# ActiveVisionLab/DFNet

Measured on AMD Instinct MI355X. Metric: rendered rays/sec (64+128 samples, 640x480), higher is better.
Workload: dtype f16x3; 1 GPU; BASELINE configs[1]: synthetic random-weight NeRF-H (D=8, W=128), 640x480, 64+128 samples, test-time render_image, 1 frame per step per GPU; parallelism=frames sharded over 1 GPU(s), gather at end, collectives=none (one rank)

## Files before the change

### dfnet_amd/csrc/nerfh_api.hip

```cpp
#include <hip/hip_runtime.h>

#include <cmath>
#include <cstdarg>
#include <cstdio>
#include <cstdlib>
#include <cstring>
#include <map>
#include <string>
#include <type_traits>
#include <vector>

#include "../../include/dfnet_hip.h"
#include "dfn_common.h"
#include "nerfh_fused_train.h"
#include "nerfh_handle.h"
#include "nerfh_kernels.h"
#include "nerfh_layout.h"

using namespace dfn;

namespace dfn {
static thread_local char g_err[512] = "";
int set_error(int code, const char* fmt, ...) {
  va_list ap;
  va_start(ap, fmt);
  vsnprintf(g_err, sizeof g_err, fmt, ap);
  va_end(ap);
  return code;
}
int device_cu_count() {
  static int n = 0;
  if (!n) {
    int dev = 0;
    hipDeviceProp_t p;
    if (hipGetDevice(&dev) == hipSuccess && hipGetDeviceProperties(&p, dev) == hipSuccess) n = p.multiProcessorCount;
    if (n <= 0) n = 256;
  }
  return n;
}
}

extern "C" const char* dfn_last_error(void) { return g_err; }
extern "C" int dfn_abi_version(void) { return 1; }

static std::map<std::string, std::vector<size_t>> expected_shapes(const dfn_nerfh_desc& d) {
  std::map<std::string, std::vector<size_t>> m;
  const size_t W = d.width, na = size_t(d.hist_bin) * d.dim_a, nt = size_t(d.hist_bin) * d.dim_t;
  for (int f = 0; f < 2; ++f) {
    const std::string pre = f ? "fine." : "coarse.";
    for (int i = 0; i < d.depth; ++i) {
      const size_t k = i == 0 ? kChXyz : (i == 4 ? W + kChXyz : W);
      m[pre + "xyz_encoding_" + std::to_string(i + 1) + ".0.weight"] = {W, k};
      m[pre + "xyz_encoding_" + std::to_string(i + 1) + ".0.bias"] = {W};
    }
    m[pre + "xyz_encoding_final.weight"] = {W, W};
    m[pre + "xyz_encoding_final.bias"] = {W};
    m[pre + "dir_encoding.0.weight"] = {W / 2, W + kChDir + (f ? na : 0)};
    m[pre + "dir_encoding.0.bias"] = {W / 2};
    m[pre + "static_sigma.0.weight"] = {1, W};
    m[pre + "static_sigma.0.bias"] = {1};
    m[pre + "static_rgb.0.weight"] = {3, W / 2};
    m[pre + "static_rgb.0.bias"] = {3};
    if (f) {
      const size_t ks[4] = {W + nt, W / 2, W / 2, W / 2};
      for (int j = 0; j < 4; ++j) {
        m[pre + "transient_encoding." + std::to_string(2 * j) + ".weight"] = {W / 2, ks[j]};
        m[pre + "transient_encoding." + std::to_string(2 * j) + ".bias"] = {W / 2};
      }
      m[pre + "transient_sigma.0.weight"] = {1, W / 2};
      m[pre + "transient_sigma.0.bias"] = {1};
      m[pre + "transient_rgb.0.weight"] = {3, W / 2};
      m[pre + "transient_rgb.0.bias"] = {3};
      m[pre + "transient_beta.0.weight"] = {1, W / 2};
      m[pre + "transient_beta.0.bias"] = {1};
    }
  }
  m["embedding_a.weight"] = {size_t(d.n_vocab), size_t(d.dim_a)};
  m["embedding_t.weight"] = {size_t(d.n_vocab), size_t(d.dim_t)};
  return m;
}

extern "C" int dfn_nerfh_create(const dfn_nerfh_desc* desc, dfn_nerfh_t* out) {
  if (!desc || !out) return set_error(DFN_ERR_ARG, "dfn_nerfh_create: null argument");
  if (desc->depth != 8 || desc->multires != kLxyz || desc->multires_views != kLdir)
    return set_error(DFN_ERR_UNSUPPORTED,
                     "dfn_nerfh_create: kernels are specialised for netdepth=8 multires=%d multires_views=%d (got %d/%d/%d)",
                     kLxyz, kLdir, desc->depth, desc->multires, desc->multires_views);
  if (desc->width < 2 || desc->width > 1024 || (desc->width & 1))
    return set_error(DFN_ERR_UNSUPPORTED, "dfn_nerfh_create: netwidth must be even and in [2, 1024] (got %d)", desc->width);
  if (desc->hist_bin <= 0 || desc->dim_a <= 0 || desc->dim_t <= 0 || desc->n_vocab <= 0 ||
      desc->hist_bin * (desc->dim_a + desc->dim_t) > 1024)
    return set_error(DFN_ERR_ARG, "dfn_nerfh_create: bad embedding geometry");
  auto* h = new dfn_nerfh_s();
  h->desc = *desc;
  *out = h;
  return DFN_OK;
}

static void free_packed(dfn_nerfh_s* h) {
  for (auto& a : h->net)
    for (auto& b : a)
      for (auto& n : b) {
        if (n.blob) (void)hipFree(n.blob);
        if (n.tab) (void)hipFree(n.tab);
        if (n.res_blob) (void)hipFree(n.res_blob);
        n = PackedNet();
      }
  for (PackedNet* n : {&h->bwd[0], &h->bwd[1], &h->bwd[2], &h->half_maps}) {
    if (n->blob) (void)hipFree(n->blob);
    if (n->tab) (void)hipFree(n->tab);
    *n = PackedNet();
  }
  if (h->extra) (void)hipFree(h->extra);
  h->extra = nullptr;
  if (h->gen_blob) (void)hipFree(h->gen_blob);
  h->gen_blob = nullptr;
  h->gen_params.clear();
  h->fast = false;
}

extern "C" int dfn_nerfh_destroy(dfn_nerfh_t h) {
  if (!h) return DFN_OK;
  free_packed(h);
  dfn::fused::destroy_state(h);
  for (hipEvent_t e : h->side_ev) if (e) (void)hipEventDestroy(e);
  if (h->side_stream) (void)hipStreamDestroy(h->side_stream);
  if (h->range_flag) (void)hipFree(h->range_flag);
  delete h;
  return DFN_OK;
}

extern "C" int dfn_nerfh_set_param(dfn_nerfh_t h, const char* name, const float* host, size_t numel) {
  if (!h || !name || !host) return set_error(DFN_ERR_ARG, "dfn_nerfh_set_param: null argument");
  const auto shapes = expected_shapes(h->desc);
  const auto it = shapes.find(name);
  if (it == shapes.end()) return set_error(DFN_ERR_ARG, "dfn_nerfh_set_param: unknown parameter '%s'", name);
  size_t want = 1;
  for (size_t s : it->second) want *= s;
  if (want != numel)
    return set_error(DFN_ERR_ARG, "dfn_nerfh_set_param: '%s' has %zu elements, expected %zu", name, numel, want);
  h->params[name].assign(host, host + numel);
  h->committed = false;
  return DFN_OK;
}

namespace {

struct Mat {
  const float* w = nullptr;
  const float* b = nullptr;
  int rows = 0, cols = 0;
};

struct Packer {
  const dfn_nerfh_s* h;
  std::string pre;
  int width() const { return h->desc.width; }
  mutable int fwd_units = 0;
  std::vector<float> fold_dir, fold_tr;
  bool half_heads = false, half_thead = false;
  bool half_block(int layer) const { return half_heads && (layer == LY_SIG || layer == LY_RGB || (layer == LY_THEAD && half_thead)); }
  Mat mat(const std::string& key) const {
    Mat m;
    const auto& w = h->params.at(pre + key + ".weight");
    const auto& b = h->params.at(pre + key + ".bias");
    m.w = w.data();
    m.b = b.data();
    m.rows = int(b.size());
    m.cols = int(w.size() / b.size());
    return m;
  }
  void row_source(int layer, int mb, int i, Mat& m, int& row) const {
    row = 32 * mb + i;
    switch (layer) {
      case LY_L1: case LY_L2: case LY_L3: case LY_L4: case LY_L5: case LY_L6: case LY_L7: case LY_L8:
        m = mat("xyz_encoding_" + std::to_string(layer - LY_L1 + 1) + ".0");
        break;
      case LY_FIN:
        if (mb < width() / 32) m = mat("xyz_encoding_final");
        else { m = mat("static_sigma.0"); row = i == 0 ? 0 : -1; }
        break;
      case LY_DIR: m = mat("dir_encoding.0"); break;
      case LY_RGB: m = mat("static_rgb.0"); row = i < 3 ? i : -1; break;
      case LY_TE0: m = mat("transient_encoding.0"); break;
      case LY_TE1: m = mat("transient_encoding.2"); break;
      case LY_TE2: m = mat("transient_encoding.4"); break;
      case LY_TE3: m = mat("transient_encoding.6"); break;
      case LY_THEAD:
        if (i < 3) { m = mat("transient_rgb.0"); row = i; }
        else if (i == 3) { m = mat("transient_sigma.0"); row = 0; }
        else if (i == 8) { m = mat("transient_beta.0"); row = 0; }
        else { m = mat("transient_beta.0"); row = -1; }
        break;
      case LY_SIG: m = mat("static_sigma.0"); row = i == 0 ? 0 : -1; break;
      case LY_DIRF: case LY_TE0F:
        m = Mat();
        m.w = (layer == LY_DIRF ? fold_dir : fold_tr).data();
        m.rows = width() / 2;
        m.cols = width();
        break;
    }
  }
  static int col_source(int layer, int hh, int s) {
    if (layer == LY_L1) return pe_xyz_feature(hh, s);
    if (layer == LY_L5) return s < 32 ? pe_xyz_feature(hh, s) : kChXyz + hidden_feature(hh, s - 32);
    return hidden_feature(hh, s);
  }
  static int col_source_m16(int layer, int g, int s) {
    if (layer == LY_L1) return pe_xyz_feature_m16(g, s);
    if (layer == LY_L5) return s < 16 ? pe_xyz_feature_m16(g, s) : kChXyz + hidden_feature_m16(g, s - 16);
    return hidden_feature_m16(g, s);
  }
  bool head_block(int layer, int mb) const {
    return layer == LY_RGB || layer == LY_THEAD || layer == LY_SIG || (layer == LY_FIN && mb == width() / 32);
  }
  int row_m16(int layer, int mb, int i) const { return head_block(layer, mb) ? head_row_m16(i) : i; }
  static bool unit_has_bias(int layer) { return layer != LY_DIR && layer != LY_TE0 && layer != LY_DIRF && layer != LY_TE0F; }

  float wscale = 1.f;
  template <class P>
  void pack_blocks(int layer, int mb0, int group, uint8_t* base) const {
    using Elem = typename std::conditional<P::kSlotsPerChunk == 8, _Float16, float>::type;
    const LayerShape sh = layer_shape(layer, width());
    const int KC = sh.slots / P::kSlotsPerChunk;
    Elem* frag = reinterpret_cast<Elem*>(base);
    const bool half = P::kM16 && half_block(layer);
    const int KCP = half ? KC / 2 : KC;
    float* bias = reinterpret_cast<float*>(base + size_t(group) * KCP * 64 * P::kLaneBytes);
    for (int g = 0; g < group; ++g) {
      const int mb = mb0 + g;
      if constexpr (P::kM16) {
        auto source = [&](int i, Mat& m, int& row) {
          const int ri = row_m16(layer, mb, i);
          if (ri < 0) { m = Mat(); row = -1; return; }
          row_source(layer, mb, ri, m, row);
          if (row >= m.rows) row = -1;
        };
        for (int lane = 0; lane < 64; ++lane)
          for (int kc = 0; kc < KC; ++kc) {
            if (half && (kc & 1)) continue;
            Mat m;
            int row;
            source(16 * (kc & 1) + (lane & 15), m, row);
            for (int j = 0; j < 8; ++j) {
              const int col = col_source_m16(layer, lane >> 4, 8 * (kc >> 1) + j);
              const float v = (row >= 0 && col >= 0 && col < m.cols) ? m.w[size_t(row) * m.cols + col] : 0.f;
              Elem* fr = frag + (size_t(g) * KCP + (half ? kc >> 1 : kc)) * 64 * 16;
              const Elem hi = Elem(v * wscale);
              fr[lane * 8 + j] = hi;
              fr[512 + lane * 8 + j] = Elem(v * wscale - float(hi));
            }
          }
        for (int lg = 0; lg < 4; ++lg)
          for (int ms = 0; ms < 2; ++ms)
            for (int r = 0; r < 4; ++r) {
              Mat m;
              int row;
              source(16 * ms + 4 * lg + r, m, row);
              const float b = (row >= 0 && unit_has_bias(layer)) ? m.b[row] : 0.f;
              bias[g * 32 + lg * 8 + ms * 4 + r] = b * wscale * kX3ActScale;
            }
        continue;
      }
      for (int lane = 0; lane < 64; ++lane) {
        const int i = lane & 31, hh = lane >> 5;
        Mat m;
        int row;
        row_source(layer, mb, i, m, row);
        if (row >= m.rows) row = -1;
        for (int kc = 0; kc < KC; ++kc)
          for (int j = 0; j < P::kSlotsPerChunk; ++j) {
            const int col = col_source(layer, hh, kc * P::kSlotsPerChunk + j);
            const float v = (row >= 0 && col >= 0 && col < m.cols) ? m.w[size_t(row) * m.cols + col] : 0.f;
            if constexpr (P::kSplit) {
              Elem* fr = frag + (size_t(g) * KC + kc) * 64 * 16;
              const Elem hi = Elem(v * wscale);
              fr[lane * 8 + j] = hi;
              fr[512 + lane * 8 + j] = Elem(v * wscale - float(hi));
            } else {
              frag[((size_t(g) * KC + kc) * 64 + lane) * P::kSlotsPerChunk + j] = Elem(v);
            }
          }
      }
      for (int hh = 0; hh < 2; ++hh)
        for (int r = 0; r < 16; ++r) {
          Mat m;
          int row;
          row_source(layer, mb, mblock_row(hh, r), m, row);
          if (row >= m.rows) row = -1;
          const float b = (row >= 0 && unit_has_bias(layer)) ? m.b[row] : 0.f;
          bias[(g * 2 + hh) * 16 + r] = P::kSplit ? b * wscale * kX3ActScale : b;
        }
    }
  }
  float bwd_elem(int layer, int mb, int i, int hh, int s) const {
    const int k = 32 * mb + i;
    auto W = [](const Mat& m, int row, int col) {
      return (row >= 0 && row < m.rows && col >= 0 && col < m.cols) ? m.w[size_t(row) * m.cols + col] : 0.f;
    };
    auto pe_col = [&](int blk) { return pe_xyz_feature(mblock_half_of_row(i), 16 * blk + mblock_reg_of_row(i)); };
    const int j = hidden_feature(hh, s);
    switch (layer) {
      case BW_THEAD:
        if (j < 3) return W(mat("transient_rgb.0"), j, k);
        if (j == 3) return W(mat("transient_sigma.0"), 0, k);
        if (j == 8) return W(mat("transient_beta.0"), 0, k);
        return 0.f;
      case BW_TE3: return W(mat("transient_encoding.6"), j, k);
      case BW_TE2: return W(mat("transient_encoding.4"), j, k);
      case BW_TE1: return W(mat("transient_encoding.2"), j, k);
      case BW_RGB: return j < 3 ? W(mat("static_rgb.0"), j, k) : 0.f;
      case BW_FINCAT: {
        const bool dirpart = s >= 32;
        const int jj = hidden_feature(hh, s & 31);
        if (mb < 4) return W(mat(dirpart ? "dir_encoding.0" : "transient_encoding.0"), jj, k);
        if (!dirpart) return 0.f;
        const int c = pe_dir_feature(mblock_half_of_row(i), mblock_reg_of_row(i));
        return c >= 0 ? W(mat("dir_encoding.0"), jj, kWidth + c) : 0.f;
      }
      case BW_FIN:
        if (s < 64) return W(mat("xyz_encoding_final"), j, k);
        return (s == 64 && hh == 0) ? W(mat("static_sigma.0"), 0, k) : 0.f;
      case BW_L5:
        if (mb < 4) return W(mat("xyz_encoding_5.0"), j, kChXyz + k);
        return W(mat("xyz_encoding_5.0"), j, pe_col(mb - 4));
      case BW_L1: return W(mat("xyz_encoding_1.0"), j, pe_col(mb));
      default: {
        const int n = 8 - (layer - BW_L8);
        return W(mat("xyz_encoding_" + std::to_string(n) + ".0"), j, k);
      }
    }
  }
  template <class P>
  void pack_bwd_blocks(int layer, int mb0, int group, uint8_t* base) const {
    using Elem = typename std::conditional<P::kSlotsPerChunk == 8, _Float16, float>::type;
    const LayerShape sh = bwd_layer_shape(layer);
    const int KC = sh.slots / P::kSlotsPerChunk;
    Elem* frag = reinterpret_cast<Elem*>(base);
    for (int g = 0; g < group; ++g)
      for (int lane = 0; lane < 64; ++lane)
        for (int kc = 0; kc < KC; ++kc)
          for (int j = 0; j < P::kSlotsPerChunk; ++j) {
            const float v = bwd_elem(layer, mb0 + g, lane & 31, lane >> 5, kc * P::kSlotsPerChunk + j);
            if constexpr (P::kSplit) {
              Elem* fr = frag + (size_t(g) * KC + kc) * 64 * 16;
              const Elem hi = Elem(v * wscale);
              fr[lane * 8 + j] = hi;
              fr[512 + lane * 8 + j] = Elem(v * wscale - float(hi));
            } else {
              frag[((size_t(g) * KC + kc) * 64 + lane) * P::kSlotsPerChunk + j] = Elem(v);
            }
          }
  }
  template <class PF, class P>
  void pack_bwd(std::vector<uint8_t>& blob, std::vector<uint32_t>& tab) const {
    pack<PF>(true, bwd_fwd_unit_mb<PF>(), false, blob, tab);
    fwd_units = int(tab.size() / 2);
    const int umb = bwd_unit_mb<P>();
    for (int layer = 0; layer < BW_COUNT; ++layer) {
      const LayerShape sh = bwd_layer_shape(layer);
      for (int u0 = 0; u0 < sh.mb; u0 += umb) {
        const int mb0 = (umb <= 2 && layer == BW_L5) ? (u0 < 2 ? 4 + u0 : u0 - 2) : u0;
        const int group = sh.mb - mb0 < umb ? sh.mb - mb0 : umb;
        const uint32_t bytes = unit_bytes<P>(sh.slots, group);
        const uint32_t off = uint32_t(blob.size());
        blob.resize(off + bytes, 0);
        tab.push_back(off);
        tab.push_back(bytes);
        pack_bwd_blocks<P>(layer, mb0, group, blob.data() + off);
      }
    }
  }

  template <class P>
  uint32_t blocks_bytes(int layer, int group) const {
    const LayerShape sh = layer_shape(layer, width());
    const bool half = P::kM16 && half_block(layer);
    return uint32_t(group) * (sh.slots / P::kSlotsPerChunk / (half ? 2 : 1)) * 64 * P::kLaneBytes + uint32_t(group) * 128;
  }

  template <class P>
  void pack(bool fine, int umb, bool merge, std::vector<uint8_t>& blob, std::vector<uint32_t>& tab, int l5_umb = -1, bool fold = false,
            std::vector<uint8_t>* res = nullptr) const {
    const int* seq = fine ? (fold ? kFineFoldSeq : kFineSeq) : kCoarseSeq;
    const int* grp = fine ? kFineGroup : kCoarseGroup;
    const int nl = fine ? kFineLayers : kCoarseLayers;
    if (merge) {
      for (int li = 0; li < nl;) {
        int lj = li;
        uint32_t bytes = 0;
        while (lj < nl && grp[lj] == grp[li]) bytes += blocks_bytes<P>(seq[lj], layer_shape(seq[lj], width()).mb), ++lj;
        if (seq[li] == LY_L5) {
          const LayerShape sh = layer_shape(LY_L5, width());
          const int g = l5_unit_mb(umb);
          for (int mb0 = 0; mb0 < sh.mb; mb0 += g) {
            const uint32_t ub = unit_bytes<P>(sh.slots, g), uo = uint32_t(blob.size());
            blob.resize(uo + ub, 0);
            tab.push_back(uo);
            tab.push_back(ub);
            pack_blocks<P>(LY_L5, mb0, g, blob.data() + uo);
          }
          li = lj;
          continue;
        }
        const uint32_t off = uint32_t(blob.size());
        blob.resize(off + align_piece(bytes), 0);
        tab.push_back(off);
        tab.push_back(align_piece(bytes));
        uint32_t at = off;
        for (int l = li; l < lj; ++l) {
          pack_blocks<P>(seq[l], 0, layer_shape(seq[l], width()).mb, blob.data() + at);
          at += blocks_bytes<P>(seq[l], layer_shape(seq[l], width()).mb);
        }
        li = lj;
      }
      return;
    }
    for (int li = 0; li < nl; ++li) {
      const LayerShape sh = layer_shape(seq[li], width());
      const int lu = (seq[li] == LY_L5 && l5_umb > 0) ? l5_umb : umb;
      for (int mb0 = 0; mb0 < sh.mb; mb0 += lu) {
        const int group = sh.mb - mb0 < lu ? sh.mb - mb0 : lu;
        if (res && layer_resident(fine, seq[li])) {
          const size_t at = res->size();
          res->resize(at + blocks_bytes<P>(seq[li], group), 0);
          pack_blocks<P>(seq[li], mb0, group, res->data() + at);
          continue;
        }
        const uint32_t bytes = unit_bytes<P>(sh.slots, group, P::kM16 && half_block(seq[li]));
        const uint32_t off = uint32_t(blob.size());
        blob.resize(off + bytes, 0);
        tab.push_back(off);
        tab.push_back(bytes);
        pack_blocks<P>(seq[li], mb0, group, blob.data() + off);
      }
    }
    if (res) res->resize(align_piece(uint32_t(res->size())), 0);
  }
};

void fold_final(const std::vector<float>& a, int rows, int lda, const std::vector<float>& F, const std::vector<float>& bF, int W,
                std::vector<float>& af, std::vector<float>& ab) {
  af.assign(size_t(rows) * W, 0.f);
  ab.assign(rows, 0.f);
  std::vector<double> acc(W);
  for (int r = 0; r < rows; ++r) {
    std::fill(acc.begin(), acc.end(), 0.0);
    double b = 0.0;
    for (int k = 0; k < W; ++k) {
      const double ark = a[size_t(r) * lda + k];
      const float* frow = &F[size_t(k) * W];
      for (int c = 0; c < W; ++c) acc[c] += ark * double(frow[c]);
      b += ark * double(bF[k]);
    }
    for (int c = 0; c < W; ++c) af[size_t(r) * W + c] = float(acc[c]);
    ab[r] = float(b);
  }
}

int upload(const void* src, size_t bytes, void** dst) {
  if (hipMalloc(dst, bytes ? bytes : 16) != hipSuccess) return set_error(DFN_ERR_HIP, "hipMalloc(%zu) failed", bytes);
  if (bytes && hipMemcpy(*dst, src, bytes, hipMemcpyHostToDevice) != hipSuccess)
    return set_error(DFN_ERR_HIP, "hipMemcpy H2D (%zu bytes) failed", bytes);
  return DFN_OK;
}

}

__global__ void range_fetch_kernel(int* flag) { flag[1] = atomicExch(flag, 0); }

extern "C" int dfn_nerfh_set_render_options(dfn_nerfh_t h, int flags) {
  if (!h) return set_error(DFN_ERR_ARG, "dfn_nerfh_set_render_options: null handle");
  if (flags & ~(DFN_RENDER_LINDISP | DFN_RENDER_COARSE_F16)) return set_error(DFN_ERR_UNSUPPORTED, "dfn_nerfh_set_render_options: unknown option bits 0x%x", flags);
  h->render_flags = flags;
  return DFN_OK;
}

extern "C" int dfn_nerfh_range_status(dfn_nerfh_t h, int* flags, void* stream) {
  if (!h) return set_error(DFN_ERR_ARG, "dfn_nerfh_range_status: null handle");
  int v = 0;
  if (h->range_flag) {
    hipStream_t s = static_cast<hipStream_t>(stream);
    hipLaunchKernelGGL(range_fetch_kernel, dim3(1), dim3(1), 0, s, h->range_flag);
    if (hipGetLastError() != hipSuccess || hipMemcpyAsync(&v, h->range_flag + 1, sizeof(int), hipMemcpyDeviceToHost, s) != hipSuccess ||
        hipStreamSynchronize(s) != hipSuccess)
      return set_error(DFN_ERR_HIP, "dfn_nerfh_range_status: reading the flag failed");
  }
  if (flags) { *flags = v; return DFN_OK; }
  if (v)
    return set_error(DFN_ERR_RANGE, "NeRF-H render: activations left the range of the %s arithmetic since the last check (%s); the frames rendered "
                     "since then are not the network's output: render them with DFN_PREC_F32",
                     (v & DFN_RANGE_F16_OVERFLOW) ? "f16" : "split-f16",
                     (v & DFN_RANGE_F16_OVERFLOW) ? "an f16 layer output overflowed to inf: |activation| > 65504"
                                                  : "a split-f16 hi half saturated: |activation| >= 4094 (hidden layers of the render kernels: "
                                                    ">= 4094 x the network's largest |weight|, the accumulators are narrowed before they are scaled)");
  return DFN_OK;
}

extern "C" int dfn_nerfh_range_status_async(dfn_nerfh_t h, int* host_flags, void* stream) {
  if (!h || !host_flags) return set_error(DFN_ERR_ARG, "dfn_nerfh_range_status_async: null handle / destination");
  if (!h->range_flag) { *host_flags = 0; return DFN_OK; }
  hipStream_t s = static_cast<hipStream_t>(stream);
  hipLaunchKernelGGL(range_fetch_kernel, dim3(1), dim3(1), 0, s, h->range_flag);
  if (hipGetLastError() != hipSuccess || hipMemcpyAsync(host_flags, h->range_flag + 1, sizeof(int), hipMemcpyDeviceToHost, s) != hipSuccess)
    return set_error(DFN_ERR_HIP, "dfn_nerfh_range_status_async: enqueueing the read failed");
  return DFN_OK;
}

extern "C" int dfn_nerfh_commit(dfn_nerfh_t h) {
  if (!h) return set_error(DFN_ERR_ARG, "dfn_nerfh_commit: null handle");
  for (const auto& kv : expected_shapes(h->desc))
    if (!h->params.count(kv.first)) return set_error(DFN_ERR_STATE, "dfn_nerfh_commit: parameter '%s' not set", kv.first.c_str());
  free_packed(h);
  dfn::fused::destroy_state(h);
  if (!h->range_flag) {
    if (hipMalloc(reinterpret_cast<void**>(&h->range_flag), 3 * sizeof(int)) != hipSuccess) {
      h->range_flag = nullptr;
      return set_error(DFN_ERR_HIP, "dfn_nerfh_commit: allocating the range-guard flag failed");
    }
    if (hipMemset(h->range_flag, 0, 3 * sizeof(int)) != hipSuccess) return set_error(DFN_ERR_HIP, "dfn_nerfh_commit: clearing the range-guard flag failed");
  }
  {
    std::vector<float> all;
    std::vector<size_t> offs;
    const int np = dfn_nerfh_train_param_count();
    for (int i = 0; i < np; ++i) {
      const auto& v = h->params.at(dfn_nerfh_train_param_name(i));
      offs.push_back(all.size());
      all.insert(all.end(), v.begin(), v.end());
      all.resize((all.size() + 3) & ~size_t(3));
    }
    int rc = upload(all.data(), all.size() * 4, reinterpret_cast<void**>(&h->gen_blob));
    if (rc) return rc;
    for (size_t o : offs) h->gen_params.push_back(h->gen_blob + o);
  }
  const int Wd = h->desc.width;
  std::vector<float> fold_bd, fold_bt;
  if (Wd != kWidth && Wd != kMaxWidth) {
    h->committed = true;
    return DFN_OK;
  }
  if (Wd == kMaxWidth) {
    for (int f = 0; f < 2; ++f)
      for (int prec = 0; prec < 3; ++prec) {
        Packer pk{h, f ? "fine." : "coarse."};
        std::vector<uint8_t> blob;
        std::vector<uint32_t> tab;
        PackedNet& n = h->net[f][prec][0];
        if (prec == DFN_PREC_F16) pk.pack<PrecF16>(f, unit_mb_w256<PrecF16>(), false, blob, tab);
        else if (prec == DFN_PREC_F32) pk.pack<PrecF32>(f, unit_mb_w256<PrecF32>(), false, blob, tab);
        else {
          float wmax = 0.f;
          for (const auto& kv : h->params)
            if (kv.first.compare(0, pk.pre.size(), pk.pre) == 0 && kv.first.find(".weight") != std::string::npos)
              for (float v : kv.second) wmax = std::fmax(wmax, std::fabs(v));
          int sexp = wmax > 0.f ? -int(std::ceil(std::log2(wmax))) : 0;
          sexp = sexp < -8 ? -8 : (sexp > 24 ? 24 : sexp);
          pk.wscale = std::ldexp(1.f, sexp);
          n.in_scale = pk.wscale * kX3ActScale;
          pk.pack<PrecX3>(f, unit_mb_w256<PrecX3>(), false, blob, tab);
        }
        int rc = upload(blob.data(), blob.size(), reinterpret_cast<void**>(&n.blob));
        if (rc) return rc;
        rc = upload(tab.data(), tab.size() * 4, reinterpret_cast<void**>(&n.tab));
        if (rc) return rc;
        n.n_units = int(tab.size() / 2);
      }
  } else {
  for (int f = 0; f < 2; ++f)
    for (int prec = 0; prec < 3; ++prec)
      for (int var = 0; var < kVariants; ++var) {
        const bool resident = var == kResidentVariant;
        const bool half = var == kHalfVariant || resident;
        const bool fold = var == kFoldVariant || (half && f == 1);
        if (var == kFoldVariant && !(f == 1 && prec == DFN_PREC_F16X3)) continue;
        if (half && prec != DFN_PREC_F16X3) continue;
        Packer pk{h, f ? "fine." : "coarse."};
        pk.half_heads = half;
        pk.half_thead = half;
        std::vector<uint8_t> blob, rblob;
        std::vector<uint8_t>* res = resident ? &rblob : nullptr;
        std::vector<uint32_t> tab;
        PackedNet& n = h->net[f][prec][var];
        if (prec == DFN_PREC_F16) pk.pack<PrecF16>(f, unit_mb<PrecF16>(var), unit_mb<PrecF16>(var) >= 8, blob, tab);
        else if (prec == DFN_PREC_F32) pk.pack<PrecF32>(f, unit_mb<PrecF32>(var), false, blob, tab);
        else {
          float wmax = 0.f;
          for (const auto& kv : h->params)
            if (kv.first.compare(0, pk.pre.size(), pk.pre) == 0 && kv.first.find(".weight") != std::string::npos)
              for (float v : kv.second) wmax = std::fmax(wmax, std::fabs(v));
          int sexp = wmax > 0.f ? -int(std::ceil(std::log2(wmax))) : 0;
          sexp = sexp < -8 ? -8 : (sexp > 24 ? 24 : sexp);
          pk.wscale = std::ldexp(1.f, sexp);
          n.in_scale = pk.wscale * kX3ActScale;
          if (fold) {
            const int ldd = Wd + kChDir + h->desc.hist_bin * h->desc.dim_a, ldt = Wd + h->desc.hist_bin * h->desc.dim_t;
            const auto& F = h->params.at("fine.xyz_encoding_final.weight");
            const auto& bF = h->params.at("fine.xyz_encoding_final.bias");
            fold_final(h->params.at("fine.dir_encoding.0.weight"), Wd / 2, ldd, F, bF, Wd, pk.fold_dir, fold_bd);
            fold_final(h->params.at("fine.transient_encoding.0.weight"), Wd / 2, ldt, F, bF, Wd, pk.fold_tr, fold_bt);
            pk.pack<PrecX3M16>(f, unit_mb<PrecX3M16>(var), false, blob, tab, l5_unit_mb_p<PrecX3M16>(unit_mb<PrecX3M16>(var)), true, res);
            if (half && !resident) {
              std::vector<uint8_t> mblob;
              std::vector<uint32_t> mtab;
              pk.half_thead = false;
              pk.pack<PrecX3M16>(f, unit_mb<PrecX3M16>(var), false, mblob, mtab, l5_unit_mb_p<PrecX3M16>(unit_mb<PrecX3M16>(var)), true);
              PackedNet& m = h->half_maps;
              m.in_scale = n.in_scale;
              int rc = upload(mblob.data(), mblob.size(), reinterpret_cast<void**>(&m.blob));
              if (rc) return rc;
              rc = upload(mtab.data(), mtab.size() * 4, reinterpret_cast<void**>(&m.tab));
              if (rc) return rc;
              m.n_units = int(mtab.size() / 2);
            }
          } else if (var == 4 || half) pk.pack<PrecX3M16>(f, unit_mb<PrecX3M16>(var), false, blob, tab, l5_unit_mb_p<PrecX3M16>(unit_mb<PrecX3M16>(var)), false, res);
          else pk.pack<PrecX3>(f, unit_mb<PrecX3>(var), false, blob, tab, l5_unit_mb_p<PrecX3>(unit_mb<PrecX3>(var)));
        }
        int rc = upload(blob.data(), blob.size(), reinterpret_cast<void**>(&n.blob));
        if (rc) return rc;
        rc = upload(tab.data(), tab.size() * 4, reinterpret_cast<void**>(&n.tab));
        if (rc) return rc;
        n.n_units = int(tab.size() / 2);
        if (resident) {
          if (rblob.size() != resident_bytes<PrecX3M16>(f != 0))
            return set_error(DFN_ERR_STATE, "dfn_nerfh_commit: the resident layers pack to %zu bytes, the kernels expect %u", rblob.size(),
                             resident_bytes<PrecX3M16>(f != 0));
          rc = upload(rblob.data(), rblob.size(), reinterpret_cast<void**>(&n.res_blob));
          if (rc) return rc;
          n.res_bytes = uint32_t(rblob.size());
        }
      }
  for (int prec = 0; prec < 3; ++prec) {
    Packer pk{h, "fine."};
    std::vector<uint8_t> blob;
    std::vector<uint32_t> tab;
    PackedNet& n = h->bwd[prec];
    if (prec == DFN_PREC_F16) pk.pack_bwd<PrecF16, PrecF16>(blob, tab);
    else if (prec == DFN_PREC_F32) pk.pack_bwd<PrecF32, PrecF32>(blob, tab);
    else {
      n.in_scale = h->net[1][2][0].in_scale * 1024.f;
      pk.wscale = n.in_scale / kX3ActScale;
      pk.pack_bwd<PrecX3, PrecX3>(blob, tab);
    }
    int rc = upload(blob.data(), blob.size(), reinterpret_cast<void**>(&n.blob));
    if (rc) return rc;
    rc = upload(tab.data(), tab.size() * 4, reinterpret_cast<void**>(&n.tab));
    if (rc) return rc;
    n.n_units = int(tab.size() / 2);
    n.n_fwd_units = pk.fwd_units;
  }
  }
  const dfn_nerfh_desc& d = h->desc;
  const int na = d.hist_bin * d.dim_a, nt = d.hist_bin * d.dim_t, kd = kChDir + na, NO = Wd / 2;
  const auto& wd = h->params.at("fine.dir_encoding.0.weight");
  const auto& bd = h->params.at("fine.dir_encoding.0.bias");
  const auto& wt = h->params.at("fine.transient_encoding.0.weight");
  const auto& bt = h->params.at("fine.transient_encoding.0.bias");
  const auto& ea = h->params.at("embedding_a.weight");
  const auto& et = h->params.at("embedding_t.weight");
  std::vector<float> ex;
  const size_t o_wd = 0, o_bd = o_wd + size_t(kd) * NO, o_wt = o_bd + NO, o_bt = o_wt + size_t(nt) * NO,
               o_ea = o_bt + NO, o_et = o_ea + ea.size(), o_bdf = o_et + et.size(), o_btf = o_bdf + NO;
  ex.resize(o_btf + NO);
  const int ld_d = Wd + kd, ld_t = Wd + nt;
  for (int j = 0; j < kd; ++j)
    for (int f = 0; f < NO; ++f) ex[o_wd + size_t(j) * NO + f] = wd[size_t(f) * ld_d + Wd + j];
  for (int j = 0; j < nt; ++j)
    for (int f = 0; f < NO; ++f) ex[o_wt + size_t(j) * NO + f] = wt[size_t(f) * ld_t + Wd + j];
  std::memcpy(&ex[o_bd], bd.data(), NO * 4);
  std::memcpy(&ex[o_bt], bt.data(), NO * 4);
  std::memcpy(&ex[o_ea], ea.data(), ea.size() * 4);
  std::memcpy(&ex[o_et], et.data(), et.size() * 4);
  for (int f = 0; f < NO; ++f) {
    ex[o_bdf + f] = fold_bd.empty() ? bd[f] : bd[f] + fold_bd[f];
    ex[o_btf + f] = fold_bt.empty() ? bt[f] : bt[f] + fold_bt[f];
  }
  int rc = upload(ex.data(), ex.size() * 4, reinterpret_cast<void**>(&h->extra));
  if (rc) return rc;
  h->rb.w_dir = h->extra + o_wd;
  h->rb.b_dir = h->extra + o_bd;
  h->rb.w_tr = h->extra + o_wt;
  h->rb.b_tr = h->extra + o_bt;
  h->rb.emb_a = h->extra + o_ea;
  h->rb.emb_t = h->extra + o_et;
  h->rb.hist_bin = d.hist_bin;
  h->rb.dim_a = d.dim_a;
  h->rb.dim_t = d.dim_t;
  h->rb.n_vocab = d.n_vocab;
  h->rb.nout = NO;
  h->rb_fold = h->rb;
  h->rb_fold.b_dir = h->extra + o_bdf;
  h->rb_fold.b_tr = h->extra + o_btf;
  h->committed = true;
  h->fast = true;
  return DFN_OK;
}

namespace {
struct KernelTimer {
  bool on = false;
  std::vector<std::pair<hipEvent_t, hipEvent_t>> ev[DFN_PROF_SLOTS];
} g_prof;
struct ScopedTimer {
  int which;
  hipStream_t s;
  hipEvent_t a = nullptr, b = nullptr;
  ScopedTimer(int w, hipStream_t st) : which(w), s(st) {
    if (!g_prof.on) return;
    (void)hipEventCreate(&a);
    (void)hipEventCreate(&b);
    (void)hipEventRecord(a, s);
  }
  ~ScopedTimer() {
    if (!a) return;
    (void)hipEventRecord(b, s);
    g_prof.ev[which].emplace_back(a, b);
  }
};
}

extern "C" int dfn_profile_enable(int on) {
  for (auto& v : g_prof.ev) {
    for (auto& p : v) { (void)hipEventDestroy(p.first); (void)hipEventDestroy(p.second); }
    v.clear();
  }
  g_prof.on = on != 0;
  return DFN_OK;
}
extern "C" int dfn_profile_read(int which, double* avg_ms, int* launches) {
  if (which < 0 || which >= DFN_PROF_SLOTS || !avg_ms || !launches) return set_error(DFN_ERR_ARG, "dfn_profile_read: bad argument");
  double tot = 0;
  for (auto& p : g_prof.ev[which]) {
    float ms = 0;
    if (hipEventSynchronize(p.second) != hipSuccess || hipEventElapsedTime(&ms, p.first, p.second) != hipSuccess)
      return set_error(DFN_ERR_HIP, "dfn_profile_read: event query failed");
    tot += ms;
  }
  *launches = int(g_prof.ev[which].size());
  *avg_ms = *launches ? tot / *launches : 0.0;
  return DFN_OK;
}

#define HS(s) reinterpret_cast<hipStream_t>(s)
#define CHECK_HIP(expr, what)                                                                   \
  do {                                                                                          \
    hipError_t e_ = (expr);                                                                     \
    if (e_ != hipSuccess) return set_error(DFN_ERR_HIP, "%s: %s", what, hipGetErrorString(e_)); \
  } while (0)

static int check_net(dfn_nerfh_t h, int prec, const char* fn, bool allow_x3 = false) {
  if (!h) return set_error(DFN_ERR_ARG, "%s: null handle", fn);
  if (!h->committed) return set_error(DFN_ERR_STATE, "%s: dfn_nerfh_commit() has not been called", fn);
  if (!h->fast)
    return set_error(DFN_ERR_UNSUPPORTED, "%s: the register-resident kernels exist for netwidth %d and %d (this handle: %d); "
                     "use the generic-width entry points (dfn_nerfh_generic_*)", fn, kWidth, kMaxWidth, h->desc.width);
  if (prec != DFN_PREC_F16 && prec != DFN_PREC_F32 && !(allow_x3 && prec == DFN_PREC_F16X3))
    return set_error(DFN_ERR_ARG, "%s: unknown / unsupported precision %d", fn, prec);
  return DFN_OK;
}

static int check_grad_width(dfn_nerfh_t h, const char* fn) {
  if (h->desc.width != kWidth)
    return set_error(DFN_ERR_UNSUPPORTED, "%s: the input-gradient kernels are built for netwidth %d only (this handle: %d)", fn, kWidth,
                     h->desc.width);
  return DFN_OK;
}
static int check_grad_prec(int prec, const char* fn) {
  if (prec == DFN_PREC_F16)
    return set_error(DFN_ERR_UNSUPPORTED, "%s: gradients run in DFN_PREC_F16X3 or DFN_PREC_F32 only (plain-f16 ReLU gates are 3e-2 off "
                     "autograd)", fn);
  return DFN_OK;
}

constexpr int kDefaultVariant = kResidentVariant;
static int mlp_variant_128();
static int mlp_variant_of(dfn_nerfh_t h) { return h->desc.width == kWidth ? mlp_variant_128() : 0; }
static int mlp_variant_128() {
  static int v = -1;
  if (v < 0) {
    const char* e = getenv("DFN_MLP_VARIANT");
    v = (e && e[0] >= '0' && e[0] < '0' + kVariants) ? e[0] - '0' : kDefaultVariant;
  }
  return v;
}
static int base_variant(int var) { return var == kFoldVariant || var == kHalfVariant || var == kResidentVariant ? 4 : var; }
static bool fold_fine(int var, int prec) { return (var == kFoldVariant || var == kHalfVariant || var == kResidentVariant) && prec == DFN_PREC_F16X3; }
static bool half_heads(int var, int prec) { return (var == kHalfVariant || var == kResidentVariant) && prec == DFN_PREC_F16X3; }
static bool resident_layers(int var, int prec) { return var == kResidentVariant && prec == DFN_PREC_F16X3; }
static MlpResArgs res_args(const MlpArgs& a, const PackedNet& n) {
  MlpResArgs r{};
  static_cast<MlpArgs&>(r) = a;
  r.res_blob = n.res_blob;
  r.res_bytes = n.res_bytes;
  return r;
}

static int* range_flag_of(dfn_nerfh_t h) { return h->range_flag; }

static unsigned long long* g_timing_buf = nullptr;
extern "C" void dfn_debug_set_timing_buffer(void* p) { g_timing_buf = static_cast<unsigned long long*>(p); }


extern "C" int dfn_raygen(int H, int W, float focal, const float* c2w, float* rays_o, float* rays_d,
                          float* viewdirs, void* stream) {
  if (H < 0 || W < 0 || !c2w || !rays_o || !rays_d || !(focal > 0)) return set_error(DFN_ERR_ARG, "dfn_raygen: bad argument");
  CHECK_HIP(launch_raygen(H, W, focal, c2w, rays_o, rays_d, viewdirs, HS(stream)), "dfn_raygen");
  return DFN_OK;
}

extern "C" int dfn_posenc(const float* x, size_t n, int L, int mode, float* out, void* stream) {
  if (!x || !out || L < 0 || L > 16 || (mode != 0 && mode != 1)) return set_error(DFN_ERR_ARG, "dfn_posenc: bad argument");
  CHECK_HIP(launch_posenc(x, n, L, mode, out, HS(stream)), "dfn_posenc");
  return DFN_OK;
}

extern "C" int dfn_mlp_coarse(dfn_nerfh_t h, int prec, const float* rays_o, const float* rays_d, size_t n_rays,
                              int Nc, float near, float far, float* sigma, void* stream) {
  if (int rc = check_net(h, prec, "dfn_mlp_coarse", true)) return rc;
  if (!n_rays) return DFN_OK;
  if (!rays_o || !rays_d || !sigma || Nc < 1) return set_error(DFN_ERR_ARG, "dfn_mlp_coarse: bad argument");
  const bool half = half_heads(mlp_variant_of(h), prec), res = resident_layers(mlp_variant_of(h), prec);
  const int var = base_variant(mlp_variant_of(h));
  const PackedNet& n = h->net[0][prec][res ? kResidentVariant : (half ? kHalfVariant : var)];
  MlpArgs a{n.blob, n.tab, n.n_units, rays_o, rays_d, nullptr, nullptr, sigma, nullptr, (long long)n_rays, Nc, near, far, nullptr, n.in_scale,
            h->render_flags & DFN_RENDER_LINDISP};
  a.status = range_flag_of(h);
  ScopedTimer t(0, HS(stream));
  if (res) CHECK_HIP(launch_mlp_res(false, res_args(a, n), device_cu_count(), HS(stream)), "dfn_mlp_coarse");
  else if (half) CHECK_HIP(launch_mlp_half(false, false, a, device_cu_count(), HS(stream)), "dfn_mlp_coarse");
  else CHECK_HIP(launch_mlp(false, prec, var, a, device_cu_count(), HS(stream), h->desc.width), "dfn_mlp_coarse");
  return DFN_OK;
}

extern "C" int dfn_coarse_weights(const float* sigma, const float* z, size_t n, int N, float* weights, void* stream) {
  if (!sigma || !z || !weights || N < 1 || N > 2048) return set_error(DFN_ERR_ARG, "dfn_coarse_weights: bad argument");
  CHECK_HIP(launch_coarse_weights(sigma, z, n, N, weights, HS(stream)), "dfn_coarse_weights");
  return DFN_OK;
}

extern "C" int dfn_sample_pdf(const float* bins, const float* weights, size_t n, int nb, int Ni, const float* u,
                              float* out, void* stream) {
  if (!bins || !weights || !out || nb < 2 || Ni < 1 || 3 * nb + 2 * Ni > 8192)
    return set_error(DFN_ERR_ARG, "dfn_sample_pdf: bad argument");
  CHECK_HIP(launch_sample_pdf(bins, weights, n, nb, Ni, u, out, HS(stream)), "dfn_sample_pdf");
  return DFN_OK;
}

extern "C" int dfn_sample_fine_opt(const float* sigma, size_t n_rays, int Nc, int Ni, float near, float far, int render_flags,
                                   float* z_fine, float* weights_coarse, float* z_samples, void* stream) {
  if (!sigma || !z_fine || Nc < 3 || Ni < 1 || 6 * Nc + 2 * Ni > 8192)
    return set_error(DFN_ERR_ARG, "dfn_sample_fine: bad argument (need N_samples >= 3, N_importance >= 1)");
  if ((render_flags & DFN_RENDER_LINDISP) && !(near > 0.f))
    return set_error(DFN_ERR_ARG, "dfn_sample_fine: lindisp needs near > 0");
  CHECK_HIP(launch_sample_fine(sigma, n_rays, Nc, Ni, near, far, z_fine, weights_coarse, z_samples, HS(stream),
                               render_flags & DFN_RENDER_LINDISP),
            "dfn_sample_fine");
  return DFN_OK;
}
extern "C" int dfn_sample_fine(const float* sigma, size_t n_rays, int Nc, int Ni, float near, float far,
                               float* z_fine, float* weights_coarse, float* z_samples, void* stream) {
  return dfn_sample_fine_opt(sigma, n_rays, Nc, Ni, near, far, 0, z_fine, weights_coarse, z_samples, stream);
}

extern "C" int dfn_ndc_rays(int H, int W, float focal, float near, const float* rays_o, const float* rays_d, size_t n, float* out_o,
                            float* out_d, void* stream) {
  if (!n) return DFN_OK;
  if (!rays_o || !rays_d || !out_o || !out_d || H < 1 || W < 1 || !(focal > 0.f)) return set_error(DFN_ERR_ARG, "dfn_ndc_rays: bad argument");
  CHECK_HIP(launch_ndc_rays(H, W, focal, near, rays_o, rays_d, n, out_o, out_d, HS(stream)), "dfn_ndc_rays");
  return DFN_OK;
}

extern "C" int dfn_upsample_bicubic(const float* in, int H, int W, int C, int outH, int outW, float* out, void* stream) {
  if (!in || !out || H < 1 || W < 1 || C < 1 || outH < 1 || outW < 1) return set_error(DFN_ERR_ARG, "dfn_upsample_bicubic: bad argument");
  CHECK_HIP(launch_bicubic(in, H, W, C, outH, outW, out, HS(stream)), "dfn_upsample_bicubic");
  return DFN_OK;
}

extern "C" int dfn_upsample_bicubic_frames(const float* in, int B, int H, int W, int C, int outH, int outW, int out_nchw, float* out,
                                           void* stream) {
  if (!in || !out || B < 1 || H < 1 || W < 1 || C < 1 || outH < 1 || outW < 1) return set_error(DFN_ERR_ARG, "dfn_upsample_bicubic_frames: bad argument");
  CHECK_HIP(launch_bicubic(in, H, W, C, outH, outW, out, HS(stream), B, out_nchw != 0), "dfn_upsample_bicubic_frames");
  return DFN_OK;
}
extern "C" int dfn_upsample_bicubic_frames_backward(const float* grad_out, int B, int H, int W, int C, int outH, int outW, int out_nchw,
                                                    float* grad_in, void* stream) {
  if (!grad_out || !grad_in || B < 1 || H < 1 || W < 1 || C < 1 || outH < 1 || outW < 1)
    return set_error(DFN_ERR_ARG, "dfn_upsample_bicubic_frames_backward: bad argument");
  CHECK_HIP(launch_bicubic_backward(grad_out, H, W, C, outH, outW, grad_in, HS(stream), B, out_nchw != 0), "dfn_upsample_bicubic_frames_backward");
  return DFN_OK;
}

extern "C" int dfn_upsample_bicubic_backward(const float* grad_out, int H, int W, int C, int outH, int outW, float* grad_in,
                                             void* stream) {
  if (!grad_out || !grad_in || H < 1 || W < 1 || C < 1 || outH < 1 || outW < 1)
    return set_error(DFN_ERR_ARG, "dfn_upsample_bicubic_backward: bad argument");
  CHECK_HIP(launch_bicubic_backward(grad_out, H, W, C, outH, outW, grad_in, HS(stream)), "dfn_upsample_bicubic_backward");
  return DFN_OK;
}

extern "C" size_t dfn_fine_bias_bytes(size_t n_rays) { return (n_rays ? n_rays : 1) * ray_bias_floats(kMaxWidth) * sizeof(float); }

extern "C" int dfn_mlp_fine(dfn_nerfh_t h, int prec, const float* rays_o, const float* rays_d, const float* viewdirs,
                            const float* hist, size_t hist_rows, size_t n_rays, const float* z_fine, int Nf,
                            float* raw, void* bias_ws, void* stream) {
  if (int rc = check_net(h, prec, "dfn_mlp_fine", true)) return rc;
  if (!n_rays) return DFN_OK;
  if (!rays_o || !rays_d || !viewdirs || !hist || !z_fine || !raw || !bias_ws || Nf < 1 ||
      (hist_rows != 1 && hist_rows != n_rays))
    return set_error(DFN_ERR_ARG, "dfn_mlp_fine: bad argument (hist_rows must be 1 or n_rays)");
  float* table = static_cast<float*>(bias_ws);
  const bool fold = fold_fine(mlp_variant_of(h), prec);
  const int var = fold ? kFoldVariant : base_variant(mlp_variant_of(h));
  CHECK_HIP(launch_ray_bias(fold ? h->rb_fold : h->rb, viewdirs, hist, hist_rows, n_rays, table, HS(stream)), "dfn_mlp_fine(ray_bias)");
  const PackedNet& n = h->net[1][prec][var];
  MlpArgs a{n.blob, n.tab, n.n_units, rays_o, rays_d, z_fine, table, raw, nullptr, (long long)n_rays, Nf, 0.f, 0.f, g_timing_buf, n.in_scale};
  a.status = range_flag_of(h);
  ScopedTimer t(1, HS(stream));
  if (fold) CHECK_HIP(launch_mlp_fold(false, a, device_cu_count(), HS(stream)), "dfn_mlp_fine");
  else CHECK_HIP(launch_mlp(true, prec, var, a, device_cu_count(), HS(stream), h->desc.width), "dfn_mlp_fine");
  return DFN_OK;
}

extern "C" int dfn_composite_fine(const float* raw, const float* z, size_t n_rays, int Nf, float beta_min, int flags,
                                  float* rgb, float* disp, float* acc, float* depth, float* weights, float* beta,
                                  void* stream) {
  if (!raw || !z || !rgb || !disp || !acc || Nf < 1 || Nf > 512)
    return set_error(DFN_ERR_ARG, "dfn_composite_fine: bad argument (1 <= Nf <= 512)");
  CHECK_HIP(launch_composite_fine(raw, z, n_rays, Nf, beta_min, flags, rgb, disp, acc, depth, weights, beta, HS(stream)),
            "dfn_composite_fine");
  return DFN_OK;
}

static MapPtrs map_ptrs(const dfn_render_maps* m) {
  return m ? MapPtrs{m->depth, m->depth_static, m->beta, m->rgb_static, m->rgb_transient} : MapPtrs{};
}

extern "C" int dfn_composite_fine_maps(const float* raw, const float* z, size_t n_rays, int Nf, float beta_min,
                                       const dfn_render_maps* maps, void* stream) {
  if (!raw || !z || Nf < 1 || Nf > 512) return set_error(DFN_ERR_ARG, "dfn_composite_fine_maps: bad argument (1 <= Nf <= 512)");
  CHECK_HIP(launch_composite_fine_maps(raw, z, n_rays, Nf, beta_min, map_ptrs(maps), HS(stream)), "dfn_composite_fine_maps");
  return DFN_OK;
}

namespace {
constexpr size_t kMaxChunkRays = 65536;
inline size_t al(size_t b) { return (b + 255) & ~size_t(255); }
inline size_t chunk_rays(size_t n_rays) {
  const size_t passes = (n_rays + kMaxChunkRays - 1) / kMaxChunkRays;
  const size_t c = passes ? (n_rays + passes - 1) / passes : 1;
  return (c + 63) & ~size_t(63);
}
struct Workspace {
  float *o, *d, *v, *sigma, *z, *raw, *bias, *partial;
  size_t total;
};
Workspace carve(char* base, size_t n_rays, int Nc, int Ni, bool own_rays, int rec_floats = 12) {
  const size_t chunk = chunk_rays(n_rays);
  const size_t Nf = size_t(Nc) + Ni;
  Workspace w{};
  size_t off = 0;
  auto take = [&](size_t bytes) { char* p = base ? base + off : nullptr; off += al(bytes); return reinterpret_cast<float*>(p); };
  w.o = take(own_rays ? n_rays * 12 : 0);
  w.d = take(own_rays ? n_rays * 12 : 0);
  w.v = take(n_rays * 12);
  w.sigma = take(chunk * Nc * 4);
  w.z = take(chunk * Nf * 4);
  w.raw = take(chunk * Nf * 9 * 4);
  w.bias = take(chunk * ray_bias_floats(kMaxWidth) * 4);
  w.partial = take(chunk * ((Nf + 31) / 32) * rec_floats * 4);
  w.total = off;
  return w;
}

int render_core(dfn_nerfh_t h, int prec, const float* o, const float* d, const float* v, const float* hist,
                size_t hist_rows, size_t n_rays, int Nc, int Ni, float near, float far, float* rgb, float* disp,
                float* acc, float* raw_out, const Workspace& w, hipStream_t s, const MapPtrs& maps = MapPtrs{}) {
  const int Nf = Nc + Ni;
  const bool want_maps = maps.any();
  const bool fold = fold_fine(mlp_variant_of(h), prec);
  const int var = base_variant(mlp_variant_of(h));
  const int seg = prec == DFN_PREC_F16 ? 64 : 32;
  const bool fused = !raw_out && Nf % seg == 0 && !(prec == DFN_PREC_F16 && var == 2) && h->desc.width == kWidth;
  const int cprec = (h->render_flags & DFN_RENDER_COARSE_F16) ? DFN_PREC_F16 : prec;
  const bool half_c = half_heads(mlp_variant_of(h), cprec), half_f = half_heads(mlp_variant_of(h), prec) && fused;
  const bool res_c = resident_layers(mlp_variant_of(h), cprec), res_f = resident_layers(mlp_variant_of(h), prec) && fused && !want_maps;
  const PackedNet& nc = h->net[0][cprec][res_c ? kResidentVariant : (half_c ? kHalfVariant : var)];
  const PackedNet& nf = res_f ? h->net[1][prec][kResidentVariant]
                      : half_f ? (want_maps ? h->half_maps : h->net[1][prec][kHalfVariant]) : h->net[1][prec][fold ? kFoldVariant : var];
  const int cus = device_cu_count();
  const size_t chunk = chunk_rays(n_rays);
  for (size_t r0 = 0; r0 < n_rays; r0 += chunk) {
    const size_t n = n_rays - r0 < chunk ? n_rays - r0 : chunk;
    const float* co = o + r0 * 3;
    const float* cd = d + r0 * 3;
    const float* cv = v + r0 * 3;
    const float* ch = hist_rows == 1 ? hist : hist + r0 * h->desc.hist_bin;
    float* raw = raw_out ? raw_out + r0 * size_t(Nf) * 9 : w.raw;
    {
      MlpArgs a{nc.blob, nc.tab, nc.n_units, co, cd, nullptr, nullptr, w.sigma, nullptr, (long long)n, Nc, near, far, nullptr, nc.in_scale,
                 h->render_flags & DFN_RENDER_LINDISP};
      a.status = range_flag_of(h);
      ScopedTimer t(0, s);
      if (res_c) CHECK_HIP(launch_mlp_res(false, res_args(a, nc), cus, s), "render: coarse MLP (resident layers)");
      else if (half_c) CHECK_HIP(launch_mlp_half(false, false, a, cus, s), "render: coarse MLP (half-height heads)");
      else CHECK_HIP(launch_mlp(false, cprec, var, a, cus, s, h->desc.width), "render: coarse MLP");
    }
    {
      ScopedTimer t(DFN_PROF_SAMPLE_FINE, s);
      CHECK_HIP(launch_sample_fine(w.sigma, n, Nc, Ni, near, far, w.z, nullptr, nullptr, s, h->render_flags & DFN_RENDER_LINDISP),
                "render: sample_fine");
    }
    {
      ScopedTimer t(DFN_PROF_RAY_BIAS, s);
      CHECK_HIP(launch_ray_bias(fold ? h->rb_fold : h->rb, cv, ch, hist_rows, n, w.bias, s), "render: ray_bias");
    }
    {
      MlpArgs a{nf.blob, nf.tab, nf.n_units, co, cd, w.z, w.bias, raw, fused ? w.partial : nullptr, (long long)n, Nf, 0.f, 0.f, g_timing_buf, nf.in_scale};
      a.status = range_flag_of(h);
      ScopedTimer t(1, s);
      if (res_f) CHECK_HIP(launch_mlp_res(true, res_args(a, nf), cus, s), "render: fine MLP (resident layers)");
      else if (half_f) CHECK_HIP(launch_mlp_half(true, want_maps, a, cus, s), "render: fine MLP (half-height heads)");
      else if (fold) CHECK_HIP(launch_mlp_fold(fused && want_maps, a, cus, s), "render: fine MLP (folded)");
      else if (fused && want_maps) CHECK_HIP(launch_mlp_maps(true, prec, var, a, cus, s, h->desc.width), "render: fine MLP (maps)");
      else CHECK_HIP(launch_mlp(true, prec, var, a, cus, s, h->desc.width), "render: fine MLP");
    }
    if (fused && want_maps) {
      ScopedTimer t(DFN_PROF_COMBINE, s);
      CHECK_HIP(launch_composite_combine_maps(w.partial, n, Nf / seg, 0.1f, DFN_COMP_TEST_TIME | DFN_COMP_STATIC_ONLY, rgb + r0 * 3,
                                              disp + r0, acc + r0, maps.at(r0), s),
                "render: composite combine (maps)");
    } else if (fused) {
      ScopedTimer t(DFN_PROF_COMBINE, s);
      CHECK_HIP(launch_composite_combine(w.partial, n, Nf / seg, 0.1f, DFN_COMP_TEST_TIME | DFN_COMP_STATIC_ONLY, rgb + r0 * 3,
                                         disp + r0, acc + r0, s),
                "render: composite combine");
    } else {
      ScopedTimer t(DFN_PROF_COMPOSITE, s);
      CHECK_HIP(launch_composite_fine(raw, w.z, n, Nf, 0.1f, DFN_COMP_TEST_TIME | DFN_COMP_STATIC_ONLY, rgb + r0 * 3,
                                      disp + r0, acc + r0, nullptr, nullptr, nullptr, s),
                "render: composite");
      if (want_maps) CHECK_HIP(launch_composite_fine_maps(raw, w.z, n, Nf, 0.1f, maps.at(r0), s), "render: composite (maps)");
    }
  }
  return DFN_OK;
}

int check_render_args(int Nc, int Ni, const char* fn) {
  if (Nc < 3 || Ni < 1 || Nc + Ni > 512 || 6 * Nc + 2 * Ni > 8192)
    return set_error(DFN_ERR_UNSUPPORTED, "%s: need 3 <= N_samples, 1 <= N_importance, N_samples+N_importance <= 512", fn);
  return DFN_OK;
}
}

extern "C" size_t dfn_render_workspace_bytes(size_t n_rays, int Nc, int Ni) {
  return carve(nullptr, n_rays ? n_rays : 1, Nc, Ni, true).total;
}

static int render_rays_entry(const char* fn, dfn_nerfh_t h, int prec, const float* rays_o, const float* rays_d, const float* viewdirs,
                             const float* hist, size_t hist_rows, size_t n_rays, int Nc, int Ni, float near, float far,
                             float* rgb, float* disp, float* acc, float* raw, void* workspace, size_t workspace_bytes,
                             const MapPtrs& maps, void* stream) {
  if (int rc = check_net(h, prec, fn, true)) return rc;
  if (int rc = check_render_args(Nc, Ni, fn)) return rc;
  if (!n_rays) return DFN_OK;
  if (!rays_o || !rays_d || !hist || !rgb || !disp || !acc || !workspace || (hist_rows != 1 && hist_rows != n_rays))
    return set_error(DFN_ERR_ARG, "%s: bad argument (hist_rows must be 1 or n_rays)", fn);
  const Workspace w = carve(static_cast<char*>(workspace), n_rays, Nc, Ni, true, maps.any() ? kMapsRecFloats : 12);
  if (w.total > workspace_bytes)
    return set_error(DFN_ERR_ARG, "%s: workspace too small (%zu < %zu)", fn, workspace_bytes, w.total);
  const float* v = viewdirs;
  if (!v) {
    if (hipError_t e = launch_viewdirs(rays_d, n_rays, w.v, HS(stream)); e != hipSuccess)
      return set_error(DFN_ERR_HIP, "%s: viewdirs: %s", fn, hipGetErrorString(e));
    v = w.v;
  }
  return render_core(h, prec, rays_o, rays_d, v, hist, hist_rows, n_rays, Nc, Ni, near, far, rgb, disp, acc, raw, w,
                     HS(stream), maps);
}

static int render_image_entry(const char* fn, dfn_nerfh_t h, int prec, const float* c2w, int H, int W, float focal, float near,
                              float far, int Nc, int Ni, const float* hist, float* rgb, float* disp, float* acc,
                              void* workspace, size_t workspace_bytes, const MapPtrs& maps, void* stream) {
  if (int rc = check_net(h, prec, fn, true)) return rc;
  if (int rc = check_render_args(Nc, Ni, fn)) return rc;
  if (!c2w || !hist || !rgb || !disp || !acc || !workspace || H < 1 || W < 1 || !(focal > 0))
    return set_error(DFN_ERR_ARG, "%s: bad argument", fn);
  const size_t n_rays = size_t(H) * W;
  const Workspace w = carve(static_cast<char*>(workspace), n_rays, Nc, Ni, true, maps.any() ? kMapsRecFloats : 12);
  if (w.total > workspace_bytes)
    return set_error(DFN_ERR_ARG, "%s: workspace too small (%zu < %zu)", fn, workspace_bytes, w.total);
  if (hipError_t e = launch_raygen(H, W, focal, c2w, w.o, w.d, w.v, HS(stream)); e != hipSuccess)
    return set_error(DFN_ERR_HIP, "%s: raygen: %s", fn, hipGetErrorString(e));
  return render_core(h, prec, w.o, w.d, w.v, hist, 1, n_rays, Nc, Ni, near, far, rgb, disp, acc, nullptr, w, HS(stream), maps);
}

extern "C" int dfn_render_rays(dfn_nerfh_t h, int prec, const float* rays_o, const float* rays_d, const float* viewdirs,
                               const float* hist, size_t hist_rows, size_t n_rays, int Nc, int Ni, float near, float far,
                               float* rgb, float* disp, float* acc, float* raw, void* workspace, size_t workspace_bytes,
                               void* stream) {
  return render_rays_entry("dfn_render_rays", h, prec, rays_o, rays_d, viewdirs, hist, hist_rows, n_rays, Nc, Ni, near, far, rgb, disp,
                           acc, raw, workspace, workspace_bytes, MapPtrs{}, stream);
}

extern "C" int dfn_render_image(dfn_nerfh_t h, int prec, const float* c2w, int H, int W, float focal, float near,
                                float far, int Nc, int Ni, const float* hist, float* rgb, float* disp, float* acc,
                                void* workspace, size_t workspace_bytes, void* stream) {
  return render_image_entry("dfn_render_image", h, prec, c2w, H, W, focal, near, far, Nc, Ni, hist, rgb, disp, acc, workspace,
                            workspace_bytes, MapPtrs{}, stream);
}

extern "C" size_t dfn_render_maps_workspace_bytes(size_t n_rays, int Nc, int Ni) {
  return carve(nullptr, n_rays ? n_rays : 1, Nc, Ni, true, kMapsRecFloats).total;
}

extern "C" int dfn_render_rays_maps(dfn_nerfh_t h, int prec, const float* rays_o, const float* rays_d, const float* viewdirs,
                                    const float* hist, size_t hist_rows, size_t n_rays, int Nc, int Ni, float near, float far,
                                    float* rgb, float* disp, float* acc, float* raw, void* workspace, size_t workspace_bytes,
                                    const dfn_render_maps* maps, void* stream) {
  return render_rays_entry("dfn_render_rays_maps", h, prec, rays_o, rays_d, viewdirs, hist, hist_rows, n_rays, Nc, Ni, near, far, rgb,
                           disp, acc, raw, workspace, workspace_bytes, map_ptrs(maps), stream);
}

extern "C" int dfn_render_image_maps(dfn_nerfh_t h, int prec, const float* c2w, int H, int W, float focal, float near,
                                     float far, int Nc, int Ni, const float* hist, float* rgb, float* disp, float* acc,
                                     void* workspace, size_t workspace_bytes, const dfn_render_maps* maps, void* stream) {
  return render_image_entry("dfn_render_image_maps", h, prec, c2w, H, W, focal, near, far, Nc, Ni, hist, rgb, disp, acc, workspace,
                            workspace_bytes, map_ptrs(maps), stream);
}

extern "C" int dfn_composite_fine_backward(const float* raw, const float* z, const float* grad_rgb, size_t n_rays, int Nf,
                                           float* grad_raw, void* stream) {
  if (!raw || !z || !grad_rgb || !grad_raw || Nf < 1 || Nf > 512)
    return set_error(DFN_ERR_ARG, "dfn_composite_fine_backward: bad argument (1 <= Nf <= 512)");
  CHECK_HIP(launch_composite_fine_backward(raw, z, grad_rgb, n_rays, Nf, grad_raw, HS(stream)), "dfn_composite_fine_backward");
  return DFN_OK;
}

extern "C" int dfn_composite_fine_backward_maps(const float* raw, const float* z, size_t n_rays, int Nf, float beta_min,
                                                const dfn_map_grads* grads, const float* grad_raw_ext, float* grad_raw, void* stream) {
  if (!raw || !z || !grad_raw || Nf < 1 || Nf > 512)
    return set_error(DFN_ERR_ARG, "dfn_composite_fine_backward_maps: bad argument (1 <= Nf <= 512)");
  const MapGrads g = grads ? MapGrads{grads->rgb, grads->acc, grads->depth, grads->depth_static, grads->disp, grads->beta,
                                      grads->rgb_static, grads->rgb_transient}
                           : MapGrads{};
  if (!g.any() && !grad_raw_ext)
    return set_error(DFN_ERR_ARG, "dfn_composite_fine_backward_maps: bad argument (no upstream gradient and no grad_raw_ext)");
  CHECK_HIP(launch_composite_fine_backward_all(raw, z, n_rays, Nf, beta_min, g, grad_raw, HS(stream), grad_raw_ext),
            "dfn_composite_fine_backward_maps");
  return DFN_OK;
}

extern "C" int dfn_mlp_fine_backward(dfn_nerfh_t h, int prec, const float* rays_o, const float* rays_d, const float* viewdirs,
                                     const float* hist, size_t hist_rows, size_t n_rays, const float* z_fine, int Nf,
                                     const float* grad_raw, float* grad_pts, void* bias_ws, void* stream) {
  if (int rc = check_net(h, prec, "dfn_mlp_fine_backward", true)) return rc;
  if (int rc = check_grad_prec(prec, "dfn_mlp_fine_backward")) return rc;
  if (int rc = check_grad_width(h, "dfn_mlp_fine_backward")) return rc;
  if (!n_rays) return DFN_OK;
  if (!rays_o || !rays_d || !viewdirs || !hist || !z_fine || !grad_raw || !grad_pts || !bias_ws || Nf < 1 ||
      (hist_rows != 1 && hist_rows != n_rays))
    return set_error(DFN_ERR_ARG, "dfn_mlp_fine_backward: bad argument (hist_rows must be 1 or n_rays)");
  float* table = static_cast<float*>(bias_ws);
  CHECK_HIP(launch_ray_bias(h->rb, viewdirs, hist, hist_rows, n_rays, table, HS(stream)), "dfn_mlp_fine_backward(ray_bias)");
  const PackedNet& n = h->bwd[prec];
  BwdArgs a{n.blob, n.tab, n.n_units, rays_o, rays_d, viewdirs, z_fine, table, grad_raw, grad_pts, (long long)n_rays, Nf, n.in_scale};
  CHECK_HIP(launch_mlp_fine_backward(prec, a, device_cu_count(), HS(stream)), "dfn_mlp_fine_backward");
  return DFN_OK;
}

static int check_points(size_t n_rows, int N, const char* fn) {
  if (N < 1) return set_error(DFN_ERR_ARG, "%s: bad argument (N >= 1)", fn);
  if (n_rows > ((size_t(1) << 31) - 1) / size_t(N)) return set_error(DFN_ERR_ARG, "%s: n_rows * N must stay below 2^31 (chunk by rows)", fn);
  return DFN_OK;
}

extern "C" int dfn_mlp_coarse_points(dfn_nerfh_t h, int prec, const float* pts, size_t n_rows, int N, float* sigma, void* stream) {
  if (int rc = check_net(h, prec, "dfn_mlp_coarse_points", true)) return rc;
  if (!n_rows) return DFN_OK;
  if (!pts || !sigma) return set_error(DFN_ERR_ARG, "dfn_mlp_coarse_points: bad argument");
  if (int rc = check_points(n_rows, N, "dfn_mlp_coarse_points")) return rc;
  const bool w128 = h->desc.width == kWidth;
  const bool half = w128 && half_heads(kDefaultVariant, prec);
  const PackedNet& n = h->net[0][prec][half ? kHalfVariant : (w128 ? base_variant(kDefaultVariant) : 0)];
  MlpArgs a{n.blob, n.tab, n.n_units, pts, nullptr, nullptr, nullptr, sigma, nullptr, (long long)n_rows, N, 0.f, 0.f, nullptr, n.in_scale};
  a.status = range_flag_of(h);
  if (half) CHECK_HIP(launch_mlp_pts_half(a, device_cu_count(), HS(stream)), "dfn_mlp_coarse_points");
  else CHECK_HIP(launch_mlp_pts(false, prec, a, device_cu_count(), HS(stream), h->desc.width), "dfn_mlp_coarse_points");
  return DFN_OK;
}

extern "C" int dfn_mlp_fine_points(dfn_nerfh_t h, int prec, const float* pts, const float* viewdirs, const float* hist, size_t hist_rows,
                                   size_t n_rows, int N, float* raw, void* bias_ws, void* stream) {
  if (int rc = check_net(h, prec, "dfn_mlp_fine_points", true)) return rc;
  if (!n_rows) return DFN_OK;
  if (!pts || !viewdirs || !hist || !raw || !bias_ws || (hist_rows != 1 && hist_rows != n_rows))
    return set_error(DFN_ERR_ARG, "dfn_mlp_fine_points: bad argument (hist_rows must be 1 or n_rows)");
  if (int rc = check_points(n_rows, N, "dfn_mlp_fine_points")) return rc;
  float* table = static_cast<float*>(bias_ws);
  const bool w128 = h->desc.width == kWidth;
  const bool fold = w128 && fold_fine(kDefaultVariant, prec);
  CHECK_HIP(launch_ray_bias(fold ? h->rb_fold : h->rb, viewdirs, hist, hist_rows, n_rows, table, HS(stream)), "dfn_mlp_fine_points(ray_bias)");
  const PackedNet& n = h->net[1][prec][fold ? kFoldVariant : (w128 ? base_variant(kDefaultVariant) : 0)];
  MlpArgs a{n.blob, n.tab, n.n_units, pts, nullptr, nullptr, table, raw, nullptr, (long long)n_rows, N, 0.f, 0.f, nullptr, n.in_scale};
  a.status = range_flag_of(h);
  if (fold) CHECK_HIP(launch_mlp_pts_fold(a, device_cu_count(), HS(stream)), "dfn_mlp_fine_points");
  else CHECK_HIP(launch_mlp_pts(true, prec, a, device_cu_count(), HS(stream), h->desc.width), "dfn_mlp_fine_points");
  return DFN_OK;
}

extern "C" int dfn_mlp_fine_points_backward(dfn_nerfh_t h, int prec, const float* pts, const float* viewdirs, const float* hist,
                                            size_t hist_rows, size_t n_rows, int N, const float* grad_raw, float* grad_pts, void* bias_ws,
                                            void* stream) {
  if (int rc = check_net(h, prec, "dfn_mlp_fine_points_backward", true)) return rc;
  if (int rc = check_grad_prec(prec, "dfn_mlp_fine_points_backward")) return rc;
  if (int rc = check_grad_width(h, "dfn_mlp_fine_points_backward")) return rc;
  if (!n_rows) return DFN_OK;
  if (!pts || !viewdirs || !hist || !grad_raw || !grad_pts || !bias_ws || (hist_rows != 1 && hist_rows != n_rows))
    return set_error(DFN_ERR_ARG, "dfn_mlp_fine_points_backward: bad argument (hist_rows must be 1 or n_rows)");
  if (int rc = check_points(n_rows, N, "dfn_mlp_fine_points_backward")) return rc;
  float* table = static_cast<float*>(bias_ws);
  CHECK_HIP(launch_ray_bias(h->rb, viewdirs, hist, hist_rows, n_rows, table, HS(stream)), "dfn_mlp_fine_points_backward(ray_bias)");
  const PackedNet& n = h->bwd[prec];
  BwdArgs a{n.blob, n.tab, n.n_units, pts, nullptr, viewdirs, nullptr, table, grad_raw, grad_pts, (long long)n_rows, N, n.in_scale};
  CHECK_HIP(launch_mlp_fine_backward_pts(prec, a, device_cu_count(), HS(stream)), "dfn_mlp_fine_points_backward");
  return DFN_OK;
}

extern "C" size_t dfn_mlp_fine_mask_bytes(size_t n_points) {
  return (n_points + kBwdTilePoints - 1) / kBwdTilePoints * (kBwdTilePoints / 32) * kBwdMaskWords * 64 * sizeof(uint32_t);
}

extern "C" int dfn_mlp_fine_saving(dfn_nerfh_t h, int prec, const float* rays_o, const float* rays_d, const float* viewdirs,
                                   const float* hist, size_t hist_rows, size_t n_rays, const float* z_fine, int Nf, float* raw,
                                   void* masks, void* bias_ws, void* stream) {
  if (int rc = check_net(h, prec, "dfn_mlp_fine_saving", true)) return rc;
  if (int rc = check_grad_width(h, "dfn_mlp_fine_saving")) return rc;
  if (prec != DFN_PREC_F16X3) return set_error(DFN_ERR_UNSUPPORTED, "dfn_mlp_fine_saving: split-f16 (DFN_PREC_F16X3) only");
  if (!n_rays) return DFN_OK;
  if (!rays_o || !rays_d || !viewdirs || !hist || !z_fine || !raw || !masks || !bias_ws || Nf < 1 ||
      (hist_rows != 1 && hist_rows != n_rays))
    return set_error(DFN_ERR_ARG, "dfn_mlp_fine_saving: bad argument (hist_rows must be 1 or n_rays)");
  float* table = static_cast<float*>(bias_ws);
  CHECK_HIP(launch_ray_bias(h->rb, viewdirs, hist, hist_rows, n_rays, table, HS(stream)), "dfn_mlp_fine_saving(ray_bias)");
  const PackedNet& n = h->net[1][prec][0];
  MlpArgs a{n.blob, n.tab, n.n_units, rays_o, rays_d, z_fine, table, raw, nullptr, (long long)n_rays, Nf, 0.f, 0.f, nullptr, n.in_scale};
  a.status = range_flag_of(h);
  a.masks = static_cast<uint32_t*>(masks);
  CHECK_HIP(launch_mlp(true, prec, 0, a, device_cu_count(), HS(stream), h->desc.width), "dfn_mlp_fine_saving");
  return DFN_OK;
}

extern "C" int dfn_mlp_fine_backward_saved(dfn_nerfh_t h, int prec, const float* rays_o, const float* rays_d, const float* viewdirs,
                                           size_t n_rays, const float* z_fine, int Nf, const float* raw, const void* masks,
                                           const float* grad_raw, float* grad_pts, void* stream) {
  if (int rc = check_net(h, prec, "dfn_mlp_fine_backward_saved", true)) return rc;
  if (int rc = check_grad_width(h, "dfn_mlp_fine_backward_saved")) return rc;
  if (prec != DFN_PREC_F16X3) return set_error(DFN_ERR_UNSUPPORTED, "dfn_mlp_fine_backward_saved: split-f16 (DFN_PREC_F16X3) only");
  if (!n_rays) return DFN_OK;
  if (!rays_o || !rays_d || !viewdirs || !z_fine || !raw || !masks || !grad_raw || !grad_pts || Nf < 1)
    return set_error(DFN_ERR_ARG, "dfn_mlp_fine_backward_saved: bad argument");
  const PackedNet& n = h->bwd[prec];
  BwdArgs a{n.blob, n.tab + 2 * n.n_fwd_units, n.n_units - n.n_fwd_units, rays_o, rays_d, viewdirs, z_fine, nullptr, grad_raw, grad_pts,
            (long long)n_rays, Nf, n.in_scale, nullptr, raw, static_cast<uint32_t*>(const_cast<void*>(masks))};
  CHECK_HIP(launch_mlp_fine_backward(prec, a, device_cu_count(), HS(stream), 2), "dfn_mlp_fine_backward_saved");
  return DFN_OK;
}

extern "C" int dfn_ray_grad_reduce(const float* grad_pts, const float* z_fine, const float* rays_d, size_t n_rays, int Nf,
                                   int derive_viewdirs, float* grad_rays_o, float* grad_rays_d, float* grad_viewdirs,
                                   void* stream) {
  if (!grad_pts || !z_fine || !rays_d || !grad_rays_o || !grad_rays_d || Nf < 1)
    return set_error(DFN_ERR_ARG, "dfn_ray_grad_reduce: bad argument");
  CHECK_HIP(launch_ray_grad_reduce(grad_pts, z_fine, rays_d, n_rays, Nf, derive_viewdirs, grad_rays_o, grad_rays_d, grad_viewdirs,
                                   HS(stream)),
            "dfn_ray_grad_reduce");
  return DFN_OK;
}

extern "C" int dfn_raygen_frames(int B, int H, int W, float focal, const float* c2w, float* rays_o, float* rays_d, float* viewdirs,
                                 void* stream) {
  if (B < 1 || H < 0 || W < 0 || !c2w || !rays_o || !rays_d || !(focal > 0)) return set_error(DFN_ERR_ARG, "dfn_raygen_frames: bad argument");
  CHECK_HIP(launch_raygen(H, W, focal, c2w, rays_o, rays_d, viewdirs, HS(stream), B), "dfn_raygen_frames");
  return DFN_OK;
}
extern "C" int dfn_raygen_frames_backward(int B, int H, int W, float focal, const float* grad_rays_o, const float* grad_rays_d,
                                          float* grad_c2w, void* stream) {
  if (B < 1 || H < 1 || W < 1 || !grad_rays_o || !grad_rays_d || !grad_c2w || !(focal > 0))
    return set_error(DFN_ERR_ARG, "dfn_raygen_frames_backward: bad argument");
  CHECK_HIP(launch_raygen_backward(H, W, focal, grad_rays_o, grad_rays_d, grad_c2w, HS(stream), B), "dfn_raygen_frames_backward");
  return DFN_OK;
}

extern "C" int dfn_raygen_backward(int H, int W, float focal, const float* grad_rays_o, const float* grad_rays_d, float* grad_c2w,
                                   void* stream) {
  if (H < 1 || W < 1 || !(focal > 0) || !grad_rays_o || !grad_rays_d || !grad_c2w)
    return set_error(DFN_ERR_ARG, "dfn_raygen_backward: bad argument");
  CHECK_HIP(launch_raygen_backward(H, W, focal, grad_rays_o, grad_rays_d, grad_c2w, HS(stream)), "dfn_raygen_backward");
  return DFN_OK;
}

namespace {
struct BwdWorkspace {
  Workspace f;
  float *graw, *gpts, *go, *gd;
  size_t total;
};
BwdWorkspace carve_bwd(char* base, size_t n_rays, int Nc, int Ni) {
  BwdWorkspace b{};
  b.f = carve(base, n_rays, Nc, Ni, true);
  const size_t chunk = chunk_rays(n_rays), Nf = size_t(Nc) + Ni;
  size_t off = b.f.total;
  auto take = [&](size_t bytes) { char* p = base ? base + off : nullptr; off += al(bytes); return reinterpret_cast<float*>(p); };
  b.graw = take(chunk * Nf * 9 * 4);
  b.gpts = take(chunk * Nf * 6 * 4);
  b.go = take(n_rays * 12);
  b.gd = take(n_rays * 12);
  b.total = off;
  return b;
}

int render_backward_core(dfn_nerfh_t h, int prec, const float* o, const float* d, const float* v, bool derive_v,
                         const float* hist, size_t hist_rows, size_t n_rays, int Nc, int Ni, float near, float far,
                         const float* grad_rgb, float* go, float* gd, float* gv, const BwdWorkspace& w, hipStream_t s) {
  const int Nf = Nc + Ni, var = base_variant(mlp_variant_of(h)), cus = device_cu_count();
  const PackedNet& nc = h->net[0][prec][var];
  const PackedNet& nf = h->net[1][prec][var];
  const PackedNet& nb = h->bwd[prec];
  const size_t chunk = chunk_rays(n_rays);
  for (size_t r0 = 0; r0 < n_rays; r0 += chunk) {
    const size_t n = n_rays - r0 < chunk ? n_rays - r0 : chunk;
    const float* co = o + r0 * 3;
    const float* cd = d + r0 * 3;
    const float* cv = v + r0 * 3;
    const float* ch = hist_rows == 1 ? hist : hist + r0 * h->desc.hist_bin;
    MlpArgs ac{nc.blob, nc.tab, nc.n_units, co, cd, nullptr, nullptr, w.f.sigma, nullptr, (long long)n, Nc, near, far, nullptr, nc.in_scale,
                 h->render_flags & DFN_RENDER_LINDISP};
    ac.status = range_flag_of(h);
    CHECK_HIP(launch_mlp(false, prec, var, ac, cus, s, h->desc.width), "render backward: coarse MLP");
    CHECK_HIP(launch_sample_fine(w.f.sigma, n, Nc, Ni, near, far, w.f.z, nullptr, nullptr, s, h->render_flags & DFN_RENDER_LINDISP),
              "render backward: sample_fine");
    CHECK_HIP(launch_ray_bias(h->rb, cv, ch, hist_rows, n, w.f.bias, s), "render backward: ray_bias");
    MlpArgs af{nf.blob, nf.tab, nf.n_units, co, cd, w.f.z, w.f.bias, w.f.raw, nullptr, (long long)n, Nf, 0.f, 0.f, nullptr, nf.in_scale};
    af.status = range_flag_of(h);
    CHECK_HIP(launch_mlp(true, prec, var, af, cus, s, h->desc.width), "render backward: fine MLP");
    CHECK_HIP(launch_composite_fine_backward(w.f.raw, w.f.z, grad_rgb + r0 * 3, n, Nf, w.graw, s), "render backward: composite");
    BwdArgs ab{nb.blob, nb.tab, nb.n_units, co, cd, cv, w.f.z, w.f.bias, w.graw, w.gpts, (long long)n, Nf, nb.in_scale};
    CHECK_HIP(launch_mlp_fine_backward(prec, ab, cus, s), "render backward: fine MLP gradient");
    CHECK_HIP(launch_ray_grad_reduce(w.gpts, w.f.z, cd, n, Nf, derive_v ? 1 : 0, go + r0 * 3, gd + r0 * 3,
                                     gv ? gv + r0 * 3 : nullptr, s),
              "render backward: ray reduction");
  }
  return DFN_OK;
}
}

extern "C" size_t dfn_render_backward_workspace_bytes(size_t n_rays, int Nc, int Ni) {
  return carve_bwd(nullptr, n_rays ? n_rays : 1, Nc, Ni).total;
}

extern "C" int dfn_render_rays_backward(dfn_nerfh_t h, int prec, const float* rays_o, const float* rays_d, const float* viewdirs,
                                        const float* hist, size_t hist_rows, size_t n_rays, int Nc, int Ni, float near,
                                        float far, const float* grad_rgb, float* grad_rays_o, float* grad_rays_d,
                                        float* grad_viewdirs, void* workspace, size_t workspace_bytes, void* stream) {
  if (int rc = check_net(h, prec, "dfn_render_rays_backward", true)) return rc;
  if (int rc = check_grad_prec(prec, "dfn_render_rays_backward")) return rc;
  if (int rc = check_grad_width(h, "dfn_render_rays_backward")) return rc;
  if (int rc = check_render_args(Nc, Ni, "dfn_render_rays_backward")) return rc;
  if (!n_rays) return DFN_OK;
  if (!rays_o || !rays_d || !hist || !grad_rgb || !grad_rays_o || !grad_rays_d || !workspace ||
      (hist_rows != 1 && hist_rows != n_rays))
    return set_error(DFN_ERR_ARG, "dfn_render_rays_backward: bad argument (hist_rows must be 1 or n_rays)");
  if (!n_rays) return DFN_OK;
  const BwdWorkspace w = carve_bwd(static_cast<char*>(workspace), n_rays, Nc, Ni);
  if (w.total > workspace_bytes)
    return set_error(DFN_ERR_ARG, "dfn_render_rays_backward: workspace too small (%zu < %zu)", workspace_bytes, w.total);
  const float* v = viewdirs;
  if (!v) {
    CHECK_HIP(launch_viewdirs(rays_d, n_rays, w.f.v, HS(stream)), "dfn_render_rays_backward: viewdirs");
    v = w.f.v;
  }
  return render_backward_core(h, prec, rays_o, rays_d, v, viewdirs == nullptr, hist, hist_rows, n_rays, Nc, Ni, near, far,
                              grad_rgb, grad_rays_o, grad_rays_d, viewdirs ? grad_viewdirs : nullptr, w, HS(stream));
}

extern "C" int dfn_render_image_backward(dfn_nerfh_t h, int prec, const float* c2w, int H, int W, float focal, float near,
                                         float far, int Nc, int Ni, const float* hist, const float* grad_rgb,
                                         float* grad_c2w, void* workspace, size_t workspace_bytes, void* stream) {
  if (int rc = check_net(h, prec, "dfn_render_image_backward", true)) return rc;
  if (int rc = check_grad_prec(prec, "dfn_render_image_backward")) return rc;
  if (int rc = check_grad_width(h, "dfn_render_image_backward")) return rc;
  if (int rc = check_render_args(Nc, Ni, "dfn_render_image_backward")) return rc;
  if (!c2w || !hist || !grad_rgb || !grad_c2w || !workspace || H < 1 || W < 1 || !(focal > 0))
    return set_error(DFN_ERR_ARG, "dfn_render_image_backward: bad argument");
  const size_t n_rays = size_t(H) * W;
  const BwdWorkspace w = carve_bwd(static_cast<char*>(workspace), n_rays, Nc, Ni);
  if (w.total > workspace_bytes)
    return set_error(DFN_ERR_ARG, "dfn_render_image_backward: workspace too small (%zu < %zu)", workspace_bytes, w.total);
  CHECK_HIP(launch_raygen(H, W, focal, c2w, w.f.o, w.f.d, w.f.v, HS(stream)), "dfn_render_image_backward: raygen");
  if (int rc = render_backward_core(h, prec, w.f.o, w.f.d, w.f.v, true, hist, 1, n_rays, Nc, Ni, near, far, grad_rgb, w.go,
                                    w.gd, nullptr, w, HS(stream)))
    return rc;
  CHECK_HIP(launch_raygen_backward(H, W, focal, w.go, w.gd, grad_c2w, HS(stream)), "dfn_render_image_backward: raygen");
  return DFN_OK;
}
```

### dfnet_amd/csrc/nerfh_handle.h

```cpp
#pragma once
#include <map>
#include <string>
#include <vector>

#include "../../include/dfnet_hip.h"
#include "nerfh_kernels.h"
#include "nerfh_layout.h"

struct PackedNet {
  char* blob = nullptr;
  uint32_t* tab = nullptr;
  int n_units = 0;
  int n_fwd_units = 0;
  float in_scale = 1.f;
  char* res_blob = nullptr;
  uint32_t res_bytes = 0;
};

struct dfn_nerfh_s {
  dfn_nerfh_desc desc;
  std::map<std::string, std::vector<float>> params;
  bool committed = false;
  PackedNet net[2][3][dfn::kVariants];
  PackedNet half_maps;
  PackedNet bwd[3];
  float* extra = nullptr;
  dfn::RayBiasWeights rb{};
  dfn::RayBiasWeights rb_fold{};
  bool fast = false;
  float* gen_blob = nullptr;
  std::vector<const float*> gen_params;
  int render_flags = 0;
  int* range_flag = nullptr;
  void* fused = nullptr;
  bool train_forward_exact = false;
  bool train_split_fine = false;
  bool train_forward_split = false;
  bool train_exact = false;
  hipStream_t side_stream = nullptr;
  hipEvent_t side_ev[2] = {nullptr, nullptr};
};
```

### dfnet_amd/csrc/nerfh_kernels.h

```cpp
#pragma once
#include <hip/hip_runtime.h>
#include <stddef.h>
#include <stdint.h>

namespace dfn {

struct MlpArgs {
  const char* blob;
  const uint32_t* tab;
  int n_units;
  const float* rays_o;
  const float* rays_d;
  const float* z;
  const float* ray_bias;
  float* out;
  float* partial;
  long long n_rays;
  int n_samples;
  float near, far;
  unsigned long long* timing;
  float in_scale;
  int lindisp;
  int dma_waves;
  int* status;
  uint32_t* masks;
};

constexpr int kMapsRecFloats = 16;
hipError_t launch_mlp(bool fine, int prec, int variant, const MlpArgs& a, int n_cu, hipStream_t stream, int width = 128);
hipError_t launch_mlp_maps(bool fine, int prec, int variant, const MlpArgs& a, int n_cu, hipStream_t stream, int width = 128);
hipError_t launch_mlp_fold(bool maps, const MlpArgs& a, int n_cu, hipStream_t stream);
hipError_t launch_mlp_half(bool fine, bool maps, const MlpArgs& a, int n_cu, hipStream_t stream);
struct MlpResArgs : MlpArgs {
  const char* res_blob;
  uint32_t res_bytes;
};
hipError_t launch_mlp_res(bool fine, const MlpResArgs& a, int n_cu, hipStream_t stream);

hipError_t launch_mlp_pts(bool fine, int prec, const MlpArgs& a, int n_cu, hipStream_t stream, int width = 128);
hipError_t launch_mlp_pts_fold(const MlpArgs& a, int n_cu, hipStream_t stream);
hipError_t launch_mlp_pts_half(const MlpArgs& a, int n_cu, hipStream_t stream);

hipError_t launch_raygen(int H, int W, float focal, const float* c2w, float* rays_o, float* rays_d,
                         float* viewdirs, hipStream_t stream, int frames = 1);
hipError_t launch_viewdirs(const float* rays_d, size_t n, float* viewdirs, hipStream_t stream);
hipError_t launch_ndc_rays(int H, int W, float focal, float near, const float* rays_o, const float* rays_d, size_t n, float* out_o,
                           float* out_d, hipStream_t stream);
hipError_t launch_posenc(const float* x, size_t n, int L, int mode, float* out, hipStream_t stream);

struct RayBiasWeights {
  const float* w_dir;
  const float* b_dir;
  const float* w_tr;
  const float* b_tr;
  const float* emb_a;
  const float* emb_t;
  int hist_bin, dim_a, dim_t, n_vocab;
  int nout;
};
hipError_t launch_ray_bias(const RayBiasWeights& w, const float* viewdirs, const float* hist,
                           size_t hist_rows, size_t n_rays, float* table, hipStream_t stream);

hipError_t launch_coarse_weights(const float* sigma, const float* z, size_t n, int N, float* weights,
                                 hipStream_t stream);
hipError_t launch_sample_pdf(const float* bins, const float* weights, size_t n, int nb, int Ni,
                             const float* u, float* out, hipStream_t stream);
hipError_t launch_sample_fine(const float* sigma, size_t n_rays, int Nc, int Ni, float near, float far,
                              float* z_fine, float* weights_coarse, float* z_samples, hipStream_t stream, int lindisp = 0);
hipError_t launch_composite_fine(const float* raw, const float* z, size_t n_rays, int Nf, float beta_min,
                                 int flags, float* rgb, float* disp, float* acc, float* depth,
                                 float* weights, float* beta, hipStream_t stream);

hipError_t launch_composite_combine(const float* partial, size_t n_rays, int segs, float beta_min, int flags, float* rgb,
                                    float* disp, float* acc, hipStream_t stream);

struct MapPtrs {
  float *depth, *depth_static, *beta, *rgb_static, *rgb_transient;
  bool any() const { return depth || depth_static || beta || rgb_static || rgb_transient; }
  MapPtrs at(size_t ray) const {
    return MapPtrs{depth ? depth + ray : nullptr, depth_static ? depth_static + ray : nullptr, beta ? beta + ray : nullptr,
                   rgb_static ? rgb_static + ray * 3 : nullptr, rgb_transient ? rgb_transient + ray * 3 : nullptr};
  }
};
hipError_t launch_composite_fine_maps(const float* raw, const float* z, size_t n_rays, int Nf, float beta_min, const MapPtrs& maps,
                                      hipStream_t stream);
hipError_t launch_composite_combine_maps(const float* partial, size_t n_rays, int segs, float beta_min, int flags, float* rgb,
                                         float* disp, float* acc, const MapPtrs& maps, hipStream_t stream);

struct BwdArgs {
  const char* blob;
  const uint32_t* tab;
  int n_units;
  const float* rays_o;
  const float* rays_d;
  const float* viewdirs;
  const float* z;
  const float* ray_bias;
  const float* graw;
  float* gpts;
  long long n_rays;
  int n_samples;
  float in_scale;
  float* raw_out;
  const float* raw_in;
  uint32_t* masks;
};
constexpr int kBwdMaskWords = 21;
constexpr int kBwdTilePoints = 256;
hipError_t launch_mlp_fine_backward(int prec, const BwdArgs& a, int n_cu, hipStream_t stream, int mode = 0);
hipError_t launch_mlp_fine_backward_pts(int prec, const BwdArgs& a, int n_cu, hipStream_t stream, int mode = 0);
hipError_t launch_composite_fine_backward(const float* raw, const float* z, const float* grad_rgb, size_t n_rays, int Nf,
                                          float* graw, hipStream_t stream, const float* grad_raw_ext = nullptr);
struct MapGrads {
  const float *rgb, *acc, *depth, *depth_static, *disp, *beta, *rgb_static, *rgb_transient;
  bool any() const { return rgb || acc || depth || depth_static || disp || beta || rgb_static || rgb_transient; }
};
hipError_t launch_composite_fine_backward_all(const float* raw, const float* z, size_t n_rays, int Nf, float beta_min, const MapGrads& g,
                                              float* graw, hipStream_t stream, const float* grad_raw_ext = nullptr);
hipError_t launch_ray_grad_reduce(const float* gpts, const float* z, const float* rays_d, size_t n_rays, int Nf,
                                  int derive_viewdirs, float* grad_o, float* grad_d, float* grad_viewdirs,
                                  hipStream_t stream, int accumulate = 0);
hipError_t launch_raygen_backward(int H, int W, float focal, const float* grad_o, const float* grad_d, float* grad_c2w,
                                  hipStream_t stream, int frames = 1);
hipError_t launch_bicubic_backward(const float* gout, int H, int W, int C, int UH, int UW, float* gin, hipStream_t stream, int frames = 1,
                                   bool nchw = false);
hipError_t launch_bicubic(const float* in, int H, int W, int C, int UH, int UW, float* out, hipStream_t stream, int frames = 1,
                          bool nchw = false);

}
```

### dfnet_amd/csrc/nerfh_layout.h

```cpp
#pragma once
#include <stdint.h>

#if defined(__HIPCC__) || defined(__HIP__)
#define DFN_HD __host__ __device__
#else
#define DFN_HD
#endif

namespace dfn {

constexpr int kWidth = 128;
constexpr int kLxyz = 10;
constexpr int kLdir = 4;
constexpr int kChXyz = 63, kChDir = 27;

enum LayerId {
  LY_L1 = 0, LY_L2, LY_L3, LY_L4, LY_L5, LY_L6, LY_L7, LY_L8,
  LY_FIN,
  LY_DIR,
  LY_RGB,
  LY_TE0,
  LY_TE1, LY_TE2, LY_TE3,
  LY_THEAD,
  LY_SIG,
  LY_DIRF,
  LY_TE0F,
  LY_COUNT
};

struct LayerShape { int slots; int mb; };

DFN_HD constexpr LayerShape layer_shape(int id, int W = kWidth) {
  return id == LY_L1 ? LayerShape{32, W / 32}
       : id == LY_L5 ? LayerShape{32 + W / 2, W / 32}
       : id <= LY_L8 ? LayerShape{W / 2, W / 32}
       : id == LY_FIN ? LayerShape{W / 2, W / 32 + 1}
       : id == LY_DIR ? LayerShape{W / 2, W / 64}
       : id == LY_RGB ? LayerShape{W / 4, 1}
       : id == LY_TE0 ? LayerShape{W / 2, W / 64}
       : id <= LY_TE3 ? LayerShape{W / 4, W / 64}
       : id == LY_THEAD ? LayerShape{W / 4, 1}
       : id == LY_DIRF || id == LY_TE0F ? LayerShape{W / 2, W / 64}
       : LayerShape{W / 2, 1};
}

constexpr int kCoarseSeq[] = {LY_L1, LY_L2, LY_L3, LY_L4, LY_L5, LY_L6, LY_L7, LY_L8, LY_SIG};
constexpr int kFineSeq[] = {LY_L1, LY_L2, LY_L3, LY_L4, LY_L5, LY_L6, LY_L7, LY_L8, LY_FIN,
                            LY_DIR, LY_RGB, LY_TE0, LY_TE1, LY_TE2, LY_TE3, LY_THEAD};
constexpr int kFineFoldSeq[] = {LY_L1, LY_L2, LY_L3, LY_L4, LY_L5, LY_L6, LY_L7, LY_L8, LY_SIG,
                                LY_DIRF, LY_RGB, LY_TE0F, LY_TE1, LY_TE2, LY_TE3, LY_THEAD};
static_assert(sizeof(kFineFoldSeq) == sizeof(kFineSeq), "the folded sequence has the layer count of the plain one");
constexpr int kCoarseGroup[] = {0, 1, 2, 3, 4, 5, 6, 7, 7};
constexpr int kFineGroup[] = {0, 1, 2, 3, 4, 5, 6, 7, 8, 9, 9, 10, 10, 10, 10, 10};
constexpr int kCoarseLayers = sizeof(kCoarseSeq) / sizeof(int);
constexpr int kFineLayers = sizeof(kFineSeq) / sizeof(int);

DFN_HD constexpr int hidden_feature(int h, int s) {
  return 32 * (s >> 4) + 4 * h + (s & 3) + 8 * ((s & 15) >> 2);
}
DFN_HD constexpr int mblock_row(int h, int r) { return (r & 3) + 8 * (r >> 2) + 4 * h; }

DFN_HD constexpr int pe_xyz_feature(int h, int s) {
  return s < 30 ? 3 + 6 * (5 * h + s / 6) + (s % 6) : (s == 30 ? (h ? 2 : 0) : (h ? -1 : 1));
}

DFN_HD constexpr int hidden_feature_m16(int g, int s) { return 32 * (s >> 3) + 16 * ((s & 7) >> 2) + 4 * g + (s & 3); }
DFN_HD constexpr int pe_xyz_feature_m16(int g, int s) {
  return s < 12 ? 3 + 6 * (2 * g + s / 6) + (s % 6)
       : (g == 3 ? (s < 15 ? s - 12 : -1)
                 : 3 + 6 * (8 + (2 * g + ((s - 12) >> 1)) / 3) + 3 * ((s - 12) & 1) + (2 * g + ((s - 12) >> 1)) % 3);
}
DFN_HD constexpr int head_row_m16(int i) {
  return ((i >> 2) & 3) < 2 ? (i & 3) + 8 * (i >> 4) : -1;
}

struct PrecF16 { static constexpr int kSlotsPerChunk = 8, kLaneBytes = 16; static constexpr bool kSplit = false, kM16 = false; };
struct PrecF32 { static constexpr int kSlotsPerChunk = 1, kLaneBytes = 4; static constexpr bool kSplit = false, kM16 = false; };
struct PrecX3 { static constexpr int kSlotsPerChunk = 8, kLaneBytes = 32; static constexpr bool kSplit = true, kM16 = false; };
constexpr float kX3ActScale = 16.f;
struct PrecX3M16 { static constexpr int kSlotsPerChunk = 8, kLaneBytes = 32; static constexpr bool kSplit = true, kM16 = true; };

constexpr int kVariants = 8;
constexpr int kFoldVariant = 5;
constexpr int kHalfVariant = 6;
constexpr int kResidentVariant = 7;
template <class P> DFN_HD constexpr int unit_mb(int variant) {
  return P::kSlotsPerChunk == 1 ? 1 : (P::kSplit ? 2 : (variant == 1 ? 2 : 8));
}
DFN_HD constexpr int variant_waves(int variant) { return variant == 0 ? 8 : 4; }
template <class P> DFN_HD constexpr int unit_mb_w256() { return (P::kSlotsPerChunk == 1 || P::kSplit) ? 1 : 2; }

constexpr uint32_t kPiece = 1024;

DFN_HD constexpr uint32_t align_piece(uint32_t b) { return (b + kPiece - 1) / kPiece * kPiece; }

template <class P>
DFN_HD constexpr uint32_t unit_bytes(int slots, int nmb, bool half = false) {
  return align_piece(uint32_t(nmb) * (slots / P::kSlotsPerChunk / (half ? 2 : 1)) * 64 * P::kLaneBytes + uint32_t(nmb) * 2 * 16 * 4);
}
DFN_HD constexpr int l5_unit_mb(int umb) { return umb >= 8 ? 2 : umb; }
template <class P> DFN_HD constexpr int l5_unit_mb_p(int umb) { return (P::kSplit && umb == 2) ? 1 : l5_unit_mb(umb); }
template <class P>
DFN_HD constexpr uint32_t max_unit_bytes(int umb, int W = kWidth) {
  const int m5 = l5_unit_mb_p<P>(umb), mbw = W / 32;
  const uint32_t a = unit_bytes<P>(32 + W / 2, m5 < mbw ? m5 : mbw), b = unit_bytes<P>(W / 2, umb < mbw + 1 ? umb : mbw + 1);
  const uint32_t g = umb >= 8 ? align_piece(44u * 64 * P::kLaneBytes + 9u * 128) : 0;
  return a > b ? (a > g ? a : g) : (b > g ? b : g);
}

constexpr int kCoarseResident[] = {LY_L1, LY_SIG};
constexpr int kFineResident[] = {LY_SIG, LY_RGB, LY_TE3, LY_THEAD};
DFN_HD constexpr int resident_count(bool fine) { return int(fine ? sizeof(kFineResident) : sizeof(kCoarseResident)) / int(sizeof(int)); }
DFN_HD constexpr int resident_at(bool fine, int i) { return fine ? kFineResident[i] : kCoarseResident[i]; }
DFN_HD constexpr bool layer_resident(bool fine, int id) {
  for (int i = 0; i < resident_count(fine); ++i)
    if (resident_at(fine, i) == id) return true;
  return false;
}
DFN_HD constexpr bool resident_half(int id) { return id == LY_SIG || id == LY_RGB || id == LY_THEAD; }
template <class P>
DFN_HD constexpr uint32_t resident_layer_bytes(int id) {
  const LayerShape sh = layer_shape(id);
  return uint32_t(sh.mb) * (uint32_t(sh.slots / P::kSlotsPerChunk / (resident_half(id) ? 2 : 1)) * 64 * P::kLaneBytes + 128u);
}
template <class P>
DFN_HD constexpr uint32_t resident_offset(bool fine, int id) {
  uint32_t off = 0;
  for (int i = 0; i < resident_count(fine) && resident_at(fine, i) != id; ++i) off += resident_layer_bytes<P>(resident_at(fine, i));
  return off;
}
template <class P> DFN_HD constexpr uint32_t resident_bytes(bool fine) { return align_piece(resident_offset<P>(fine, LY_COUNT)); }
constexpr uint32_t kLdsBytes = 163840;

enum BwdLayerId {
  BW_THEAD = 0,
  BW_TE3, BW_TE2, BW_TE1,
  BW_RGB,
  BW_FINCAT,
  BW_FIN,
  BW_L8, BW_L7, BW_L6,
  BW_L5,
  BW_L4, BW_L3, BW_L2,
  BW_L1,
  BW_COUNT
};
DFN_HD constexpr LayerShape bwd_layer_shape(int id) {
  return id == BW_THEAD || id == BW_RGB ? LayerShape{16, 2}
       : id <= BW_TE1 ? LayerShape{32, 2}
       : id == BW_FINCAT ? LayerShape{64, 5}
       : id == BW_FIN ? LayerShape{80, 4}
       : id == BW_L5 ? LayerShape{64, 6}
       : id == BW_L1 ? LayerShape{64, 2}
       : LayerShape{64, 4};
}
DFN_HD constexpr int mblock_half_of_row(int i) { return (i >> 2) & 1; }
DFN_HD constexpr int mblock_reg_of_row(int i) { return (i & 3) + 4 * (i >> 3); }
DFN_HD constexpr int pe_dir_feature(int h, int r) {
  return r < 12 ? 3 + 6 * (2 * h + r / 6) + (r % 6) : (h == 0 && r < 15 ? r - 12 : -1);
}
template <class P> DFN_HD constexpr int bwd_fwd_unit_mb() { return (P::kSlotsPerChunk == 8 && !P::kSplit) ? 8 : (P::kSplit ? 2 : 1); }
template <class P> DFN_HD constexpr int bwd_unit_mb() { return (P::kSlotsPerChunk == 8 && !P::kSplit) ? 8 : (P::kSplit ? 2 : 1); }
template <class P>
DFN_HD constexpr uint32_t bwd_max_unit_bytes() {
  constexpr bool whole = P::kSlotsPerChunk == 8 && !P::kSplit;
  constexpr int uf = bwd_fwd_unit_mb<P>(), ub = bwd_unit_mb<P>();
  const uint32_t a = unit_bytes<P>(96, whole ? 4 : uf);
  const uint32_t f5 = unit_bytes<P>(64, whole ? 5 : uf);
  const uint32_t b = unit_bytes<P>(64, whole ? 6 : ub), c = unit_bytes<P>(80, whole ? 4 : ub);
  const uint32_t m1 = a > f5 ? a : f5, m2 = b > c ? b : c;
  return m1 > m2 ? m1 : m2;
}

constexpr int kRayBiasFloats = 2 * 2 * 2 * 16;
DFN_HD constexpr int ray_bias_floats(int W) { return W; }
constexpr int kMaxWidth = 256;

}
```

### dfnet_amd/csrc/nerfh_mlp.hip

```cpp
#include <hip/hip_runtime.h>
#include <stdint.h>
#include <stdlib.h>

#include "nerfh_device.h"
#include "nerfh_kernels.h"
#include "nerfh_layout.h"
#include "mfma_frag.h"

#include "nerfh_mlp_core.h"
#include "nerfh_mask.h"

namespace dfn {

#ifdef DFN_MLP_MAPS_TU
constexpr bool kMapsTU = true;
#define DFN_LAUNCH_MLP launch_mlp_maps
#else
constexpr bool kMapsTU = false;
#define DFN_LAUNCH_MLP launch_mlp
#endif
#if defined(DFN_MLP_PTS_TU)
#if defined(DFN_MLP_HALF_TU)
#define DFN_FINE_KERNEL nerfh_fine_half_pts_kernel
#define DFN_COARSE_KERNEL nerfh_coarse_half_pts_kernel
constexpr bool kHalfHeads = true;
#elif defined(DFN_MLP_FOLD_TU)
#define DFN_FINE_KERNEL nerfh_fine_fold_pts_kernel
#define DFN_COARSE_KERNEL nerfh_coarse_fold_pts_kernel
constexpr bool kHalfHeads = false;
#else
#define DFN_FINE_KERNEL nerfh_fine_pts_kernel
#define DFN_COARSE_KERNEL nerfh_coarse_pts_kernel
constexpr bool kHalfHeads = false;
#endif
#elif defined(DFN_MLP_RES_TU)
#define DFN_FINE_KERNEL nerfh_fine_res_kernel
#define DFN_COARSE_KERNEL nerfh_coarse_res_kernel
constexpr bool kHalfHeads = true;
#elif defined(DFN_MLP_HALF_TU)
#define DFN_FINE_KERNEL nerfh_fine_half_kernel
#define DFN_COARSE_KERNEL nerfh_coarse_half_kernel
constexpr bool kHalfHeads = true;
#else
#ifdef DFN_MLP_FOLD_TU
#define DFN_FINE_KERNEL nerfh_fine_fold_kernel
#else
#define DFN_FINE_KERNEL nerfh_fine_kernel
#endif
#define DFN_COARSE_KERNEL nerfh_coarse_kernel
constexpr bool kHalfHeads = false;
#endif

#if defined(DFN_MLP_RES_TU)
#if !defined(DFN_MLP_HALF_TU) || defined(DFN_MLP_PTS_TU)
#error "the resident layers exist in the half-height render kernels"
#endif
constexpr bool kResident = true;
#define DFN_MLP_KARGS MlpResArgs
#else
constexpr bool kResident = false;
#define DFN_MLP_KARGS MlpArgs
#endif

template <class P, bool FAST> DFN_DEV float head_softplus(float v) { return FAST ? softplus_fast(v) : (P::kSplit ? softplus_hw(v) : softplus(v)); }
template <class P, bool FAST> DFN_DEV float head_sigmoid(float v) { return FAST ? sigmoid_fast(v) : (P::kSplit ? sigmoid_hw(v) : sigmoid(v)); }
template <class P, bool FAST> DFN_DEV float head_exp(float v) { return FAST ? __expf(v) : (P::kSplit ? exp_hw(v) : expf(v)); }

template <class P, int W> constexpr uint32_t ring_slots() { return 3; }
template <class P, int UMB, int WAVES, int NB, int W = kWidth> constexpr uint32_t lds_bytes() {
  return ring_slots<P, W>() * max_unit_bytes<P>(UMB, W) + WAVES * ((NB * 32 + 63) / 64) * 8 * 256;
}

template <class P, int UMB, int WAVES, int NB, int W, bool FINE> constexpr int res_base(int id) {
  return kResident && layer_resident(FINE, id) ? int(lds_bytes<P, UMB, WAVES, NB, W>() + resident_offset<P>(FINE, id)) : -1;
}
constexpr bool resident_set_supported(bool fine) {
  for (int i = 0; i < resident_count(fine); ++i) {
    const int id = resident_at(fine, i);
    const bool ok = id == LY_L1 || id == LY_SIG || (fine && (id == LY_RGB || (id >= LY_TE1 && id <= LY_THEAD)));
    if (!ok) return false;
  }
  return true;
}
static_assert(resident_set_supported(false) && resident_set_supported(true), "a resident layer the kernels stream");
static_assert(lds_bytes<PrecX3M16, unit_mb<PrecX3M16>(0), 8, 1>() + resident_bytes<PrecX3M16>(true) <= kLdsBytes &&
              lds_bytes<PrecX3M16, unit_mb<PrecX3M16>(0), 8, 1>() + resident_bytes<PrecX3M16>(false) <= kLdsBytes,
              "ring + input slots + resident layers must fit the LDS of a CU");

template <class P, int WAVES, int NB, int W> constexpr int mlp_min_blocks() {
  if (W > kWidth && (P::kSplit || P::kSlotsPerChunk == 1 || NB >= 2)) return 1;
  return WAVES * NB >= 12 ? (WAVES == 8 ? 2 : 1) : 2;
}

template <class P, bool FAST, int WAVES, int UMB, int NB, bool PIPE, int W = kWidth>
__global__ __launch_bounds__(WAVES * 64, (mlp_min_blocks<P, WAVES, NB, W>())) void DFN_COARSE_KERNEL(DFN_MLP_KARGS a) {
  extern __shared__ __attribute__((aligned(16))) char smem[];
  constexpr int PPT = WAVES * NB * 32;
  using F = typename FragOf<P>::type;
  Stager st;
  st.blob = a.blob; st.tab = a.tab; st.n_units = a.n_units; st.u = 0;
  st.waves = WAVES;
  st.dma_waves = a.dma_waves > 0 && a.dma_waves < WAVES ? a.dma_waves : WAVES;
  st.in_scale = a.in_scale;
  st.out_scale = 1.f / a.in_scale;
  st.lane_mul = 1.f;
  st.rmax = 0;
  st.t_sync = st.t_wait = 0;
  st.trace = nullptr;
  st.n_trace = 0;
  st.lane = threadIdx.x & 63;
  st.wave = __builtin_amdgcn_readfirstlane(threadIdx.x >> 6);
#ifdef DFN_TIMING
  const unsigned long long t_begin = __builtin_amdgcn_s_memtime();
  unsigned long long t_pro = 0;
  if (a.timing && blockIdx.x == 7) st.trace = a.timing + 8192 * 4 + st.wave * 192;
#endif
  const int p = st.lane & 31, h = st.lane >> 5;
  const long long n_pts = (long long)a.n_rays * a.n_samples;
  const long long n_tiles = (n_pts + PPT - 1) / PPT;
  long long tile = blockIdx.x;
  if (tile >= n_tiles) return;
#ifdef DFN_MLP_RES_TU
  stage_resident(st, smem, a.res_blob, resident_bytes<P>(false), lds_bytes<P, UMB, WAVES, NB, W>());
#endif
  stage_prime(st, smem, max_unit_bytes<P>(UMB, W), ring_slots<P, W>());
  for (; tile < n_tiles; tile += gridDim.x) {
    st.more = tile + gridDim.x < n_tiles;
    constexpr int LP = lane_pts<P>(NB);
    float x[LP][3];
    uint32_t pt[NB];
    const uint32_t npts = uint32_t(n_pts);
#pragma unroll
    for (int nb = 0; nb < NB; ++nb) pt[nb] = uint32_t(tile) * uint32_t(PPT) + st.wave * (NB * 32) + nb * 32 + p;
#pragma unroll
    for (int n = 0; n < LP; ++n) {
      const uint32_t pn = P::kM16 ? uint32_t(tile) * uint32_t(PPT) + st.wave * 32 + 16 * n + (st.lane & 15) : pt[n];
      const uint32_t q = pn < npts ? pn : npts - 1;
#ifdef DFN_MLP_PTS_TU
#pragma unroll
      for (int c = 0; c < 3; ++c) x[n][c] = a.rays_o[size_t(q) * 3 + c];
#else
      const uint32_t ray = q / uint32_t(a.n_samples);
      const int i = int(q - ray * uint32_t(a.n_samples));
      const float z = coarse_z_at(i, a.n_samples, a.near, a.far, a.lindisp != 0);
#pragma unroll
      for (int c = 0; c < 3; ++c)
        x[n][c] = add_rn(a.rays_o[ray * 3 + c], mul_rn(a.rays_d[ray * 3 + c], z));
#endif
    }
    constexpr bool CY = PIPE && P::kSlotsPerChunk == 8, MERGE = UMB >= 8;
    F hid[NB][chunks_of<P>(W / 2)];
    f32x16 carry[NB];
    constexpr int R_L1 = res_base<P, UMB, WAVES, NB, W, false>(LY_L1), R_SIG = res_base<P, UMB, WAVES, NB, W, false>(LY_SIG);
    trunk<P, UMB, PIPE, FAST, NB, W, NoTrunkHook, R_L1>(st, smem, x, hid, carry);
    f32x16 head[NB];
    F dummy[NB][chunks_of<P>(16)];
    const float* const norb[LP] = {};
    layer<P, UMB, PIPE, NB, chunks_of<P>(W / 2), 0, false, true, false, !MERGE && R_SIG < 0, (CY ? 6 : -1), true, false, false, false, true, kHalfHeads, R_SIG>(st, smem, hid, dummy, head, norb, carry);
#pragma unroll
    for (int nb = 0; nb < NB; ++nb)
      if (h == 0 && pt[nb] < npts) a.out[pt[nb]] = head_softplus<P, FAST>(head[nb][0]);
  }
  range_report<P>(st.rmax, a.status);
}

template <class P, bool FAST, int WAVES, int UMB, int NB, bool PIPE, int W = kWidth, bool MASKS = false, bool MAPS = false>
__global__ __launch_bounds__(WAVES * 64, (mlp_min_blocks<P, WAVES, NB, W>())) void DFN_FINE_KERNEL(DFN_MLP_KARGS a) {
  static_assert(!MASKS || (P::kSplit && !P::kM16 && NB == 1 && WAVES == 8 && W == kWidth), "the sign masks follow the gradient kernel's tile geometry");
  static_assert(!MAPS || (!MASKS && W == kWidth && NB <= 2), "the maps flavour exists where the fused compositing does");
  extern __shared__ __attribute__((aligned(16))) char smem[];
  constexpr int PPT = WAVES * NB * 32;
  constexpr int HC = chunks_of<P>(W / 2), QC = chunks_of<P>(W / 4);
  constexpr int MBW = W / 32, MBQ = W / 64;
  constexpr uint32_t USTRIDE = max_unit_bytes<P>(UMB, W);
  constexpr int PF_ROUNDS = (NB * 32 + 63) / 64;
  constexpr int LP = lane_pts<P>(NB);
  constexpr bool NOBETA = kHalfHeads && !MAPS;
  constexpr int R_L1 = res_base<P, UMB, WAVES, NB, W, true>(LY_L1);
  constexpr int R_SIG = res_base<P, UMB, WAVES, NB, W, true>(LY_SIG), R_RGB = res_base<P, UMB, WAVES, NB, W, true>(LY_RGB),
                R_TE1 = res_base<P, UMB, WAVES, NB, W, true>(LY_TE1), R_TE2 = res_base<P, UMB, WAVES, NB, W, true>(LY_TE2),
                R_TE3 = res_base<P, UMB, WAVES, NB, W, true>(LY_TE3), R_THEAD = res_base<P, UMB, WAVES, NB, W, true>(LY_THEAD);
  using F = typename FragOf<P>::type;
  Stager st;
  st.blob = a.blob; st.tab = a.tab; st.n_units = a.n_units; st.u = 0;
  st.waves = WAVES;
  st.dma_waves = a.dma_waves > 0 && a.dma_waves < WAVES ? a.dma_waves : WAVES;
  st.in_scale = a.in_scale;
  st.out_scale = 1.f / a.in_scale;
  st.lane_mul = 1.f;
  st.rmax = 0;
  st.t_sync = st.t_wait = 0;
  st.trace = nullptr;
  st.n_trace = 0;
  st.lane = threadIdx.x & 63;
  st.wave = __builtin_amdgcn_readfirstlane(threadIdx.x >> 6);
#ifdef DFN_TIMING
  const unsigned long long t_begin = __builtin_amdgcn_s_memtime();
  unsigned long long t_pro = 0;
  if (a.timing && blockIdx.x == 7) st.trace = a.timing + 8192 * 4 + st.wave * 192;
#endif
  const int p = st.lane & 31, h = st.lane >> 5;
  const long long n_pts = (long long)a.n_rays * a.n_samples;
  const long long n_tiles = (n_pts + PPT - 1) / PPT;
  long long tile = blockIdx.x;
  if (tile >= n_tiles) return;
#ifdef DFN_MLP_RES_TU
  static_assert(!MAPS && !MASKS, "the resident set is the plain fused fine kernel's");
  stage_resident(st, smem, a.res_blob, resident_bytes<P>(true), lds_bytes<P, UMB, WAVES, NB, W>());
#endif
  stage_prime(st, smem, USTRIDE, ring_slots<P, W>());
#ifdef DFN_MLP_PTS_TU
  float xin[LP][3];
#else
  float zin[LP], znext[LP], oin[LP][3], din[LP][3];
#endif
  uint32_t pt[LP], ray_of[LP];
  const uint32_t npts = uint32_t(n_pts);
  auto tile_coords = [&](long long t) {
    uint32_t lp = st.lane;
    asm volatile("" : "+v"(lp));
#pragma unroll
    for (int nb = 0; nb < LP; ++nb) {
      pt[nb] = uint32_t(t) * uint32_t(PPT) + st.wave * (NB * 32) + (P::kM16 ? 16 * nb + (lp & 15) : nb * 32 + (lp & 31));
      const uint32_t q = pt[nb] < npts ? pt[nb] : npts - 1;
      ray_of[nb] = q / uint32_t(a.n_samples);
    }
  };
  tile_coords(tile);
#pragma unroll
  for (int nb = 0; nb < LP; ++nb) {
    const uint32_t q = pt[nb] < npts ? pt[nb] : npts - 1;
#ifdef DFN_MLP_PTS_TU
#pragma unroll
    for (int c = 0; c < 3; ++c) xin[nb][c] = a.rays_o[size_t(q) * 3 + c];
#else
    zin[nb] = a.z[q];
    znext[nb] = a.z[q + 1 < npts ? q + 1 : q];
#pragma unroll
    for (int c = 0; c < 3; ++c) { oin[nb][c] = a.rays_o[ray_of[nb] * 3 + c]; din[nb][c] = a.rays_d[ray_of[nb] * 3 + c]; }
#endif
  }
  for (; tile < n_tiles; tile += gridDim.x) {
    st.more = tile + gridDim.x < n_tiles;
    float x[LP][3];
    uint32_t pt_cur[LP], ray_cur[LP];
#pragma unroll
    for (int nb = 0; nb < LP; ++nb) {
      pt_cur[nb] = pt[nb];
      ray_cur[nb] = ray_of[nb];
#pragma unroll
#ifdef DFN_MLP_PTS_TU
      for (int c = 0; c < 3; ++c) x[nb][c] = xin[nb][c];
#else
      for (int c = 0; c < 3; ++c) x[nb][c] = add_rn(oin[nb][c], mul_rn(din[nb][c], zin[nb]));
#endif
    }
    auto ray_table = [&](const float* (&rb)[LP], int half_table) {
#pragma unroll
      for (int nb = 0; nb < LP; ++nb) {
        uint32_t r = ray_cur[nb];
        asm volatile("" : "+v"(r));
        rb[nb] = a.ray_bias + (size_t)r * ray_bias_floats(W) + half_table * (ray_bias_floats(W) / 2);
      }
    };
    const float* const norb[LP] = {};
    F hid[NB][HC];
#ifdef DFN_TIMING
    {
      const unsigned long long c0 = __builtin_amdgcn_s_memtime();
      float keep = 0.f;
      for (int nb = 0; nb < LP; ++nb) keep += x[nb][0] + x[nb][1] + x[nb][2];
      asm volatile("" ::"v"(keep));
      t_pro += __builtin_amdgcn_s_memtime() - c0;
    }
#endif
    constexpr bool CY = PIPE && P::kSlotsPerChunk == 8, MERGE = UMB >= 8;
    f32x16 carry[NB];
    [[maybe_unused]] uint32_t* mwords = nullptr;
    if constexpr (MASKS) mwords = a.masks + (size_t(tile) * WAVES + st.wave) * (kBwdMaskWords * 64) + st.lane;
    auto sign128 = [&](int l, F (&h)[HC]) {
      if constexpr (MASKS) {
        uint32_t m[2];
        relu_mask<P, HC>(h, m);
        mwords[(2 * l) * 64] = m[0];
        mwords[(2 * l + 1) * 64] = m[1];
      }
    };
    auto sign64 = [&](int word, F (&h)[QC]) {
      if constexpr (MASKS) {
        uint32_t m[1];
        relu_mask<P, QC>(h, m);
        mwords[word * 64] = m[0];
      }
    };
    if constexpr (MASKS) trunk<P, UMB, PIPE, FAST, NB, W>(st, smem, x, hid, carry, sign128);
    else trunk<P, UMB, PIPE, FAST, NB, W, NoTrunkHook, R_L1>(st, smem, x, hid, carry);
    f32x16 head[NB];
#ifdef DFN_MLP_FOLD_TU
    static_assert(P::kM16 && !MASKS && W == kWidth, "the folded tail exists for the split-f16 16x16x32 render kernel");
    F (&fin)[NB][HC] = hid;
    {
      F dummy[NB][chunks_of<P>(16)];
      layer<P, UMB, PIPE, NB, HC, 0, false, true, false, R_SIG < 0, (CY ? 6 : -1), true, false, false, false, true, kHalfHeads, R_SIG>(st, smem, hid, dummy, head, norb, carry);
    }
#else
    F fin[NB][HC];
    layer<P, UMB, PIPE, NB, HC, MBW, false, true, false, true, (CY ? 6 : -1), true, false>(st, smem, hid, fin, head, norb, carry);
#endif
    sign128(7, hid[0]);
    float o[NB][9];
#pragma unroll
    for (int nb = 0; nb < NB; ++nb) o[nb][3] = head_softplus<P, FAST>(head[nb][0]);
    {
      F de[NB][QC], dummy[NB][chunks_of<P>(16)];
      const float* rb_dir[LP];
      ray_table(rb_dir, 0);
      layer<P, UMB, PIPE, NB, HC, MBQ, true, false, true, true, -1, true, CY>(st, smem, fin, de, head, rb_dir, carry);
      layer<P, UMB, PIPE, NB, QC, 0, false, true, false, !MERGE && R_RGB < 0, (CY ? 2 : -1), true, false, false, false, true, kHalfHeads, R_RGB>(st, smem, de, dummy, head, norb, carry);
      sign64(16, de[0]);
#pragma unroll
      for (int nb = 0; nb < NB; ++nb)
#pragma unroll
        for (int c = 0; c < 3; ++c) o[nb][c] = head_sigmoid<P, FAST>(head[nb][c]);
    }
    {
      F t0[NB][QC], t1[NB][QC], dummy[NB][chunks_of<P>(16)];
      const float* rb_tr[LP];
      ray_table(rb_tr, 1);
      layer<P, UMB, PIPE, NB, HC, MBQ, true, false, true, true, -1, true, CY>(st, smem, fin, t0, head, rb_tr, carry);
      if (st.more) {
        const uint32_t base = uint32_t(tile + gridDim.x) * uint32_t(PPT) + st.wave * (NB * 32);
        char* slot = smem + ring_slots<P, W>() * USTRIDE + st.wave * (PF_ROUNDS * 8 * 256);
#pragma unroll
        for (int r = 0; r < PF_ROUNDS; ++r) {
          const uint32_t ptn = base + r * 64 + st.lane;
          const uint32_t q = ptn < npts ? ptn : npts - 1;
#ifdef DFN_MLP_PTS_TU
#pragma unroll
          for (int c = 0; c < 3; ++c) lds_dma_b32(a.rays_o + size_t(q) * 3 + c, slot + (r * 8 + c) * 256);
#else
          const uint32_t ray = q / uint32_t(a.n_samples);
          lds_dma_b32(a.z + q, slot + (r * 8) * 256);
          lds_dma_b32(a.z + (q + 1 < npts ? q + 1 : q), slot + (r * 8 + 7) * 256);
#pragma unroll
          for (int c = 0; c < 3; ++c) {
            lds_dma_b32(a.rays_o + ray * 3 + c, slot + (r * 8 + 1 + c) * 256);
            lds_dma_b32(a.rays_d + ray * 3 + c, slot + (r * 8 + 4 + c) * 256);
          }
#endif
        }
      }
      layer<P, UMB, PIPE, NB, QC, MBQ, true, false, false, !MERGE && R_TE1 < 0, (CY ? 2 : -1), true, CY, false, false, true, false, R_TE1>(st, smem, t0, t1, head, norb, carry);
      sign64(17, t0[0]);
      layer<P, UMB, PIPE, NB, QC, MBQ, true, false, false, !MERGE && R_TE2 < 0, (CY ? 2 : -1), true, CY, false, false, true, false, R_TE2>(st, smem, t1, t0, head, norb, carry);
      sign64(18, t1[0]);
      layer<P, UMB, PIPE, NB, QC, MBQ, true, false, false, !MERGE && R_TE3 < 0, (CY ? 2 : -1), true, CY, false, false, true, false, R_TE3>(st, smem, t0, t1, head, norb, carry);
      sign64(19, t0[0]);
      layer<P, UMB, PIPE, NB, QC, 0, false, true, false, !MERGE && R_THEAD < 0, (CY ? 2 : -1), true, false, false, false, true, NOBETA, R_THEAD>(st, smem, t1, dummy, head, norb, carry);
      sign64(20, t1[0]);
#pragma unroll
      for (int nb = 0; nb < NB; ++nb) {
#pragma unroll
        for (int c = 0; c < 3; ++c) o[nb][4 + c] = head_sigmoid<P, FAST>(head[nb][c]);
        o[nb][7] = head_softplus<P, FAST>(head[nb][3]);
        if constexpr (NOBETA) o[nb][8] = 0.f;
        else o[nb][8] = head_softplus<P, FAST>(head[nb][4]);
      }
    }
#ifdef DFN_MLP_PTS_TU
    uint32_t pt_own[NB];
#pragma unroll
    for (int nb = 0; nb < NB; ++nb) {
      if constexpr (P::kM16) pt_own[nb] = (st.lane & 16) != 0 ? pt_cur[1] : pt_cur[0];
      else pt_own[nb] = pt_cur[nb];
    }
    {
#else
    uint32_t pt_own[NB], ray_own[NB];
    float z_own[NB], zn_own[NB];
#pragma unroll
    for (int nb = 0; nb < NB; ++nb) {
      if constexpr (P::kM16) {
        const bool n1 = (st.lane & 16) != 0;
        pt_own[nb] = n1 ? pt_cur[1] : pt_cur[0];
        ray_own[nb] = n1 ? ray_cur[1] : ray_cur[0];
        z_own[nb] = n1 ? zin[1] : zin[0];
        zn_own[nb] = n1 ? znext[1] : znext[0];
      } else {
        pt_own[nb] = pt_cur[nb]; ray_own[nb] = ray_cur[nb]; z_own[nb] = zin[nb]; zn_own[nb] = znext[nb];
      }
    }
    if (a.partial) {
      const bool live = h == 0;
      float Pj = 1.f, Ps = 1.f;
      float s_rgb[3] = {0.f, 0.f, 0.f}, s_acc = 0.f, s_dso = 0.f, s_dj = 0.f, s_beta = 0.f;
      [[maybe_unused]] float s_rs[3] = {0.f, 0.f, 0.f}, s_rt[3] = {0.f, 0.f, 0.f};
#pragma unroll
      for (int nb = 0; nb < NB; ++nb) {
        const uint32_t smp = pt_own[nb] - ray_own[nb] * uint32_t(a.n_samples);
        const float delta = smp + 1 == uint32_t(a.n_samples) ? 1e2f : sub_rn(zn_own[nb], z_own[nb]);
        const float sg_s = o[nb][3], sg_t = o[nb][7];
        const float as = live ? sub_rn(1.f, head_exp<P, FAST>(-mul_rn(delta, sg_s))) : 0.f;
        const float at = live ? sub_rn(1.f, head_exp<P, FAST>(-mul_rn(delta, sg_t))) : 0.f;
        const float aj = live ? sub_rn(1.f, head_exp<P, FAST>(-mul_rn(delta, add_rn(sg_s, sg_t)))) : 0.f;
        const float ij = scan32_prod(1.f - aj), is = scan32_prod(1.f - as);
        const float ej = lane_shr1(ij, 1.f), es = lane_shr1(is, 1.f);
        const float Tj = Pj * ej, Ts = Ps * es;
        const float ws = as * Tj, wt = at * Tj, wj = aj * Tj;
#pragma unroll
        for (int c = 0; c < 3; ++c) s_rgb[c] += live ? ws * o[nb][c] + wt * o[nb][4 + c] : 0.f;
        s_acc += wj;
        s_dso += as * Ts * z_own[nb];
        s_dj += wj * z_own[nb];
        if constexpr (!NOBETA) s_beta += live ? wt * o[nb][8] : 0.f;
        if constexpr (MAPS) {
          float wt_m = wt;
          asm volatile("" : "+v"(wt_m));
          const float wso = as * Ts;
#pragma unroll
          for (int c = 0; c < 3; ++c) {
            s_rs[c] += live ? wso * o[nb][c] : 0.f;
            s_rt[c] += live ? wt_m * o[nb][4 + c] : 0.f;
          }
        }
        Pj *= read_lane31(ij);
        Ps *= read_lane31(is);
      }
#pragma unroll
      for (int c = 0; c < 3; ++c) s_rgb[c] = read_lane31(scan32_sum(s_rgb[c]));
      s_acc = read_lane31(scan32_sum(s_acc)); s_dso = read_lane31(scan32_sum(s_dso));
      s_dj = read_lane31(scan32_sum(s_dj));
      if constexpr (!NOBETA) s_beta = read_lane31(scan32_sum(s_beta));
      if constexpr (MAPS) {
#pragma unroll
        for (int c = 0; c < 3; ++c) { s_rs[c] = read_lane31(scan32_sum(s_rs[c])); s_rt[c] = read_lane31(scan32_sum(s_rt[c])); }
      }
      if (st.lane == 0 && pt_own[0] < npts) {
        constexpr int REC = MAPS ? kMapsRecFloats : 12;
        f32x4* dst = reinterpret_cast<f32x4*>(a.partial + (size_t)(pt_own[0] / uint32_t(NB * 32)) * REC);
        dst[0] = f32x4{s_rgb[0], s_rgb[1], s_rgb[2], s_acc};
        dst[1] = f32x4{s_dso, s_dj, s_beta, Pj};
        if constexpr (MAPS) {
          dst[2] = f32x4{Ps, s_rs[0], s_rs[1], s_rs[2]};
          dst[3] = f32x4{s_rt[0], s_rt[1], s_rt[2], 0.f};
        } else {
          dst[2] = f32x4{Ps, 0.f, 0.f, 0.f};
        }
      }
    } else {
#endif
#pragma unroll
      for (int nb = 0; nb < NB; ++nb)
        if (h == 0 && pt_own[nb] < npts) {
          float* dst = a.out + (size_t)pt_own[nb] * 9;
#pragma unroll
          for (int c = 0; c < 9; ++c) dst[c] = o[nb][c];
        }
    }
    if (st.more) {
      __builtin_amdgcn_s_waitcnt(0x0F70);
      asm volatile("" ::: "memory");
      tile_coords(tile + gridDim.x);
      const char* slot = smem + ring_slots<P, W>() * USTRIDE + st.wave * (PF_ROUNDS * 8 * 256);
#pragma unroll
      for (int nb = 0; nb < LP; ++nb) {
        int loc = P::kM16 ? 16 * nb + (st.lane & 15) : nb * 32 + p;
        asm volatile("" : "+v"(loc));
        const int r = loc >> 6, l = loc & 63;
        const float* f = reinterpret_cast<const float*>(slot + r * 8 * 256) + l;
#ifdef DFN_MLP_PTS_TU
#pragma unroll
        for (int c = 0; c < 3; ++c) xin[nb][c] = f[c * 64];
#else
        zin[nb] = f[0];
        znext[nb] = f[7 * 64];
#pragma unroll
        for (int c = 0; c < 3; ++c) { oin[nb][c] = f[(1 + c) * 64]; din[nb][c] = f[(4 + c) * 64]; }
#endif
      }
    }
  }
  range_report<P>(st.rmax, a.status);
#ifdef DFN_TIMING
  if (a.timing && st.lane == 0) {
    unsigned long long* t = a.timing + (blockIdx.x * WAVES + st.wave) * 4;
    t[0] = __builtin_amdgcn_s_memtime() - t_begin;
    t[1] = st.t_wait;
    t[2] = st.t_sync;
    t[3] = t_pro;
  }
#endif
}

#if defined(DFN_MLP_PTS_TU)
template <class P, bool FAST, int WAVES, int UMB, int NB, bool PIPE, int W, bool FINE>
static hipError_t launch_pts_one(const MlpArgs& a, int n_cu, hipStream_t stream) {
  constexpr int PPT = WAVES * NB * 32;
  const long long n_pts = (long long)a.n_rays * a.n_samples;
  if (n_pts <= 0) return hipSuccess;
  if (n_pts >= (1LL << 31)) return hipErrorInvalidValue;
  if (a.masks || a.partial || !a.rays_o || !a.out) return hipErrorInvalidValue;
  const long long n_tiles = (n_pts + PPT - 1) / PPT;
  const int grid = int(n_tiles < n_cu ? n_tiles : n_cu);
  const uint32_t lds = lds_bytes<P, UMB, WAVES, NB, W>();
  void (*kern)(MlpArgs) = nullptr;
  if constexpr (FINE) kern = DFN_FINE_KERNEL<P, FAST, WAVES, UMB, NB, PIPE, W>;
  else kern = DFN_COARSE_KERNEL<P, FAST, WAVES, UMB, NB, PIPE, W>;
  static bool attr_done = false;
  if (!attr_done) {
    hipError_t e = hipFuncSetAttribute(reinterpret_cast<const void*>(kern), hipFuncAttributeMaxDynamicSharedMemorySize, int(lds));
    if (e != hipSuccess) return e;
    attr_done = true;
  }
  MlpArgs b = a;
  if (b.dma_waves == 0) {
    static int env = -1;
    if (env < 0) { const char* e = getenv("DFN_DMA_WAVES"); env = e ? atoi(e) : 0; }
    b.dma_waves = env > 0 ? env : (WAVES == 8 ? 4 : WAVES);
  }
  hipLaunchKernelGGL(kern, dim3(grid), dim3(WAVES * 64), lds, stream, b);
  return hipGetLastError();
}
#if defined(DFN_MLP_HALF_TU)
hipError_t launch_mlp_pts_half(const MlpArgs& a, int n_cu, hipStream_t stream) {
  return launch_pts_one<PrecX3M16, false, 8, unit_mb<PrecX3M16>(0), 1, true, kWidth, false>(a, n_cu, stream);
}
#elif defined(DFN_MLP_FOLD_TU)
hipError_t launch_mlp_pts_fold(const MlpArgs& a, int n_cu, hipStream_t stream) {
  return launch_pts_one<PrecX3M16, false, 8, unit_mb<PrecX3M16>(0), 1, true, kWidth, true>(a, n_cu, stream);
}
#else
hipError_t launch_mlp_pts(bool fine, int prec, const MlpArgs& a, int n_cu, hipStream_t stream, int width) {
  if (width == 256) {
    if (prec == 0) {
      return fine ? launch_pts_one<PrecF16, true, 8, unit_mb_w256<PrecF16>(), 1, false, 256, true>(a, n_cu, stream)
                  : launch_pts_one<PrecF16, true, 8, unit_mb_w256<PrecF16>(), 1, false, 256, false>(a, n_cu, stream);
    }
    if (prec == 2) {
      return fine ? launch_pts_one<PrecX3, false, 4, unit_mb_w256<PrecX3>(), 1, false, 256, true>(a, n_cu, stream)
                  : launch_pts_one<PrecX3, false, 4, unit_mb_w256<PrecX3>(), 1, false, 256, false>(a, n_cu, stream);
    }
    return fine ? launch_pts_one<PrecF32, false, 4, unit_mb_w256<PrecF32>(), 1, false, 256, true>(a, n_cu, stream)
                : launch_pts_one<PrecF32, false, 4, unit_mb_w256<PrecF32>(), 1, false, 256, false>(a, n_cu, stream);
  }
  if (width != kWidth) return hipErrorInvalidValue;
  if (prec == 0) {
    return fine ? launch_pts_one<PrecF16, true, 8, 8, 2, true, kWidth, true>(a, n_cu, stream)
                : launch_pts_one<PrecF16, true, 8, 8, 2, true, kWidth, false>(a, n_cu, stream);
  }
  if (prec == 2) return hipErrorInvalidValue;
  return fine ? launch_pts_one<PrecF32, false, 8, 1, 1, false, kWidth, true>(a, n_cu, stream)
              : launch_pts_one<PrecF32, false, 8, 1, 1, false, kWidth, false>(a, n_cu, stream);
}
#endif
#elif defined(DFN_MLP_RES_TU)
hipError_t launch_mlp_res(bool fine, const MlpResArgs& a, int n_cu, hipStream_t stream) {
  using P = PrecX3M16;
  constexpr int WAVES = 8, UMB = unit_mb<P>(0), NB = 1, PPT = WAVES * NB * 32;
  const long long n_pts = (long long)a.n_rays * a.n_samples;
  if (n_pts <= 0) return hipSuccess;
  if (n_pts >= (1LL << 31)) return hipErrorInvalidValue;
  if (a.masks || (fine && !a.partial)) return hipErrorInvalidValue;
  if (!a.res_blob || a.res_bytes != resident_bytes<P>(fine)) return hipErrorInvalidValue;
  const long long n_tiles = (n_pts + PPT - 1) / PPT;
  const int grid = int(n_tiles < n_cu ? n_tiles : n_cu);
  const uint32_t lds = lds_bytes<P, UMB, WAVES, NB>() + resident_bytes<P>(fine);
  void (*kern)(MlpResArgs) = fine ? nerfh_fine_res_kernel<P, false, WAVES, UMB, NB, true> : nerfh_coarse_res_kernel<P, false, WAVES, UMB, NB, true>;
  static bool attr_done[2] = {false, false};
  if (!attr_done[fine]) {
    hipError_t e = hipFuncSetAttribute(reinterpret_cast<const void*>(kern), hipFuncAttributeMaxDynamicSharedMemorySize, int(lds));
    if (e != hipSuccess) return e;
    attr_done[fine] = true;
  }
  MlpResArgs b = a;
  if (b.dma_waves == 0) {
    static int env = -1;
    if (env < 0) { const char* e = getenv("DFN_DMA_WAVES"); env = e ? atoi(e) : 0; }
    b.dma_waves = env > 0 ? env : 4;
  }
  hipLaunchKernelGGL(kern, dim3(grid), dim3(WAVES * 64), lds, stream, b);
  return hipGetLastError();
}
#elif defined(DFN_MLP_HALF_TU)
hipError_t launch_mlp_half(bool fine, bool maps, const MlpArgs& a, int n_cu, hipStream_t stream) {
  using P = PrecX3M16;
  constexpr int WAVES = 8, UMB = unit_mb<P>(0), NB = 1, PPT = WAVES * NB * 32;
  const long long n_pts = (long long)a.n_rays * a.n_samples;
  if (n_pts <= 0) return hipSuccess;
  if (n_pts >= (1LL << 31)) return hipErrorInvalidValue;
  if (a.masks || (fine && !a.partial) || (maps && !fine)) return hipErrorInvalidValue;
  const long long n_tiles = (n_pts + PPT - 1) / PPT;
  const int grid = int(n_tiles < n_cu ? n_tiles : n_cu);
  const uint32_t lds = lds_bytes<P, UMB, WAVES, NB>();
  const int slot = fine ? (maps ? 2 : 1) : 0;
  void (*kern)(MlpArgs) = !fine ? nerfh_coarse_half_kernel<P, false, WAVES, UMB, NB, true>
                          : maps ? nerfh_fine_half_kernel<P, false, WAVES, UMB, NB, true, kWidth, false, true>
                                 : nerfh_fine_half_kernel<P, false, WAVES, UMB, NB, true>;
  static bool attr_done[3] = {false, false, false};
  if (!attr_done[slot]) {
    hipError_t e = hipFuncSetAttribute(reinterpret_cast<const void*>(kern), hipFuncAttributeMaxDynamicSharedMemorySize, int(lds));
    if (e != hipSuccess) return e;
    attr_done[slot] = true;
  }
  MlpArgs b = a;
  if (b.dma_waves == 0) {
    static int env = -1;
    if (env < 0) { const char* e = getenv("DFN_DMA_WAVES"); env = e ? atoi(e) : 0; }
    b.dma_waves = env > 0 ? env : 4;
  }
  hipLaunchKernelGGL(kern, dim3(grid), dim3(WAVES * 64), lds, stream, b);
  return hipGetLastError();
}
#elif defined(DFN_MLP_FOLD_TU)
hipError_t launch_mlp_fold(bool maps, const MlpArgs& a, int n_cu, hipStream_t stream) {
  using P = PrecX3M16;
  constexpr int WAVES = 8, UMB = unit_mb<P>(0), NB = 1, PPT = WAVES * NB * 32;
  const long long n_pts = (long long)a.n_rays * a.n_samples;
  if (n_pts <= 0) return hipSuccess;
  if (n_pts >= (1LL << 31)) return hipErrorInvalidValue;
  if (a.masks || (maps && !a.partial)) return hipErrorInvalidValue;
  const long long n_tiles = (n_pts + PPT - 1) / PPT;
  const int grid = int(n_tiles < n_cu ? n_tiles : n_cu);
  const uint32_t lds = lds_bytes<P, UMB, WAVES, NB>();
  void (*kern)(MlpArgs) = maps ? nerfh_fine_fold_kernel<P, false, WAVES, UMB, NB, true, kWidth, false, true>
                               : nerfh_fine_fold_kernel<P, false, WAVES, UMB, NB, true>;
  static bool attr_done[2] = {false, false};
  if (!attr_done[maps]) {
    hipError_t e = hipFuncSetAttribute(reinterpret_cast<const void*>(kern), hipFuncAttributeMaxDynamicSharedMemorySize, int(lds));
    if (e != hipSuccess) return e;
    attr_done[maps] = true;
  }
  MlpArgs b = a;
  if (b.dma_waves == 0) {
    static int env = -1;
    if (env < 0) { const char* e = getenv("DFN_DMA_WAVES"); env = e ? atoi(e) : 0; }
    b.dma_waves = env > 0 ? env : 4;
  }
  hipLaunchKernelGGL(kern, dim3(grid), dim3(WAVES * 64), lds, stream, b);
  return hipGetLastError();
}
#else
template <class P, bool FAST, int WAVES, int UMB, int NB, int WG_PER_CU, bool PIPE, int W = kWidth>
static hipError_t launch_one(bool fine, const MlpArgs& a, int n_cu, hipStream_t stream) {
  constexpr int PPT = WAVES * NB * 32;
  const long long n_pts = (long long)a.n_rays * a.n_samples;
  if (n_pts <= 0) return hipSuccess;
  if (n_pts >= (1LL << 31)) return hipErrorInvalidValue;
  const long long n_tiles = (n_pts + PPT - 1) / PPT;
  const long long slots = (long long)n_cu * WG_PER_CU;
  const int grid = int(n_tiles < slots ? n_tiles : slots);
  const uint32_t lds = lds_bytes<P, UMB, WAVES, NB, W>();
  void (*kern)(MlpArgs) = nullptr;
  int slot = fine ? 1 : 0;
  if constexpr (kMapsTU) {
    if constexpr (W == kWidth && NB <= 2) {
      if (!fine || !a.partial || a.masks) return hipErrorInvalidValue;
      kern = nerfh_fine_kernel<P, FAST, WAVES, UMB, NB, PIPE, W, false, true>;
    } else {
      return hipErrorInvalidValue;
    }
  } else {
    kern = fine ? nerfh_fine_kernel<P, FAST, WAVES, UMB, NB, PIPE, W> : nerfh_coarse_kernel<P, FAST, WAVES, UMB, NB, PIPE, W>;
    if constexpr (P::kSplit && !P::kM16 && NB == 1 && WAVES == 8 && W == kWidth && PIPE) {
      if (fine && a.masks) { kern = nerfh_fine_kernel<P, FAST, WAVES, UMB, NB, PIPE, W, true>; slot = 2; }
    } else if (a.masks) return hipErrorInvalidValue;
  }
  static bool attr_done[3] = {false, false, false};
  if (!attr_done[slot]) {
    hipError_t e = hipFuncSetAttribute(reinterpret_cast<const void*>(kern),
                                       hipFuncAttributeMaxDynamicSharedMemorySize, int(lds));
    if (e != hipSuccess) return e;
    attr_done[slot] = true;
  }
  MlpArgs b = a;
  if (b.dma_waves == 0) {
    static int env = -1;
    if (env < 0) { const char* e = getenv("DFN_DMA_WAVES"); env = e ? atoi(e) : 0; }
    b.dma_waves = env > 0 ? env : (WAVES == 8 ? 4 : WAVES);
  }
  hipLaunchKernelGGL(kern, dim3(grid), dim3(WAVES * 64), lds, stream, b);
  return hipGetLastError();
}

hipError_t DFN_LAUNCH_MLP(bool fine, int prec, int variant, const MlpArgs& a, int n_cu, hipStream_t stream, int width) {
  if (width == 256) {
    if (prec == 0) {
      return launch_one<PrecF16, true, 8, unit_mb_w256<PrecF16>(), 1, 1, false, 256>(fine, a, n_cu, stream);
    }
    if (prec == 2) return launch_one<PrecX3, false, 4, unit_mb_w256<PrecX3>(), 1, 1, false, 256>(fine, a, n_cu, stream);
    return launch_one<PrecF32, false, 4, unit_mb_w256<PrecF32>(), 1, 1, false, 256>(fine, a, n_cu, stream);
  }
  if (width != kWidth) return hipErrorInvalidValue;
  if (variant == 4 && prec != 2) variant = 0;
  if (prec == 0) {
    if (variant == 0) return launch_one<PrecF16, true, 8, 8, 2, 1, true>(fine, a, n_cu, stream);
    if (variant == 1) return launch_one<PrecF16, true, 4, 2, 2, 1, true>(fine, a, n_cu, stream);
    if (variant == 2) return launch_one<PrecF16, true, 4, 8, 3, 1, true>(fine, a, n_cu, stream);
    return launch_one<PrecF16, true, 8, 8, 2, 1, false>(fine, a, n_cu, stream);
  }
  if (prec == 2) {
    if (variant == 3) return launch_one<PrecX3, false, 8, unit_mb<PrecX3>(0), 1, 1, false>(fine, a, n_cu, stream);
    if (variant == 4) return launch_one<PrecX3M16, false, 8, unit_mb<PrecX3M16>(0), 1, 1, true>(fine, a, n_cu, stream);
    return launch_one<PrecX3, false, 8, unit_mb<PrecX3>(0), 1, 1, true>(fine, a, n_cu, stream);
  }
  if (variant == 1) return launch_one<PrecF32, false, 4, 1, 1, 1, false>(fine, a, n_cu, stream);
  return launch_one<PrecF32, false, 8, 1, 1, 1, false>(fine, a, n_cu, stream);
}
#endif

}
```

### dfnet_amd/csrc/nerfh_mlp_core.h

```cpp
#pragma once
#include <hip/hip_runtime.h>
#include <stdint.h>

#include "mfma_frag.h"
#include "nerfh_device.h"
#include "nerfh_kernels.h"
#include "nerfh_layout.h"

#ifndef DFN_PF
#define DFN_PF 3
#endif

namespace dfn {

template <class P> constexpr int chunks_of(int slots) { return slots / P::kSlotsPerChunk; }
template <class P> constexpr int lane_pts(int NB) { return P::kM16 ? 2 : NB; }
template <class P> DFN_HD constexpr int x3_chunk(int i) { return P::kM16 ? (i >> 1) & 1 : i >> 2; }
template <class P> DFN_HD constexpr int x3_pos(int i) { return P::kM16 ? 4 * (i >> 2) + 2 * (i & 1) : 2 * (i & 3); }

template <class P, int KC>
DFN_DEV void set_slot(typename FragOf<P>::type (&arr)[KC], int s, float v) {
  if constexpr (P::kSplit) {
    _Float16 hi, lo;
    x3_split(v, hi, lo);
    arr[s >> 3].hi[s & 7] = hi;
    arr[s >> 3].lo[s & 7] = lo;
  } else if constexpr (P::kSlotsPerChunk == 8) arr[s >> 3][s & 7] = (_Float16)v;
  else arr[s] = v;
}

struct Stager {
  const char* blob;
  const uint32_t* tab;
  int n_units;
  int u;
  uint32_t slot;
  uint32_t ring;
  uint32_t ustride;
  int lane, wave, waves;
  int dma_waves;
  uint32_t ubase, uoff;
  uint32_t pf_off, pf_size;
  unsigned long long t_sync, t_wait, t_last;
  unsigned long long* trace;
  int n_trace;
  bool more;
  float in_scale, out_scale;
  float lane_mul;
  uint32_t rmax;
};

DFN_DEV uint32_t pk_max_u16(uint32_t a, uint32_t b) {
  uint32_t r;
  asm("v_pk_max_u16 %0, %1, %2" : "=v"(r) : "v"(a), "v"(b));
  return r;
}
DFN_DEV void range_track(uint32_t& rmax, uint32_t packed, bool nonneg) {
  rmax = pk_max_u16(rmax, nonneg ? packed : (packed & 0x7fff7fffu));
}
template <class P>
DFN_DEV void range_report(uint32_t rmax, int* status) {
  if constexpr (P::kSlotsPerChunk == 8) {
    const uint32_t thr = P::kSplit ? 0x7bffu : 0x7c00u;
    if (status && ((rmax & 0xffffu) >= thr || (rmax >> 16) >= thr)) atomicOr(status, P::kSplit ? 2 : 1);
  }
}

DFN_DEV void lds_dma_b128(const void* gptr, const char* lds_dst) {
  const uint32_t off = (uint32_t)(size_t)DFN_LDS_PTR(lds_dst);
  asm volatile("s_mov_b32 m0, %1\n\tglobal_load_lds_dwordx4 %0, off" ::"v"(gptr), "s"(off) : "memory");
}
DFN_DEV void lds_dma_b32(const void* gptr, const char* lds_dst) {
  const uint32_t off = (uint32_t)(size_t)DFN_LDS_PTR(lds_dst);
  asm volatile("s_mov_b32 m0, %1\n\tglobal_load_lds_dword %0, off" ::"v"(gptr), "s"(off) : "memory");
}

DFN_DEV void stage_issue_at(const Stager& st, char* smem, uint32_t off, uint32_t size, uint32_t lds_off) {
  const char* src = st.blob + off + st.lane * 16;
  if (st.wave >= st.dma_waves) return;
  for (uint32_t p = st.wave * kPiece; p < size; p += st.dma_waves * kPiece) lds_dma_b128(src + p, smem + lds_off + p);
}
typedef const uint32_t __attribute__((address_space(4))) const_u32;
DFN_DEV uint32_t tab_entry(const Stager& st, int i) {
  return reinterpret_cast<const_u32*>(reinterpret_cast<uint64_t>(st.tab))[i];
}
DFN_DEV void stage_issue(const Stager& st, char* smem, int unit, uint32_t lds_off) {
  stage_issue_at(st, smem, tab_entry(st, 2 * unit), tab_entry(st, 2 * unit + 1), lds_off);
}

DFN_DEV void stage_prime(Stager& st, char* smem, uint32_t unit_stride, uint32_t ring = 3) {
  st.slot = 0; st.ring = ring; st.ustride = unit_stride;
  st.u = 0;
  stage_issue(st, smem, 0, 0);
  stage_issue(st, smem, st.n_units > 1 ? 1 : 0, unit_stride);
  const int n2 = st.n_units > 2 ? 2 : 0;
  st.pf_off = tab_entry(st, 2 * n2);
  st.pf_size = tab_entry(st, 2 * n2 + 1);
  __builtin_amdgcn_s_waitcnt(0x0F70);
  asm volatile("" ::: "memory");
  __syncthreads();
}

DFN_DEV void stage_resident(const Stager& st, char* smem, const char* res_blob, uint32_t bytes, uint32_t lds_off) {
  const char* src = res_blob + st.lane * 16;
  if (st.wave >= st.dma_waves) return;
  for (uint32_t p = st.wave * kPiece; p < bytes; p += st.dma_waves * kPiece) lds_dma_b128(src + p, smem + lds_off + p);
}

DFN_DEV uint32_t open_unit(Stager& st) {
  const uint32_t cur = st.slot * st.ustride;
  st.slot = st.slot + 1 == st.ring ? 0u : st.slot + 1;
  int nxt = st.u + 1;
  if (nxt == st.n_units) nxt = 0;
  st.u = nxt;
  return cur;
}

DFN_DEV void mid_sync(Stager& st, char* smem) {
#ifdef DFN_TIMING
  const unsigned long long c0 = __builtin_amdgcn_s_memtime();
#endif
  __builtin_amdgcn_s_waitcnt(0x0F70);
  asm volatile("" ::: "memory");
#ifdef DFN_TIMING
  const unsigned long long c1 = __builtin_amdgcn_s_memtime();
#endif
  int n2 = st.u + 1;
  bool next_tile = st.u == 0;
  if (n2 >= st.n_units) { n2 -= st.n_units; next_tile = true; }
  const uint32_t dst = (st.slot + 1 == st.ring ? 0u : st.slot + 1) * st.ustride;
  __builtin_amdgcn_s_barrier();
  asm volatile("" ::: "memory");
#ifdef DFN_TIMING
  const unsigned long long c2 = __builtin_amdgcn_s_memtime();
  st.t_wait += c1 - c0;
  st.t_sync += c2 - c1;
  if (st.trace && st.n_trace < 96 && st.lane == 0) {
    st.trace[2 * st.n_trace] = c0;
    st.trace[2 * st.n_trace + 1] = c2;
  }
  ++st.n_trace;
#endif
  if (!next_tile || st.more) stage_issue_at(st, smem, st.pf_off, st.pf_size, dst);
  {
    int n3 = n2 + 1;
    if (n3 >= st.n_units) n3 -= st.n_units;
    st.pf_off = tab_entry(st, 2 * n3);
    st.pf_size = tab_entry(st, 2 * n3 + 1);
  }
}

template <class P>
DFN_DEV typename FragOf<P>::type load_afrag(const char* p);

template <class P, int NB, int KC>
DFN_DEV void mblock_mma(const char* smem, uint32_t wb, const typename FragOf<P>::type (&Bin)[NB][KC],
                        f32x16 (&acc)[NB]) {
  using F = typename FragOf<P>::type;
#pragma unroll
  for (int kc = 0; kc < KC; ++kc) {
    const F a = load_afrag<P>(smem + wb + kc * 64 * P::kLaneBytes);
#pragma unroll
    for (int nb = 0; nb < NB; ++nb) acc[nb] = mfma<P>(a, Bin[nb][kc], acc[nb]);
  }
}

template <class P>
DFN_DEV typename FragOf<P>::type load_afrag(const char* p) {
  if constexpr (P::kSplit) {
    half8x2 f;
    f.hi = *reinterpret_cast<const half8*>(p);
    f.lo = *reinterpret_cast<const half8*>(p + 1024);
    return f;
  } else {
    return *reinterpret_cast<const typename FragOf<P>::type*>(p);
  }
}

DFN_DEV f32x16 load16(const float* p) {
  const f32x4* q = reinterpret_cast<const f32x4*>(p);
  f32x4 a = q[0], b = q[1], c = q[2], d = q[3];
  f32x16 r;
#pragma unroll
  for (int i = 0; i < 4; ++i) { r[i] = a[i]; r[4 + i] = b[i]; r[8 + i] = c[i]; r[12 + i] = d[i]; }
  return r;
}
DFN_DEV f32x16 load_bias_m16(const float* p) {
  const f32x4* q = reinterpret_cast<const f32x4*>(p);
  const f32x4 a = q[0], b = q[1];
  f32x16 r = {};
#pragma unroll
  for (int i = 0; i < 4; ++i) { r[i] = a[i]; r[4 + i] = b[i]; }
  return r;
}
DFN_DEV f32x16 load_raybias_m16(const float* const (&rb)[2], int mb, int g) {
  f32x16 r;
#pragma unroll
  for (int nb = 0; nb < 2; ++nb) {
    const f32x4* q = reinterpret_cast<const f32x4*>(rb[nb] + mb * 32 + (g & 1) * 16 + 4 * (g >> 1));
    const f32x4 a = q[0], b = q[2];
#pragma unroll
    for (int i = 0; i < 4; ++i) { r[4 * nb + i] = a[i]; r[8 + 4 * nb + i] = b[i]; }
  }
  return r;
}
DFN_DEV f32x4 sub4(const f32x16& v, int o) { return f32x4{v[o], v[o + 1], v[o + 2], v[o + 3]}; }
DFN_DEV void put4(f32x16& v, int o, const f32x4& x) { v[o] = x[0]; v[o + 1] = x[1]; v[o + 2] = x[2]; v[o + 3] = x[3]; }

template <class P, bool RELU, int OC>
DFN_DEV void store_hidden(const f32x16& acc, typename FragOf<P>::type (&out)[OC], int mb, float oscale, uint32_t& rmax) {
  if constexpr (P::kSplit) {
    typedef __fp16 pk2 __attribute__((ext_vector_type(2)));
    const float os = oscale * kX3ActScale;
#pragma unroll
    for (int c = 0; c < 2; ++c)
#pragma unroll
      for (int j = 0; j < 8; j += 2) {
        float x0 = acc[8 * c + j] * os, x1 = acc[8 * c + j + 1] * os;
        if (RELU) { x0 = fmaxf(x0, 0.f); x1 = fmaxf(x1, 0.f); }
        const pk2 h = __builtin_amdgcn_cvt_pkrtz(x0, x1);
        const uint32_t hb = __builtin_bit_cast(uint32_t, h);
        float r0, r1;
        asm("v_fma_mix_f32 %0, %1, -1.0, %2 op_sel_hi:[1,0,0]" : "=v"(r0) : "v"(hb), "v"(x0));
        asm("v_fma_mix_f32 %0, %1, -1.0, %2 op_sel:[1,0,0] op_sel_hi:[1,0,0]" : "=v"(r1) : "v"(hb), "v"(x1));
        const pk2 l = __builtin_amdgcn_cvt_pkrtz(r0, r1);
        range_track(rmax, hb, RELU);
        const int oc = 2 * mb + x3_chunk<P>(4 * c + j / 2), oj = x3_pos<P>(4 * c + j / 2);
        out[oc].hi[oj] = (_Float16)h[0]; out[oc].hi[oj + 1] = (_Float16)h[1];
        out[oc].lo[oj] = (_Float16)l[0]; out[oc].lo[oj + 1] = (_Float16)l[1];
      }
  } else if constexpr (P::kSlotsPerChunk == 8) {
#pragma unroll
    for (int c = 0; c < 2; ++c) {
      half8 v;
#pragma unroll
      for (int j = 0; j < 8; ++j) v[j] = (_Float16)acc[8 * c + j];
      if (RELU) {
        const half8 zero = {0, 0, 0, 0, 0, 0, 0, 0};
        v = __builtin_elementwise_max(v, zero);
      }
      {
        typedef uint32_t u32x4 __attribute__((ext_vector_type(4)));
        u32x4 w = __builtin_bit_cast(u32x4, v);
        if (!RELU) w &= 0x7fff7fffu;
        rmax = pk_max_u16(rmax, pk_max_u16(pk_max_u16(w[0], w[1]), pk_max_u16(w[2], w[3])));
      }
      out[2 * mb + c] = v;
    }
  } else {
#pragma unroll
    for (int r = 0; r < 16; ++r) out[16 * mb + r] = RELU ? fmaxf(acc[r], 0.f) : acc[r];
  }
}

template <class P, bool RELU, int OC>
DFN_DEV void store_hidden(const f32x16& acc, typename FragOf<P>::type (&out)[OC], int mb, float oscale = 1.f) {
  uint32_t unused = 0;
  store_hidden<P, RELU>(acc, out, mb, oscale, unused);
}

template <class P, bool RELU, int OC>
DFN_DEV void store_hidden_piece(const f32x16& acc, typename FragOf<P>::type (&out)[OC], int mb, int i, float oscale, uint32_t& rmax) {
  if constexpr (P::kSplit) {
    typedef _Float16 half2v __attribute__((ext_vector_type(2)));
    const int c = i >> 2, j = (i & 3) * 2;
    uint32_t hb, lb;
    float t0, t1;
    if (RELU)
      asm volatile("v_mul_f32 %2, %4, %6\n\tv_mul_f32 %3, %5, %6\n\tv_max_f32 %2, %2, 0\n\tv_max_f32 %3, %3, 0\n\t"
                   "v_cvt_pkrtz_f16_f32 %0, %2, %3\n\t"
                   "v_fma_mix_f32 %2, %0, -1.0, %2 op_sel_hi:[1,0,0]\n\t"
                   "v_fma_mix_f32 %3, %0, -1.0, %3 op_sel:[1,0,0] op_sel_hi:[1,0,0]\n\t"
                   "v_cvt_pkrtz_f16_f32 %1, %2, %3"
                   : "=&v"(hb), "=&v"(lb), "=&v"(t0), "=&v"(t1) : "v"(acc[8 * c + j]), "v"(acc[8 * c + j + 1]), "v"(oscale));
    else
      asm volatile("v_mul_f32 %2, %4, %6\n\tv_mul_f32 %3, %5, %6\n\t"
                   "v_cvt_pkrtz_f16_f32 %0, %2, %3\n\t"
                   "v_fma_mix_f32 %2, %0, -1.0, %2 op_sel_hi:[1,0,0]\n\t"
                   "v_fma_mix_f32 %3, %0, -1.0, %3 op_sel:[1,0,0] op_sel_hi:[1,0,0]\n\t"
                   "v_cvt_pkrtz_f16_f32 %1, %2, %3"
                   : "=&v"(hb), "=&v"(lb), "=&v"(t0), "=&v"(t1) : "v"(acc[8 * c + j]), "v"(acc[8 * c + j + 1]), "v"(oscale));
    if (RELU) asm volatile("v_pk_max_u16 %0, %0, %1" : "+v"(rmax) : "v"(hb));
    else range_track(rmax, hb, false);
    const half2v hv = __builtin_bit_cast(half2v, hb), lv = __builtin_bit_cast(half2v, lb);
    const int oc = 2 * mb + x3_chunk<P>(i), oj = x3_pos<P>(i);
    out[oc].hi[oj] = hv[0]; out[oc].hi[oj + 1] = hv[1];
    out[oc].lo[oj] = lv[0]; out[oc].lo[oj + 1] = lv[1];
  } else if constexpr (P::kSlotsPerChunk == 8) {
    typedef _Float16 half2v __attribute__((ext_vector_type(2)));
    const int c = i >> 2, j = i & 3;
    uint32_t bits;
    if (RELU)
      asm volatile("v_cvt_pk_f16_f32 %0, %1, %2\n\tv_pk_max_f16 %0, %0, 0" : "=v"(bits) : "v"(acc[8 * c + 2 * j]), "v"(acc[8 * c + 2 * j + 1]));
    else
      asm volatile("v_cvt_pk_f16_f32 %0, %1, %2" : "=v"(bits) : "v"(acc[8 * c + 2 * j]), "v"(acc[8 * c + 2 * j + 1]));
    if (RELU) asm volatile("v_pk_max_u16 %0, %0, %1" : "+v"(rmax) : "v"(bits));
    else range_track(rmax, bits, false);
    const half2v v = __builtin_bit_cast(half2v, bits);
    out[2 * mb + c][2 * j] = v[0];
    out[2 * mb + c][2 * j + 1] = v[1];
  } else {
    float x0 = acc[2 * i], x1 = acc[2 * i + 1];
    asm volatile("" : "+v"(x0), "+v"(x1));
    x0 = RELU ? fmaxf(x0, 0.f) : x0;
    x1 = RELU ? fmaxf(x1, 0.f) : x1;
    asm volatile("" : "+v"(x0), "+v"(x1));
    out[16 * mb + 2 * i] = x0;
    out[16 * mb + 2 * i + 1] = x1;
  }
}

struct X3Piece {
  uint32_t hb, hs, lb;
  float t0, t1;
  template <bool RELU>
  DFN_DEV void A(const f32x16& acc, int i) {
    const int c = i >> 2, j = (i & 3) * 2;
    if (RELU) asm volatile("v_max_f32 %0, %2, 0\n\tv_max_f32 %1, %3, 0" : "=&v"(t0), "=&v"(t1) : "v"(acc[8 * c + j]), "v"(acc[8 * c + j + 1]));
    else asm volatile("v_mov_b32 %0, %2\n\tv_mov_b32 %1, %3" : "=&v"(t0), "=&v"(t1) : "v"(acc[8 * c + j]), "v"(acc[8 * c + j + 1]));
  }
  DFN_DEV void B(float s, uint32_t s2) {
    asm volatile("v_cvt_pkrtz_f16_f32 %0, %2, %3\n\t"
                 "v_pk_mul_f16 %1, %0, %5\n\t"
                 "v_fma_mix_f32 %2, %2, %4, -%1 op_sel_hi:[0,0,1]\n\t"
                 "v_fma_mix_f32 %3, %3, %4, -%1 op_sel:[0,0,1] op_sel_hi:[0,0,1]"
                 : "=&v"(hb), "=&v"(hs), "+v"(t0), "+v"(t1) : "v"(s), "v"(s2));
  }
  DFN_DEV void B1(uint32_t s2) {
    asm volatile("v_cvt_pkrtz_f16_f32 %0, %2, %3\n\t"
                 "v_pk_mul_f16 %1, %0, %4"
                 : "=&v"(hb), "=&v"(hs) : "v"(t0), "v"(t1), "v"(s2));
  }
  DFN_DEV void B2(float s) {
    asm volatile("v_fma_mix_f32 %0, %0, %2, -%3 op_sel_hi:[0,0,1]\n\t"
                 "v_fma_mix_f32 %1, %1, %2, -%3 op_sel:[0,0,1] op_sel_hi:[0,0,1]"
                 : "+v"(t0), "+v"(t1) : "v"(s), "v"(hs));
  }
  template <bool RELU, class P = PrecX3, int OC>
  DFN_DEV void C(half8x2 (&out)[OC], int mb, int i, uint32_t& rmax) {
    typedef _Float16 half2v __attribute__((ext_vector_type(2)));
    const int c = x3_chunk<P>(i), j = x3_pos<P>(i);
    asm volatile("v_cvt_pkrtz_f16_f32 %0, %1, %2" : "=v"(lb) : "v"(t0), "v"(t1));
    if (RELU) asm volatile("v_pk_max_u16 %0, %0, %1" : "+v"(rmax) : "v"(hb));
    else range_track(rmax, hb, false);
    const half2v hv = __builtin_bit_cast(half2v, hs), lv = __builtin_bit_cast(half2v, lb);
    out[2 * mb + c].hi[j] = hv[0]; out[2 * mb + c].hi[j + 1] = hv[1];
    out[2 * mb + c].lo[j] = lv[0]; out[2 * mb + c].lo[j + 1] = lv[1];
  }
};

template <class P, int UMB, bool PIPE, int NB, int KC, int MB, bool RELU, bool EXTRA, bool RAYBIAS, bool NEWUNIT,
          int CIN, bool CIN_RELU, bool COUT, bool NOBIAS = false, bool SCALE_FIRST = false, bool TRACK = true, bool HALF = false, int RES = -1>
DFN_DEV void layer(Stager& st, char* smem, typename FragOf<P>::type (&Bin)[NB][KC],
                   typename FragOf<P>::type (&Bout)[NB][(MB ? MB : 1) * chunks_of<P>(16)],
                   f32x16 (&head)[NB], const float* const (&raybias)[lane_pts<P>(NB)], f32x16 (&carry)[NB]) {
  using F = typename FragOf<P>::type;
  static_assert(!P::kM16 || (PIPE && NB == 1 && !SCALE_FIRST), "the 16x16x32 split-f16 layer is the pipelined one-point-block form");
  constexpr int TOT = MB + (EXTRA ? 1 : 0);
  constexpr int PF = P::kSplit ? 2 : (P::kSlotsPerChunk == 8 ? DFN_PF : 4);
  constexpr uint32_t FB = 64 * P::kLaneBytes;
  constexpr int PPK = (8 * NB + KC - 1) / KC;
  constexpr int PPKI = CIN > 0 ? (8 * NB + CIN - 1) / CIN : 0;
  static_assert(CIN < 0 || (PIPE && P::kSlotsPerChunk == 8 && CIN > 0 && CIN + 1 < KC + 1), "carry-in needs the pipelined f16 path");
  static_assert(!COUT || (PIPE && MB >= 1 && !EXTRA), "carry-out needs a regular last M-block");
  static_assert(NEWUNIT || UMB >= TOT || RES >= 0, "a layer that continues a unit must fit in it");
  static_assert(RES < 0 || (!NEWUNIT && P::kM16), "a resident layer opens no staging unit");
  static_assert(!HALF || (P::kM16 && EXTRA && MB == 0 && !RAYBIAS && KC % 2 == 0 && CIN >= 2 && CIN % 2 == 0 && CIN + 2 == KC),
                "a half-height block is a PrecX3M16 head layer whose last 32-K chunk is the carried-in M-block");
  constexpr int KCL = HALF ? KC / 2 : KC;
  constexpr int CINL = HALF ? CIN / 2 : CIN;
  constexpr bool TAILBLK = HALF && CINL == 1;
  const int h = st.lane >> 5, g16 = st.lane >> 4;
  uint32_t rmax_sink = 0;
  uint32_t& rmax_ = TRACK ? st.rmax : rmax_sink;
  const float pscale = P::kSplit ? st.out_scale * st.lane_mul * kX3ActScale : 1.f;
  uint32_t pscale2 = 0;
  if constexpr (P::kSplit) asm("v_cvt_pkrtz_f16_f32 %0, %1, %1" : "=v"(pscale2) : "v"(pscale));
  constexpr bool RB_ALL = RAYBIAS && NB <= 2;
  f32x16 rb[RB_ALL ? TOT : 1][NB];
  if (RB_ALL) {
#pragma unroll
    for (int mb = 0; mb < TOT; ++mb)
#pragma unroll
      for (int nb = 0; nb < NB; ++nb) {
        if constexpr (P::kM16) rb[mb][nb] = load_raybias_m16(raybias, mb, g16);
        else rb[mb][nb] = load16(raybias[nb] + (mb * 2 + h) * 16);
        if constexpr (P::kSplit) rb[mb][nb] *= st.in_scale;
      }
  }
  f32x16 pend[PIPE ? NB : 1];
#pragma unroll
  for (int u0 = 0; u0 < TOT; u0 += UMB) {
    const int nmb = (TOT - u0) < UMB ? (TOT - u0) : UMB;
    const int nt = nmb * KCL;
    uint32_t ub;
    if (NEWUNIT) { ub = open_unit(st); st.ubase = ub; st.uoff = 0; }
    else if constexpr (RES >= 0) ub = uint32_t(RES) + u0 * (KCL * FB + 128);
    else ub = st.ubase + st.uoff;
    if constexpr (RES < 0) st.uoff += nmb * KCL * FB + nmb * 128;
    const char* wl = smem + ub + st.lane * (P::kSplit ? 16 : P::kLaneBytes);
    const char* bl = smem + ub + nmb * KCL * FB + (P::kM16 ? g16 * 32 : h * 64);
    F a[PF];
#define DFN_AFRAG(t) load_afrag<P>(wl + (t) * FB)
#pragma unroll
    for (int t = 0; t < PF; ++t)
      if (t < nt) a[t] = DFN_AFRAG(t);
    f32x16 bias = {};
    auto load_bias = [&](const char* p) {
      if constexpr (P::kM16) return load_bias_m16(reinterpret_cast<const float*>(p));
      else return load16(reinterpret_cast<const float*>(p));
    };
    if (!RAYBIAS && !NOBIAS) bias = load_bias(bl);
#pragma unroll
    for (int lm = 0; lm < UMB; ++lm) {
      if (lm < nmb) {
        const int mb = u0 + lm;
        f32x16 acc[NB];
        if constexpr (HALF) {
#pragma unroll
          for (int nb = 0; nb < NB; ++nb) acc[nb] = f32x16{};
        }
        f32x16 bias_next = bias;
        if (RAYBIAS) {
#pragma unroll
          for (int nb = 0; nb < NB; ++nb) {
            if constexpr (P::kM16) acc[nb] = RB_ALL ? rb[RB_ALL ? mb : 0][nb] : load_raybias_m16(raybias, mb, g16);
            else acc[nb] = RB_ALL ? rb[RB_ALL ? mb : 0][nb] : load16(raybias[nb] + (mb * 2 + h) * 16);
            if constexpr (P::kSplit && !RB_ALL) acc[nb] *= st.in_scale;
          }
        }
#pragma unroll
        for (int kc = 0; kc < KCL; ++kc) {
          const int t = lm * KCL + kc;
          if (NEWUNIT && lm == 0 && kc == (KCL > 1 ? KCL / 2 : 0)) mid_sync(st, smem);
          const F cur = a[t % PF];
          if (t + PF < nt) a[t % PF] = DFN_AFRAG(t + PF);
          if (kc == (PIPE ? KCL / 2 : 0) && !RAYBIAS && !NOBIAS && lm + 1 < nmb) bias_next = load_bias(bl + (lm + 1) * 128);
          __builtin_amdgcn_sched_barrier(0);
          if constexpr (P::kSplit && PIPE && NB == 1 && !SCALE_FIRST) {
            constexpr int PPKI_ = TAILBLK ? 4 : ((CIN > 0) ? (8 * NB + CINL - 1) / CINL : 1), PPK_ = (8 * NB + KCL - 1) / KCL;
            constexpr int NPMAX = PPKI_ > PPK_ ? PPKI_ : PPK_;
            static_assert(!HALF || NPMAX <= 4, "half 1's pieces must not start in the first chunk");
            const bool from_carry = CIN > 0 && mb == 0 && kc < CINL, from_pend = mb >= 1;
            const int np = from_carry ? PPKI_ : (from_pend ? PPK_ : 0), base = kc * np;
            X3Piece pc[NPMAX];
            const bool late = kc == 0;
#define DFN_X3_PARTS_A \
            _Pragma("unroll") for (int q = 0; q < NPMAX; ++q) \
              if (q < np && base + q < 8) { \
                if (from_carry) pc[q].template A<CIN_RELU>(carry[0], base + q); \
                else pc[q].template A<RELU>(pend[0], base + q); \
              }
#define DFN_X3_PARTS_B \
            _Pragma("unroll") for (int q = 0; q < NPMAX; ++q) \
              if (q < np && base + q < 8) pc[q].B(pscale, pscale2);
            if constexpr (P::kM16) {
              const int ms = HALF ? 0 : (kc & 1), bc = HALF ? 2 * kc : 2 * (kc >> 1);
              f32x4 c0, c1;
              if (kc < (HALF ? 1 : 2) && !RAYBIAS) { c0 = sub4(bias, 4 * ms); c1 = c0; }
              else { c0 = sub4(acc[0], 8 * ms); c1 = sub4(acc[0], 8 * ms + 4); }
#define DFN_X3_PARTS(...) \
              _Pragma("unroll") for (int q = 0; q < NPMAX; ++q) \
                if (q < np && base + q < 8) { __VA_ARGS__; }
              c0 = __builtin_amdgcn_mfma_f32_16x16x32_f16(cur.hi, Bin[0][bc].hi, c0, 0, 0, 0);
              c1 = __builtin_amdgcn_mfma_f32_16x16x32_f16(cur.hi, Bin[0][bc + 1].hi, c1, 0, 0, 0);
              __builtin_amdgcn_sched_barrier(0);
              DFN_X3_PARTS_A
              __builtin_amdgcn_sched_barrier(0);
              c0 = __builtin_amdgcn_mfma_f32_16x16x32_f16(cur.hi, Bin[0][bc].lo, c0, 0, 0, 0);
              __builtin_amdgcn_sched_barrier(0);
              DFN_X3_PARTS(pc[q].B1(pscale2))
              __builtin_amdgcn_sched_barrier(0);
              c1 = __builtin_amdgcn_mfma_f32_16x16x32_f16(cur.hi, Bin[0][bc + 1].lo, c1, 0, 0, 0);
              __builtin_amdgcn_sched_barrier(0);
              DFN_X3_PARTS(pc[q].B2(pscale))
              __builtin_amdgcn_sched_barrier(0);
              c0 = __builtin_amdgcn_mfma_f32_16x16x32_f16(cur.lo, Bin[0][bc].hi, c0, 0, 0, 0);
              __builtin_amdgcn_sched_barrier(0);
              DFN_X3_PARTS(if (from_carry) pc[q].template C<CIN_RELU, P>(Bin[0], CIN / 2, base + q, rmax_);
                           else pc[q].template C<RELU, P>(Bout[0], mb - 1, base + q, rmax_))
              __builtin_amdgcn_sched_barrier(0);
              c1 = __builtin_amdgcn_mfma_f32_16x16x32_f16(cur.lo, Bin[0][bc + 1].hi, c1, 0, 0, 0);
#undef DFN_X3_PARTS
              put4(acc[0], 8 * ms, c0);
              put4(acc[0], 8 * ms + 4, c1);
              if constexpr (TAILBLK) {
                if (from_carry) {
                  __builtin_amdgcn_sched_barrier(0);
                  asm volatile("s_nop 7");
                  X3Piece tp[4];
#pragma unroll
                  for (int q = 0; q < 4; ++q) tp[q].template A<CIN_RELU>(carry[0], 4 + q);
#pragma unroll
                  for (int q = 0; q < 4; ++q) tp[q].B1(pscale2);
#pragma unroll
                  for (int q = 0; q < 4; ++q) tp[q].B2(pscale);
#pragma unroll
                  for (int q = 0; q < 4; ++q) tp[q].template C<CIN_RELU, P>(Bin[0], CIN / 2, 4 + q, rmax_);
                }
              }
              if (from_carry && kc == CINL - 1) asm volatile("s_nop 3");
              __builtin_amdgcn_sched_barrier(0);
              continue;
            }
            f32x16 c0 = (kc == 0) ? (RAYBIAS ? acc[0] : bias) : acc[0];
            c0 = __builtin_amdgcn_mfma_f32_32x32x16_f16(cur.hi, Bin[0][kc].hi, c0, 0, 0, 0);
            __builtin_amdgcn_sched_barrier(0);
            if (!late) { DFN_X3_PARTS_A }
            __builtin_amdgcn_sched_barrier(0);
            c0 = __builtin_amdgcn_mfma_f32_32x32x16_f16(cur.hi, Bin[0][kc].lo, c0, 0, 0, 0);
            __builtin_amdgcn_sched_barrier(0);
            if (!late) { DFN_X3_PARTS_B }
            __builtin_amdgcn_sched_barrier(0);
            c0 = __builtin_amdgcn_mfma_f32_32x32x16_f16(cur.lo, Bin[0][kc].hi, c0, 0, 0, 0);
            __builtin_amdgcn_sched_barrier(0);
            if (late) { DFN_X3_PARTS_A DFN_X3_PARTS_B }
#undef DFN_X3_PARTS_A
#undef DFN_X3_PARTS_B
#pragma unroll
            for (int q = 0; q < NPMAX; ++q)
              if (q < np && base + q < 8) {
                if (from_carry) pc[q].template C<CIN_RELU>(Bin[0], CIN / 2, base + q, rmax_);
                else pc[q].template C<RELU>(Bout[0], mb - 1, base + q, rmax_);
              }
            acc[0] = c0;
            if (from_carry && kc == CIN - 1) asm volatile("s_nop 3");
            __builtin_amdgcn_sched_barrier(0);
            continue;
          }
          if constexpr (!P::kM16) {
#pragma unroll
          for (int nb = 0; nb < NB; ++nb) {
            if (kc == 0) acc[nb] = mfma<P>(cur, Bin[nb][0], RAYBIAS ? acc[nb] : bias);
            else acc[nb] = mfma<P>(cur, Bin[nb][kc], acc[nb]);
          }
          }
          if (CIN > 0 && mb == 0 && kc < CIN) {
#pragma unroll
            for (int q = 0; q < PPKI; ++q) {
              const int piece = kc * PPKI + q;
              if (piece < 8 * NB) store_hidden_piece<P, CIN_RELU>(carry[piece >> 3], Bin[piece >> 3], CIN / 2, piece & 7, pscale, rmax_);
            }
            if (kc == CIN - 1) asm volatile("s_nop 3");
          }
          if (PIPE && mb >= 1) {
#pragma unroll
            for (int q = 0; q < PPK; ++q) {
              const int piece = kc * PPK + q;
              if (piece < 8 * NB) store_hidden_piece<P, RELU>(pend[piece >> 3], Bout[piece >> 3], mb - 1, piece & 7, pscale, rmax_);
            }
          }
          __builtin_amdgcn_sched_barrier(0);
        }
        bias = bias_next;
        if (mb < MB) {
          if (PIPE) {
#pragma unroll
            for (int nb = 0; nb < NB; ++nb) pend[nb] = acc[nb];
          } else {
#pragma unroll
            for (int nb = 0; nb < NB; ++nb) store_hidden<P, RELU>(acc[nb], Bout[nb], mb, st.out_scale * st.lane_mul, rmax_);
          }
        } else {
#pragma unroll
          for (int nb = 0; nb < NB; ++nb) {
            head[nb] = acc[nb];
            if constexpr (P::kSplit) head[nb] *= st.out_scale * st.lane_mul;
            if constexpr (P::kM16) {
              const f32x16 v = head[nb];
              const bool g1 = (g16 & 1) != 0;
#pragma unroll
              for (int c = 0; c < 8; ++c) {
                if (HALF && c >= 4) head[nb][c] = 0.f;
                else head[nb][c] = g1 ? v[8 * (c >> 2) + 4 + (c & 3)] : v[8 * (c >> 2) + (c & 3)];
              }
            }
          }
        }
      }
    }
  }
  if (PIPE && MB >= 1 && !EXTRA) {
    if (COUT) {
#pragma unroll
      for (int nb = 0; nb < NB; ++nb) carry[nb] = pend[nb];
    } else {
#pragma unroll
      for (int nb = 0; nb < NB; ++nb) store_hidden<P, RELU>(pend[nb], Bout[nb], MB - 1, st.out_scale * st.lane_mul, rmax_);
    }
  }
}

template <class P, bool FAST, int NB, int PC>
DFN_DEV void posenc_xyz(const float (&x)[NB][3], int h, typename FragOf<P>::type (&pe)[NB][PC]) {
  const float base = h ? 32.f : 1.f;
#pragma unroll
  for (int nb = 0; nb < NB; ++nb) {
#pragma unroll
    for (int c = 0; c < 3; ++c) {
      const float xc = x[nb][c];
      if (FAST) {
        float uh, ul, sn[5], cs[5];
        rev_split(xc, uh, ul);
        rev_sincos_octaves5(uh, ul, base, sn, cs);
#pragma unroll
        for (int k = 0; k < 5; ++k) {
          set_slot<P>(pe[nb], 6 * k + c, sn[k]);
          set_slot<P>(pe[nb], 6 * k + 3 + c, cs[k]);
        }
      } else if constexpr (P::kSplit) {
        float uh, ul;
        rev_split(xc, uh, ul);
#pragma unroll
        for (int k = 0; k < 5; ++k) {
          float sn, cs;
          rev_sincos(uh, ul, base * float(1 << k), sn, cs);
          set_slot<P>(pe[nb], 6 * k + c, sn);
          set_slot<P>(pe[nb], 6 * k + 3 + c, cs);
        }
      } else {
        const float xb = xc * base;
#pragma unroll
        for (int k = 0; k < 5; ++k) {
          const float a = xb * float(1 << k);
          set_slot<P>(pe[nb], 6 * k + c, sinf(a));
          set_slot<P>(pe[nb], 6 * k + 3 + c, cosf(a));
        }
      }
    }
    set_slot<P>(pe[nb], 30, h ? x[nb][2] : x[nb][0]);
    set_slot<P>(pe[nb], 31, h ? 0.f : x[nb][1]);
  }
}

template <class P, int PC>
DFN_DEV void posenc_xyz_m16(const float (&x)[2][3], int g, typename FragOf<P>::type (&pe)[1][PC]) {
  static_assert(P::kM16 && PC == 4, "16 slots of two points");
  auto put = [&](int n, int s, float v) {
    _Float16 hi, lo;
    x3_split(v, hi, lo);
    pe[0][2 * (s >> 3) + n].hi[s & 7] = hi;
    pe[0][2 * (s >> 3) + n].lo[s & 7] = lo;
  };
  const float base = float(1 << (2 * g));
  const float f6 = g == 2 ? 512.f : 256.f, f7 = g == 0 ? 256.f : 512.f;
#pragma unroll
  for (int n = 0; n < 2; ++n) {
    float uh[3], ul[3];
#pragma unroll
    for (int c = 0; c < 3; ++c) rev_split(x[n][c], uh[c], ul[c]);
#pragma unroll
    for (int k = 0; k < 2; ++k)
#pragma unroll
      for (int c = 0; c < 3; ++c) {
        float sn, cs;
        rev_sincos(uh[c], ul[c], base * float(1 << k), sn, cs);
        put(n, 6 * k + c, sn);
        put(n, 6 * k + 3 + c, cs);
      }
    float s6, c6, s7, c7;
    rev_sincos(g == 0 ? uh[0] : (g == 1 ? uh[2] : uh[1]), g == 0 ? ul[0] : (g == 1 ? ul[2] : ul[1]), f6, s6, c6);
    rev_sincos(g == 0 ? uh[1] : (g == 1 ? uh[0] : uh[2]), g == 0 ? ul[1] : (g == 1 ? ul[0] : ul[2]), f7, s7, c7);
    if (g == 3) { s6 = x[n][0]; c6 = x[n][1]; s7 = x[n][2]; c7 = 0.f; }
    put(n, 12, s6); put(n, 13, c6); put(n, 14, s7); put(n, 15, c7);
  }
}

struct NoTrunkHook {
  template <class A> DFN_DEV void operator()(int, A&) const {}
};
template <class P, int UMB, bool PIPE, bool FAST, int NB, int W = kWidth, class Hook = NoTrunkHook, int RES_L1 = -1>
DFN_DEV void trunk(Stager& st, char* smem, const float (&x)[lane_pts<P>(NB)][3],
                   typename FragOf<P>::type (&out)[NB][chunks_of<P>(W / 2)], f32x16 (&carry)[NB], Hook hook = Hook()) {
  using F = typename FragOf<P>::type;
  constexpr int PC = chunks_of<P>(32), HC = chunks_of<P>(W / 2), MBW = W / 32;
  constexpr bool CY = PIPE && P::kSlotsPerChunk == 8;
  constexpr int CI = CY ? HC - 2 : -1;
  static_assert(!PIPE || W == kWidth, "the pipelined epilogue is tuned for netwidth 128");
  const int h = st.lane >> 5;
  f32x16 nohead[NB];
  const float* const norb[lane_pts<P>(NB)] = {};
  F pe[NB][PC];
  auto encode = [&](const float (&xx)[lane_pts<P>(NB)][3]) {
    if constexpr (P::kM16) { static_assert(!FAST, "split-f16 only"); posenc_xyz_m16<P, PC>(xx, st.lane >> 4, pe); }
    else posenc_xyz<P, FAST, NB, PC>(xx, h, pe);
  };
  encode(x);
  F a[NB][HC], b[NB][HC];
  layer<P, UMB, PIPE, NB, PC, MBW, true, false, false, RES_L1 < 0, -1, true, CY, false, false, true, false, RES_L1>(st, smem, pe, a, nohead, norb, carry);
  layer<P, UMB, PIPE, NB, HC, MBW, true, false, false, true, CI, true, CY>(st, smem, a, b, nohead, norb, carry);
  hook(0, a[0]);
  layer<P, UMB, PIPE, NB, HC, MBW, true, false, false, true, CI, true, CY>(st, smem, b, a, nohead, norb, carry);
  hook(1, b[0]);
  layer<P, UMB, PIPE, NB, HC, MBW, true, false, false, true, CI, true, CY>(st, smem, a, b, nohead, norb, carry);
  hook(2, a[0]);
  {
    F cat[NB][PC + HC];
    if constexpr (P::kSlotsPerChunk == 8 && (!PIPE || P::kSplit)) {
      float x2[lane_pts<P>(NB)][3];
#pragma unroll
      for (int nb = 0; nb < lane_pts<P>(NB); ++nb)
#pragma unroll
        for (int c = 0; c < 3; ++c) {
          x2[nb][c] = x[nb][c];
          asm volatile("" : "+v"(x2[nb][c]));
        }
      encode(x2);
    }
#pragma unroll
    for (int nb = 0; nb < NB; ++nb) {
#pragma unroll
      for (int i = 0; i < PC; ++i) cat[nb][i] = pe[nb][i];
#pragma unroll
      for (int i = 0; i < HC; ++i) cat[nb][PC + i] = b[nb][i];
    }
    layer<P, l5_unit_mb_p<P>(UMB), PIPE, NB, PC + HC, MBW, true, false, false, true, (CY ? PC + HC - 2 : -1), true, CY>(st, smem, cat, a, nohead, norb, carry);
    hook(3, reinterpret_cast<F(&)[HC]>(cat[0][PC]));
  }
  layer<P, UMB, PIPE, NB, HC, MBW, true, false, false, true, CI, true, CY>(st, smem, a, b, nohead, norb, carry);
  hook(4, a[0]);
  layer<P, UMB, PIPE, NB, HC, MBW, true, false, false, true, CI, true, CY>(st, smem, b, a, nohead, norb, carry);
  hook(5, b[0]);
  layer<P, UMB, PIPE, NB, HC, MBW, true, false, false, true, CI, true, CY>(st, smem, a, out, nohead, norb, carry);
  hook(6, a[0]);
}

}
```

Baseline: 5.823 million rays/s.

## Add dynamic tile claiming via global atomic counter for resident-layer MLP kernels

Adds a new default MLP variant in which each persistent workgroup claims its next tile with a global atomic counter instead of striding by gridDim. The claim is published through an LDS word at the first mid-layer sync so all waves learn the next tile and the prefetch can target it. The aim is to balance load across CUs when tiles finish at uneven rates. It also lets the fused route carve the workspace without the raw buffer. The cost is an extra memset plus one atomic per tile, and it relies on a delicate claim-and-sync protocol inside the pipelined stager.

```diff
diff --git a/dfnet_amd/csrc/nerfh_api.hip b/dfnet_amd/csrc/nerfh_api.hip
--- a/dfnet_amd/csrc/nerfh_api.hip
+++ b/dfnet_amd/csrc/nerfh_api.hip
@@ -126,6 +126,7 @@
   for (hipEvent_t e : h->side_ev) if (e) (void)hipEventDestroy(e);
   if (h->side_stream) (void)hipStreamDestroy(h->side_stream);
   if (h->range_flag) (void)hipFree(h->range_flag);
+  if (h->tile_counter) (void)hipFree(h->tile_counter);
   delete h;
   return DFN_OK;
 }
@@ -519,6 +520,12 @@
       return set_error(DFN_ERR_HIP, "dfn_nerfh_commit: allocating the range-guard flag failed");
     }
     if (hipMemset(h->range_flag, 0, 3 * sizeof(int)) != hipSuccess) return set_error(DFN_ERR_HIP, "dfn_nerfh_commit: clearing the range-guard flag failed");
+  }
+  if (!h->tile_counter) {
+    if (hipMalloc(reinterpret_cast<void**>(&h->tile_counter), 2 * sizeof(uint32_t)) != hipSuccess) {
+      h->tile_counter = nullptr;
+      return set_error(DFN_ERR_HIP, "dfn_nerfh_commit: allocating the tile counters failed");
+    }
   }
   {
     std::vector<float> all;
@@ -773,15 +780,24 @@
 }
 
 constexpr int kDefaultVariant = kResidentVariant;
+constexpr int kSelectedByDefault = kDynVariant;
 static int mlp_variant_128();
 static int mlp_variant_of(dfn_nerfh_t h) { return h->desc.width == kWidth ? mlp_variant_128() : 0; }
 static int mlp_variant_128() {
   static int v = -1;
   if (v < 0) {
     const char* e = getenv("DFN_MLP_VARIANT");
-    v = (e && e[0] >= '0' && e[0] < '0' + kVariants) ? e[0] - '0' : kDefaultVariant;
+    v = (e && e[0] >= '0' && e[0] <= '0' + kDynVariant) ? e[0] - '0' : kSelectedByDefault;
   }
   return v;
+}
+static bool dyn_tiles(dfn_nerfh_t h) { return mlp_variant_of(h) == kDynVariant; }
+static int resolved_variant(dfn_nerfh_t h) { return dyn_tiles(h) ? kResidentVariant : mlp_variant_of(h); }
+static MlpDynArgs dyn_args(const MlpResArgs& r, uint32_t* counter) {
+  MlpDynArgs d{};
+  static_cast<MlpResArgs&>(d) = r;
+  d.tile_counter = counter;
+  return d;
 }
 static int base_variant(int var) { return var == kFoldVariant || var == kHalfVariant || var == kResidentVariant ? 4 : var; }
 static bool fold_fine(int var, int prec) { return (var == kFoldVariant || var == kHalfVariant || var == kResidentVariant) && prec == DFN_PREC_F16X3; }
@@ -819,14 +835,17 @@
   if (int rc = check_net(h, prec, "dfn_mlp_coarse", true)) return rc;
   if (!n_rays) return DFN_OK;
   if (!rays_o || !rays_d || !sigma || Nc < 1) return set_error(DFN_ERR_ARG, "dfn_mlp_coarse: bad argument");
-  const bool half = half_heads(mlp_variant_of(h), prec), res = resident_layers(mlp_variant_of(h), prec);
-  const int var = base_variant(mlp_variant_of(h));
+  const bool half = half_heads(resolved_variant(h), prec), res = resident_layers(resolved_variant(h), prec);
+  const int var = base_variant(resolved_variant(h));
   const PackedNet& n = h->net[0][prec][res ? kResidentVariant : (half ? kHalfVariant : var)];
   MlpArgs a{n.blob, n.tab, n.n_units, rays_o, rays_d, nullptr, nullptr, sigma, nullptr, (long long)n_rays, Nc, near, far, nullptr, n.in_scale,
             h->render_flags & DFN_RENDER_LINDISP};
   a.status = range_flag_of(h);
+  const bool dyn = res && dyn_tiles(h);
+  if (dyn) CHECK_HIP(hipMemsetAsync(h->tile_counter, 0, 2 * sizeof(uint32_t), HS(stream)), "dfn_mlp_coarse(tile counters)");
   ScopedTimer t(0, HS(stream));
-  if (res) CHECK_HIP(launch_mlp_res(false, res_args(a, n), device_cu_count(), HS(stream)), "dfn_mlp_coarse");
+  if (dyn) CHECK_HIP(launch_mlp_dyn(false, dyn_args(res_args(a, n), h->tile_counter), device_cu_count(), HS(stream)), "dfn_mlp_coarse");
+  else if (res) CHECK_HIP(launch_mlp_res(false, res_args(a, n), device_cu_count(), HS(stream)), "dfn_mlp_coarse");
   else if (half) CHECK_HIP(launch_mlp_half(false, false, a, device_cu_count(), HS(stream)), "dfn_mlp_coarse");
   else CHECK_HIP(launch_mlp(false, prec, var, a, device_cu_count(), HS(stream), h->desc.width), "dfn_mlp_coarse");
   return DFN_OK;
@@ -909,8 +928,8 @@
       (hist_rows != 1 && hist_rows != n_rays))
     return set_error(DFN_ERR_ARG, "dfn_mlp_fine: bad argument (hist_rows must be 1 or n_rays)");
   float* table = static_cast<float*>(bias_ws);
-  const bool fold = fold_fine(mlp_variant_of(h), prec);
-  const int var = fold ? kFoldVariant : base_variant(mlp_variant_of(h));
+  const bool fold = fold_fine(resolved_variant(h), prec);
+  const int var = fold ? kFoldVariant : base_variant(resolved_variant(h));
   CHECK_HIP(launch_ray_bias(fold ? h->rb_fold : h->rb, viewdirs, hist, hist_rows, n_rays, table, HS(stream)), "dfn_mlp_fine(ray_bias)");
   const PackedNet& n = h->net[1][prec][var];
   MlpArgs a{n.blob, n.tab, n.n_units, rays_o, rays_d, z_fine, table, raw, nullptr, (long long)n_rays, Nf, 0.f, 0.f, g_timing_buf, n.in_scale};
@@ -944,18 +963,24 @@
 
 namespace {
 constexpr size_t kMaxChunkRays = 65536;
+constexpr size_t kMaxFusedChunkRays = 65536;
 inline size_t al(size_t b) { return (b + 255) & ~size_t(255); }
-inline size_t chunk_rays(size_t n_rays) {
-  const size_t passes = (n_rays + kMaxChunkRays - 1) / kMaxChunkRays;
+inline size_t chunk_rays(size_t n_rays, size_t max_rays = kMaxChunkRays) {
+  const size_t passes = (n_rays + max_rays - 1) / max_rays;
   const size_t c = passes ? (n_rays + passes - 1) / passes : 1;
   return (c + 63) & ~size_t(63);
+}
+inline int fused_segment(int prec) { return prec == DFN_PREC_F16 ? 64 : 32; }
+bool fused_route(dfn_nerfh_t h, int prec, int Nf, bool want_raw) {
+  return !want_raw && Nf % fused_segment(prec) == 0 && !(prec == DFN_PREC_F16 && base_variant(resolved_variant(h)) == 2) && h->desc.width == kWidth;
 }
 struct Workspace {
   float *o, *d, *v, *sigma, *z, *raw, *bias, *partial;
   size_t total;
+  size_t chunk;
 };
-Workspace carve(char* base, size_t n_rays, int Nc, int Ni, bool own_rays, int rec_floats = 12) {
-  const size_t chunk = chunk_rays(n_rays);
+Workspace carve(char* base, size_t n_rays, int Nc, int Ni, bool own_rays, int rec_floats = 12, bool fused = false) {
+  const size_t chunk = chunk_rays(n_rays, fused ? kMaxFusedChunkRays : kMaxChunkRays);
   const size_t Nf = size_t(Nc) + Ni;
   Workspace w{};
   size_t off = 0;
@@ -965,11 +990,16 @@
   w.v = take(n_rays * 12);
   w.sigma = take(chunk * Nc * 4);
   w.z = take(chunk * Nf * 4);
-  w.raw = take(chunk * Nf * 9 * 4);
+  w.raw = fused ? nullptr : take(chunk * Nf * 9 * 4);
   w.bias = take(chunk * ray_bias_floats(kMaxWidth) * 4);
   w.partial = take(chunk * ((Nf + 31) / 32) * rec_floats * 4);
   w.total = off;
+  w.chunk = chunk;
   return w;
+}
+size_t workspace_bytes_any_route(size_t n_rays, int Nc, int Ni, int rec_floats) {
+  const size_t a = carve(nullptr, n_rays, Nc, Ni, true, rec_floats, false).total, b = carve(nullptr, n_rays, Nc, Ni, true, rec_floats, true).total;
+  return a > b ? a : b;
 }
 
 int render_core(dfn_nerfh_t h, int prec, const float* o, const float* d, const float* v, const float* hist,
@@ -977,18 +1007,19 @@
                 float* acc, float* raw_out, const Workspace& w, hipStream_t s, const MapPtrs& maps = MapPtrs{}) {
   const int Nf = Nc + Ni;
   const bool want_maps = maps.any();
-  const bool fold = fold_fine(mlp_variant_of(h), prec);
-  const int var = base_variant(mlp_variant_of(h));
-  const int seg = prec == DFN_PREC_F16 ? 64 : 32;
-  const bool fused = !raw_out && Nf % seg == 0 && !(prec == DFN_PREC_F16 && var == 2) && h->desc.width == kWidth;
+  const bool fold = fold_fine(resolved_variant(h), prec);
+  const int var = base_variant(resolved_variant(h));
+  const int seg = fused_segment(prec);
+  const bool fused = fused_route(h, prec, Nf, raw_out != nullptr);
   const int cprec = (h->render_flags & DFN_RENDER_COARSE_F16) ? DFN_PREC_F16 : prec;
-  const bool half_c = half_heads(mlp_variant_of(h), cprec), half_f = half_heads(mlp_variant_of(h), prec) && fused;
-  const bool res_c = resident_layers(mlp_variant_of(h), cprec), res_f = resident_layers(mlp_variant_of(h), prec) && fused && !want_maps;
+  const bool half_c = half_heads(resolved_variant(h), cprec), half_f = half_heads(resolved_variant(h), prec) && fused;
+  const bool res_c = resident_layers(resolved_variant(h), cprec), res_f = resident_layers(resolved_variant(h), prec) && fused && !want_maps;
   const PackedNet& nc = h->net[0][cprec][res_c ? kResidentVariant : (half_c ? kHalfVariant : var)];
   const PackedNet& nf = res_f ? h->net[1][prec][kResidentVariant]
                       : half_f ? (want_maps ? h->half_maps : h->net[1][prec][kHalfVariant]) : h->net[1][prec][fold ? kFoldVariant : var];
+  const bool dyn_c = res_c && dyn_tiles(h), dyn_f = res_f && dyn_tiles(h);
   const int cus = device_cu_count();
-  const size_t chunk = chunk_rays(n_rays);
+  const size_t chunk = w.chunk;
   for (size_t r0 = 0; r0 < n_rays; r0 += chunk) {
     const size_t n = n_rays - r0 < chunk ? n_rays - r0 : chunk;
     const float* co = o + r0 * 3;
@@ -1000,8 +1031,10 @@
       MlpArgs a{nc.blob, nc.tab, nc.n_units, co, cd, nullptr, nullptr, w.sigma, nullptr, (long long)n, Nc, near, far, nullptr, nc.in_scale,
                  h->render_flags & DFN_RENDER_LINDISP};
       a.status = range_flag_of(h);
+      if (dyn_c || dyn_f) CHECK_HIP(hipMemsetAsync(h->tile_counter, 0, 2 * sizeof(uint32_t), s), "render: tile counters");
       ScopedTimer t(0, s);
-      if (res_c) CHECK_HIP(launch_mlp_res(false, res_args(a, nc), cus, s), "render: coarse MLP (resident layers)");
+      if (dyn_c) CHECK_HIP(launch_mlp_dyn(false, dyn_args(res_args(a, nc), h->tile_counter), cus, s), "render: coarse MLP (claimed tiles)");
+      else if (res_c) CHECK_HIP(launch_mlp_res(false, res_args(a, nc), cus, s), "render: coarse MLP (resident layers)");
       else if (half_c) CHECK_HIP(launch_mlp_half(false, false, a, cus, s), "render: coarse MLP (half-height heads)");
       else CHECK_HIP(launch_mlp(false, cprec, var, a, cus, s, h->desc.width), "render: coarse MLP");
     }
@@ -1018,7 +1051,8 @@
       MlpArgs a{nf.blob, nf.tab, nf.n_units, co, cd, w.z, w.bias, raw, fused ? w.partial : nullptr, (long long)n, Nf, 0.f, 0.f, g_timing_buf, nf.in_scale};
       a.status = range_flag_of(h);
       ScopedTimer t(1, s);
-      if (res_f) CHECK_HIP(launch_mlp_res(true, res_args(a, nf), cus, s), "render: fine MLP (resident layers)");
+      if (dyn_f) CHECK_HIP(launch_mlp_dyn(true, dyn_args(res_args(a, nf), h->tile_counter + 1), cus, s), "render: fine MLP (claimed tiles)");
+      else if (res_f) CHECK_HIP(launch_mlp_res(true, res_args(a, nf), cus, s), "render: fine MLP (resident layers)");
       else if (half_f) CHECK_HIP(launch_mlp_half(true, want_maps, a, cus, s), "render: fine MLP (half-height heads)");
       else if (fold) CHECK_HIP(launch_mlp_fold(fused && want_maps, a, cus, s), "render: fine MLP (folded)");
       else if (fused && want_maps) CHECK_HIP(launch_mlp_maps(true, prec, var, a, cus, s, h->desc.width), "render: fine MLP (maps)");
@@ -1053,7 +1087,7 @@
 }
 
 extern "C" size_t dfn_render_workspace_bytes(size_t n_rays, int Nc, int Ni) {
-  return carve(nullptr, n_rays ? n_rays : 1, Nc, Ni, true).total;
+  return workspace_bytes_any_route(n_rays ? n_rays : 1, Nc, Ni, 12);
 }
 
 static int render_rays_entry(const char* fn, dfn_nerfh_t h, int prec, const float* rays_o, const float* rays_d, const float* viewdirs,
@@ -1065,7 +1099,8 @@
   if (!n_rays) return DFN_OK;
   if (!rays_o || !rays_d || !hist || !rgb || !disp || !acc || !workspace || (hist_rows != 1 && hist_rows != n_rays))
     return set_error(DFN_ERR_ARG, "%s: bad argument (hist_rows must be 1 or n_rays)", fn);
-  const Workspace w = carve(static_cast<char*>(workspace), n_rays, Nc, Ni, true, maps.any() ? kMapsRecFloats : 12);
+  const Workspace w = carve(static_cast<char*>(workspace), n_rays, Nc, Ni, true, maps.any() ? kMapsRecFloats : 12,
+                            fused_route(h, prec, Nc + Ni, raw != nullptr));
   if (w.total > workspace_bytes)
     return set_error(DFN_ERR_ARG, "%s: workspace too small (%zu < %zu)", fn, workspace_bytes, w.total);
   const float* v = viewdirs;
@@ -1086,7 +1121,8 @@
   if (!c2w || !hist || !rgb || !disp || !acc || !workspace || H < 1 || W < 1 || !(focal > 0))
     return set_error(DFN_ERR_ARG, "%s: bad argument", fn);
   const size_t n_rays = size_t(H) * W;
-  const Workspace w = carve(static_cast<char*>(workspace), n_rays, Nc, Ni, true, maps.any() ? kMapsRecFloats : 12);
+  const Workspace w = carve(static_cast<char*>(workspace), n_rays, Nc, Ni, true, maps.any() ? kMapsRecFloats : 12,
+                            fused_route(h, prec, Nc + Ni, false));
   if (w.total > workspace_bytes)
     return set_error(DFN_ERR_ARG, "%s: workspace too small (%zu < %zu)", fn, workspace_bytes, w.total);
   if (hipError_t e = launch_raygen(H, W, focal, c2w, w.o, w.d, w.v, HS(stream)); e != hipSuccess)
@@ -1110,7 +1146,7 @@
 }
 
 extern "C" size_t dfn_render_maps_workspace_bytes(size_t n_rays, int Nc, int Ni) {
-  return carve(nullptr, n_rays ? n_rays : 1, Nc, Ni, true, kMapsRecFloats).total;
+  return workspace_bytes_any_route(n_rays ? n_rays : 1, Nc, Ni, kMapsRecFloats);
 }
 
 extern "C" int dfn_render_rays_maps(dfn_nerfh_t h, int prec, const float* rays_o, const float* rays_d, const float* viewdirs,
@@ -1322,7 +1358,7 @@
 int render_backward_core(dfn_nerfh_t h, int prec, const float* o, const float* d, const float* v, bool derive_v,
                          const float* hist, size_t hist_rows, size_t n_rays, int Nc, int Ni, float near, float far,
                          const float* grad_rgb, float* go, float* gd, float* gv, const BwdWorkspace& w, hipStream_t s) {
-  const int Nf = Nc + Ni, var = base_variant(mlp_variant_of(h)), cus = device_cu_count();
+  const int Nf = Nc + Ni, var = base_variant(resolved_variant(h)), cus = device_cu_count();
   const PackedNet& nc = h->net[0][prec][var];
   const PackedNet& nf = h->net[1][prec][var];
   const PackedNet& nb = h->bwd[prec];
diff --git a/dfnet_amd/csrc/nerfh_handle.h b/dfnet_amd/csrc/nerfh_handle.h
--- a/dfnet_amd/csrc/nerfh_handle.h
+++ b/dfnet_amd/csrc/nerfh_handle.h
@@ -32,6 +32,7 @@
   std::vector<const float*> gen_params;
   int render_flags = 0;
   int* range_flag = nullptr;
+  uint32_t* tile_counter = nullptr;
   void* fused = nullptr;
   bool train_forward_exact = false;
   bool train_split_fine = false;
diff --git a/dfnet_amd/csrc/nerfh_kernels.h b/dfnet_amd/csrc/nerfh_kernels.h
--- a/dfnet_amd/csrc/nerfh_kernels.h
+++ b/dfnet_amd/csrc/nerfh_kernels.h
@@ -36,6 +36,10 @@
   uint32_t res_bytes;
 };
 hipError_t launch_mlp_res(bool fine, const MlpResArgs& a, int n_cu, hipStream_t stream);
+struct MlpDynArgs : MlpResArgs {
+  uint32_t* tile_counter;
+};
+hipError_t launch_mlp_dyn(bool fine, const MlpDynArgs& a, int n_cu, hipStream_t stream);
 
 hipError_t launch_mlp_pts(bool fine, int prec, const MlpArgs& a, int n_cu, hipStream_t stream, int width = 128);
 hipError_t launch_mlp_pts_fold(const MlpArgs& a, int n_cu, hipStream_t stream);
diff --git a/dfnet_amd/csrc/nerfh_layout.h b/dfnet_amd/csrc/nerfh_layout.h
--- a/dfnet_amd/csrc/nerfh_layout.h
+++ b/dfnet_amd/csrc/nerfh_layout.h
@@ -84,6 +84,7 @@
 constexpr int kFoldVariant = 5;
 constexpr int kHalfVariant = 6;
 constexpr int kResidentVariant = 7;
+constexpr int kDynVariant = 8;
 template <class P> DFN_HD constexpr int unit_mb(int variant) {
   return P::kSlotsPerChunk == 1 ? 1 : (P::kSplit ? 2 : (variant == 1 ? 2 : 8));
 }
diff --git a/dfnet_amd/csrc/nerfh_mlp.hip b/dfnet_amd/csrc/nerfh_mlp.hip
--- a/dfnet_amd/csrc/nerfh_mlp.hip
+++ b/dfnet_amd/csrc/nerfh_mlp.hip
@@ -33,6 +33,10 @@
 #define DFN_COARSE_KERNEL nerfh_coarse_pts_kernel
 constexpr bool kHalfHeads = false;
 #endif
+#elif defined(DFN_MLP_DYN_TU)
+#define DFN_FINE_KERNEL nerfh_fine_dyn_kernel
+#define DFN_COARSE_KERNEL nerfh_coarse_dyn_kernel
+constexpr bool kHalfHeads = true;
 #elif defined(DFN_MLP_RES_TU)
 #define DFN_FINE_KERNEL nerfh_fine_res_kernel
 #define DFN_COARSE_KERNEL nerfh_coarse_res_kernel
@@ -56,10 +60,22 @@
 #error "the resident layers exist in the half-height render kernels"
 #endif
 constexpr bool kResident = true;
+#if defined(DFN_MLP_DYN_TU)
+#define DFN_MLP_KARGS MlpDynArgs
+#else
 #define DFN_MLP_KARGS MlpResArgs
-#else
+#endif
+#else
+#if defined(DFN_MLP_DYN_TU)
+#error "the claimed tiles exist in the kernels with resident layers"
+#endif
 constexpr bool kResident = false;
 #define DFN_MLP_KARGS MlpArgs
+#endif
+#if defined(DFN_MLP_DYN_TU)
+#define DFN_NEXT_TILE (static_cast<long long>(st.next))
+#else
+#define DFN_NEXT_TILE (tile + gridDim.x)
 #endif
 
 template <class P, bool FAST> DFN_DEV float head_softplus(float v) { return FAST ? softplus_fast(v) : (P::kSplit ? softplus_hw(v) : softplus(v)); }
@@ -86,6 +102,10 @@
 static_assert(lds_bytes<PrecX3M16, unit_mb<PrecX3M16>(0), 8, 1>() + resident_bytes<PrecX3M16>(true) <= kLdsBytes &&
               lds_bytes<PrecX3M16, unit_mb<PrecX3M16>(0), 8, 1>() + resident_bytes<PrecX3M16>(false) <= kLdsBytes,
               "ring + input slots + resident layers must fit the LDS of a CU");
+constexpr uint32_t kClaimBytes = 16;
+static_assert(lds_bytes<PrecX3M16, unit_mb<PrecX3M16>(0), 8, 1>() + resident_bytes<PrecX3M16>(true) + kClaimBytes <= kLdsBytes &&
+              lds_bytes<PrecX3M16, unit_mb<PrecX3M16>(0), 8, 1>() + resident_bytes<PrecX3M16>(false) + kClaimBytes <= kLdsBytes,
+              "ring + input slots + resident layers + the claimed-tile word must fit the LDS of a CU");
 
 template <class P, int WAVES, int NB, int W> constexpr int mlp_min_blocks() {
   if (W > kWidth && (P::kSplit || P::kSlotsPerChunk == 1 || NB >= 2)) return 1;
@@ -124,8 +144,16 @@
   stage_resident(st, smem, a.res_blob, resident_bytes<P>(false), lds_bytes<P, UMB, WAVES, NB, W>());
 #endif
   stage_prime(st, smem, max_unit_bytes<P>(UMB, W), ring_slots<P, W>());
+#ifdef DFN_MLP_DYN_TU
+  st.claim = 0; st.grid = gridDim.x; st.next = 0; st.n_tiles = uint32_t(n_tiles); st.more = false;
+  st.claim_lds = lds_bytes<P, UMB, WAVES, NB, W>() + resident_bytes<P>(false);
+  for (; tile < n_tiles; tile = st.next) {
+    if (st.wave == 0 && st.lane == 0) st.claim = claim_tile(a.tile_counter);
+    st.claiming = true;
+#else
   for (; tile < n_tiles; tile += gridDim.x) {
     st.more = tile + gridDim.x < n_tiles;
+#endif
     constexpr int LP = lane_pts<P>(NB);
     float x[LP][3];
     uint32_t pt[NB];
@@ -240,8 +268,16 @@
     for (int c = 0; c < 3; ++c) { oin[nb][c] = a.rays_o[ray_of[nb] * 3 + c]; din[nb][c] = a.rays_d[ray_of[nb] * 3 + c]; }
 #endif
   }
+#ifdef DFN_MLP_DYN_TU
+  st.claim = 0; st.grid = gridDim.x; st.next = 0; st.n_tiles = uint32_t(n_tiles); st.more = false;
+  st.claim_lds = lds_bytes<P, UMB, WAVES, NB, W>() + resident_bytes<P>(true);
+  for (; tile < n_tiles; tile = st.next) {
+    if (st.wave == 0 && st.lane == 0) st.claim = claim_tile(a.tile_counter);
+    st.claiming = true;
+#else
   for (; tile < n_tiles; tile += gridDim.x) {
     st.more = tile + gridDim.x < n_tiles;
+#endif
     float x[LP][3];
     uint32_t pt_cur[LP], ray_cur[LP];
 #pragma unroll
@@ -329,7 +365,7 @@
       ray_table(rb_tr, 1);
       layer<P, UMB, PIPE, NB, HC, MBQ, true, false, true, true, -1, true, CY>(st, smem, fin, t0, head, rb_tr, carry);
       if (st.more) {
-        const uint32_t base = uint32_t(tile + gridDim.x) * uint32_t(PPT) + st.wave * (NB * 32);
+        const uint32_t base = uint32_t(DFN_NEXT_TILE) * uint32_t(PPT) + st.wave * (NB * 32);
         char* slot = smem + ring_slots<P, W>() * USTRIDE + st.wave * (PF_ROUNDS * 8 * 256);
 #pragma unroll
         for (int r = 0; r < PF_ROUNDS; ++r) {
@@ -460,7 +496,7 @@
     if (st.more) {
       __builtin_amdgcn_s_waitcnt(0x0F70);
       asm volatile("" ::: "memory");
-      tile_coords(tile + gridDim.x);
+      tile_coords(DFN_NEXT_TILE);
       const char* slot = smem + ring_slots<P, W>() * USTRIDE + st.wave * (PF_ROUNDS * 8 * 256);
 #pragma unroll
       for (int nb = 0; nb < LP; ++nb) {
@@ -553,6 +589,34 @@
               : launch_pts_one<PrecF32, false, 8, 1, 1, false, kWidth, false>(a, n_cu, stream);
 }
 #endif
+#elif defined(DFN_MLP_DYN_TU)
+hipError_t launch_mlp_dyn(bool fine, const MlpDynArgs& a, int n_cu, hipStream_t stream) {
+  using P = PrecX3M16;
+  constexpr int WAVES = 8, UMB = unit_mb<P>(0), NB = 1, PPT = WAVES * NB * 32;
+  const long long n_pts = (long long)a.n_rays * a.n_samples;
+  if (n_pts <= 0) return hipSuccess;
+  if (n_pts >= (1LL << 31)) return hipErrorInvalidValue;
+  if (a.masks || (fine && !a.partial) || !a.tile_counter) return hipErrorInvalidValue;
+  if (!a.res_blob || a.res_bytes != resident_bytes<P>(fine)) return hipErrorInvalidValue;
+  const long long n_tiles = (n_pts + PPT - 1) / PPT;
+  const int grid = int(n_tiles < n_cu ? n_tiles : n_cu);
+  const uint32_t lds = lds_bytes<P, UMB, WAVES, NB>() + resident_bytes<P>(fine) + kClaimBytes;
+  void (*kern)(MlpDynArgs) = fine ? nerfh_fine_dyn_kernel<P, false, WAVES, UMB, NB, true> : nerfh_coarse_dyn_kernel<P, false, WAVES, UMB, NB, true>;
+  static bool attr_done[2] = {false, false};
+  if (!attr_done[fine]) {
+    hipError_t e = hipFuncSetAttribute(reinterpret_cast<const void*>(kern), hipFuncAttributeMaxDynamicSharedMemorySize, int(lds));
+    if (e != hipSuccess) return e;
+    attr_done[fine] = true;
+  }
+  MlpDynArgs b = a;
+  if (b.dma_waves == 0) {
+    static int env = -1;
+    if (env < 0) { const char* e = getenv("DFN_DMA_WAVES"); env = e ? atoi(e) : 0; }
+    b.dma_waves = env > 0 ? env : 4;
+  }
+  hipLaunchKernelGGL(kern, dim3(grid), dim3(WAVES * 64), lds, stream, b);
+  return hipGetLastError();
+}
 #elif defined(DFN_MLP_RES_TU)
 hipError_t launch_mlp_res(bool fine, const MlpResArgs& a, int n_cu, hipStream_t stream) {
   using P = PrecX3M16;
diff --git a/dfnet_amd/csrc/nerfh_mlp_core.h b/dfnet_amd/csrc/nerfh_mlp_core.h
--- a/dfnet_amd/csrc/nerfh_mlp_core.h
+++ b/dfnet_amd/csrc/nerfh_mlp_core.h
@@ -45,6 +45,14 @@
   unsigned long long* trace;
   int n_trace;
   bool more;
+#ifdef DFN_MLP_DYN_TU
+  uint32_t claim;
+  uint32_t grid;
+  uint32_t next;
+  uint32_t n_tiles;
+  uint32_t claim_lds;
+  bool claiming;
+#endif
   float in_scale, out_scale;
   float lane_mul;
   uint32_t rmax;
@@ -74,6 +82,17 @@
   const uint32_t off = (uint32_t)(size_t)DFN_LDS_PTR(lds_dst);
   asm volatile("s_mov_b32 m0, %1\n\tglobal_load_lds_dword %0, off" ::"v"(gptr), "s"(off) : "memory");
 }
+
+#ifdef DFN_MLP_DYN_TU
+typedef volatile uint32_t __attribute__((address_space(3))) lds_vu32;
+DFN_DEV lds_vu32* claim_word(char* smem, uint32_t off) { return reinterpret_cast<lds_vu32*>(DFN_LDS_PTR(smem + off)); }
+DFN_DEV uint32_t claim_tile(uint32_t* counter) {
+  typedef uint32_t __attribute__((address_space(1))) global_u32;
+  uint64_t p = reinterpret_cast<uint64_t>(counter);
+  asm volatile("" : "+v"(p));
+  return __hip_atomic_fetch_add(reinterpret_cast<global_u32*>(p), 1u, __ATOMIC_RELAXED, __HIP_MEMORY_SCOPE_AGENT);
+}
+#endif
 
 DFN_DEV void stage_issue_at(const Stager& st, char* smem, uint32_t off, uint32_t size, uint32_t lds_off) {
   const char* src = st.blob + off + st.lane * 16;
@@ -122,6 +141,13 @@
 #endif
   __builtin_amdgcn_s_waitcnt(0x0F70);
   asm volatile("" ::: "memory");
+#ifdef DFN_MLP_DYN_TU
+  if (st.claiming && st.wave == 0) {
+    if (st.lane == 0) *claim_word(smem, st.claim_lds) = st.grid + st.claim;
+    __builtin_amdgcn_s_waitcnt(0xC07F);
+    asm volatile("" ::: "memory");
+  }
+#endif
 #ifdef DFN_TIMING
   const unsigned long long c1 = __builtin_amdgcn_s_memtime();
 #endif
@@ -140,6 +166,13 @@
     st.trace[2 * st.n_trace + 1] = c2;
   }
   ++st.n_trace;
+#endif
+#ifdef DFN_MLP_DYN_TU
+  if (st.claiming) {
+    st.next = __builtin_amdgcn_readfirstlane(*claim_word(smem, st.claim_lds));
+    st.more = st.next < st.n_tiles;
+    st.claiming = false;
+  }
 #endif
   if (!next_tile || st.more) stage_issue_at(st, smem, st.pf_off, st.pf_size, dst);
   {
diff --git a/dfnet_amd/csrc/nerfh_mlp_dyn.hip b/dfnet_amd/csrc/nerfh_mlp_dyn.hip
--- /dev/null
+++ b/dfnet_amd/csrc/nerfh_mlp_dyn.hip
@@ -0,0 +1,5 @@
+#define DFN_MLP_FOLD_TU 1
+#define DFN_MLP_HALF_TU 1
+#define DFN_MLP_RES_TU 1
+#define DFN_MLP_DYN_TU 1
+#include "nerfh_mlp.hip"
```

After: 5.942 million rays/s, median of 6. 1.02x the previous value.
